# USDA-ARS-GBRU/itsxpress

Hardware: AMD Instinct MI355X
Metric: reads/sec trimmed (ITS2, stand-in taxon Tracheophyta for Fungi) (higher is better)
Workload: dtype u8+f32

## Files before the change

### include/itsx_hip.h

```cpp
#ifndef ITSX_HIP_H
#define ITSX_HIP_H
#include <stdint.h>

#ifdef __cplusplus
extern "C" {
#endif

#define ITSX_ABI_VERSION 6

enum {
  ITSX_OK            =  0,
  ITSX_E_ARG         = -1,
  ITSX_E_IO          = -2,
  ITSX_E_FORMAT      = -3,
  ITSX_E_DEVICE      = -4,
  ITSX_E_UNSUPPORTED = -5,
  ITSX_E_COLLISION   = -6,
  ITSX_E_NOMEM       = -7
};

typedef struct itsx_ctx itsx_ctx;
typedef struct itsx_stream itsx_stream;
typedef struct itsx_keyset itsx_keyset;
typedef struct itsx_twriter itsx_twriter;
// ... 213 lines not shown
int itsx_write_uc(const itsx_ctx *ctx, const char *path);
int itsx_write_rep_fasta(const itsx_ctx *ctx, const char *path);
int itsx_write_domtbl(const itsx_ctx *ctx, const char *path);
int itsx_write_derep_arrays(const char *uc_path, const char *rep_path, int64_t n, const int64_t *rep_of, const int8_t *strand,
                            const int32_t *len, const char *names, const int64_t *name_offsets, const char *seed_bases,
                            const int64_t *seed_offs, int64_t n_seeds);
int itsx_write_domtbl_arrays(const char *path, const itsx_domain *rows, int64_t n_rows, int64_t Z, const int64_t *domz, int32_t n_profiles,
                             const char *prof_names, const int64_t *prof_name_offsets, const int32_t *prof_M, const float *prof_tau,
                             const float *prof_lambda, const char *target_names, const int64_t *target_name_offsets);
const char *itsx_writers_last_error(void);
int itsx_profile_params(const itsx_ctx *ctx, int i, int32_t *M, float *evparam6);
int itsx_get_unique_seqs(itsx_ctx *ctx, char *bases, int64_t cap, int64_t *offsets);

int itsx_get_read_names(const itsx_ctx *ctx, char *names, int64_t cap, int64_t *offsets);

int itsx_get_stats(const itsx_ctx *ctx, itsx_stats *out, int64_t out_size);
int itsx_release_scratch(itsx_ctx *ctx);
int64_t itsx_switches(const itsx_ctx *ctx, char *buf, int64_t cap);
int64_t itsx_switch_registry(char *buf, int64_t cap);

int itsx_write_trimmed_fastq(const char *seq_path, const char *out_path, int compression, int trim_ccs,
                             const int32_t *start, const int32_t *stop, int64_t n_records,
                             int64_t *n_written, int64_t *total_len);
int itsx_twriter_open(const char *out_path, int compression, int trim_ccs, itsx_twriter **w);
int itsx_twriter_set_mode(itsx_twriter *w, int32_t mode);
int itsx_twriter_set_device(itsx_twriter *w, itsx_ctx *ctx);
int itsx_twriter_text(itsx_twriter *w, const char *text, int64_t avail, int32_t last);
int itsx_twriter_coords(itsx_twriter *w, int64_t first_record, int64_t n, const int32_t *start, const int32_t *stop, const uint8_t *decided);
int itsx_twriter_update(itsx_twriter *w, const int64_t *records, int64_t m, const int32_t *start, const int32_t *stop);
int itsx_twriter_close(itsx_twriter *w, int64_t *n_written, int64_t *total_len);

int itsx_write_trimmed_paired(const char *r1_path, const char *r2_path, const char *out1_path, const char *out2_path,
                              int compression, int trim_ccs, const char *names, const int64_t *name_offsets, int64_t n_names,
                              const int32_t *start, const int32_t *stop, const int32_t *tlen, int64_t *n_written);
const char *itsx_trim_last_error(void);
int  itsx_io_read(const char *path, char **text, int64_t *len);
int  itsx_fastq_ids(const char *path, char **names, int64_t **offsets, int64_t *n_records);
void itsx_io_free(char *text);
int  itsx_io_codecs(void);
int64_t itsx_io_parallel_inflates(void);
void itsx_io_cache_clear(void);

int itsx_debug_set_domains(itsx_ctx *ctx, const itsx_domain *rows, int64_t n_rows, const int64_t *seg_rows, int32_t n_segs, int mode);
int64_t itsx_debug_get_rows(itsx_ctx *ctx, itsx_domain *rows, int64_t cap);
int itsx_debug_read_hashes(itsx_ctx *ctx, uint64_t *fwd, uint64_t *rc);
int itsx_debug_read_samples(itsx_ctx *ctx, int32_t *device_ids, int32_t *host_ids);
int itsx_debug_packed_read(const itsx_ctx *ctx, int64_t i, uint32_t *words, int32_t *nwords,
                           uint32_t *exc, int32_t *nexc);
int itsx_debug_calibrate(itsx_ctx *ctx, int pattern, double gbytes, int iters, int64_t *bytes_per_launch, double *ms_per_launch);
int itsx_debug_issue(itsx_ctx *ctx, int op, int waves_per_simd, int iters, double *cycles_per_instr, double *ms);
int itsx_debug_detmath(itsx_ctx *ctx, const double *x, int64_t n, double *out_log, double *out_exp);
int itsx_debug_logf(itsx_ctx *ctx, const float *x, int64_t n, float *out);
int itsx_debug_dust(itsx_ctx *ctx, uint8_t *masked);

#ifdef __cplusplus
}
#endif
#endif
```

### itsxpress_amd/_lib.py

```python
import ctypes as C
import os
import subprocess

import numpy as np

_HERE = os.path.dirname(os.path.abspath(__file__))
LIB_PATH = os.path.join(_HERE, "libitsx_hip.so")
ABI_VERSION = 6
_LIB = None


class EngineError(subprocess.SubprocessError):

    def __init__(self, code, message):
        super().__init__("itsx_hip error %d: %s" % (code, message))
        self.code = code
        self.message = message


DOMAIN_DTYPE = np.dtype([("rep", "<i8"), ("prof", "<i4"), ("tlen", "<i4"), ("ienv", "<i4"), ("jenv", "<i4"),
                         ("dom_idx", "<i4"), ("ndom", "<i4"), ("flags", "<i4"), ("envsc", "<f4"),
                         ("domcorrection", "<f4"), ("dombias", "<f4"), ("bitscore", "<f4"), ("lnP", "<f8"),
                         ("seq_score", "<f4"), ("seq_bias", "<f4"), ("seq_reported", "<i4"),
                         ("dom_reported", "<i4")], align=True)
# ... 9 lines not shown
                ("msv_cells", "<i8"), ("msv_launches", "<i8"), ("ms_fwd_kernel", "<f4"), ("ms_bwd_kernel", "<f4"),
                ("fwd_rows", "<i8"), ("ms_env_kernel", "<f4"), ("ms_bias_kernel", "<f4"), ("env_rows", "<i8"),
                ("n_env_unique", "<i8"), ("ms_decode_kernel", "<f4"), ("n_batches", "<i4"), ("ms_cluster", "<f4"),
                ("n_tw_units_device", "<i4"), ("cl_windows", "<i8"), ("cl_cuts", "<i8"), ("cl_alignments", "<i8"), ("ms_merge", "<f4"),
                ("ms_trim_plan", "<f4"), ("cl_certified", "<i8"), ("ms_pack", "<f4"), ("ms_trim_copy", "<f4"),
                ("n_uniq_multi_winner", "<i8"), ("n_reads_multi_winner", "<i8"), ("n_uniq_region_cap", "<i8"),
                ("n_reads_region_cap", "<i8"), ("n_mr_clustered", "<i8"), ("n_mr_failed", "<i8"), ("n_mr_envelopes", "<i8"),
                ("ms_ensemble", "<f4"), ("ms_deflate", "<f4"), ("n_mr_distinct", "<i8"), ("n_slab_shrinks", "<i8"), ("ms_vit_kernel", "<f4"), ("n_tw_units_host", "<i4"),
                ("n_mr_fail_kind", "<i8", (8,)), ("n_rows_resident", "<i8"),
                ("lazy", "<i4"), ("n_bound_launches", "<i4"), ("n_lazy_pending_profiles", "<i8"), ("n_lazy_completed", "<i8"), ("n_lazy_completed_profiles", "<i8"), ("n_mr_overflow", "<i8"), ("ms_lazy_complete", "<f4"), ("lazy_bound_maxdiff", "<f4"), ("n_lazy_evaluated", "<i8"), ("n_lazy_round1", "<i8"),
                ("n_lazy_pending", "<i8"), ("n_lazy_reruns", "<i8"), ("bound_rows", "<i8"), ("ms_bound_kernel", "<f4"),
                ("ms_lazy_select", "<f4"),
                ("share_B", "<i4"), ("share_batches", "<i4"), ("share_nodes", "<i8"), ("share_chains", "<i8"), ("msv_rows", "<i8"), ("msv_rows_full", "<i8"),
                ("bound_rows_full", "<i8"), ("n_share_helpers", "<i8"), ("share_mismatch", "<i8"), ("ms_share_build", "<f4"), ("share_frac", "<f4"),
                ("two_sided", "<i4"), ("n_bwd_launches", "<i4"), ("n_joined", "<i8"), ("bwd_chains", "<i8"), ("gamma_nodes", "<i8"), ("bwd_rows", "<i8"),
                ("two_fwd_rows", "<i8"), ("two_bwd_rows", "<i8"), ("two_rows_full", "<i8"), ("join_maxdiff", "<f4"), ("ms_bwd_bound", "<f4"),
                ("n_lazy_topup", "<i8"), ("ms_lazy_topup", "<f4"), ("ms_lazy_topup_stages", "<f4"),
                ("ms_inflate", "<f4"), ("n_inflate_members", "<i4"), ("n_inflate_device", "<i8"), ("n_inflate_declined", "<i8")]
STATS_TAIL_FIELDS = [("ms_parse", "<f4"), ("parse_reserved", "<i4"), ("n_parse_device", "<i8"), ("n_parse_declined", "<i8")]
STATS_DTYPE_ALL = np.dtype(STATS_FIELDS + STATS_TAIL_FIELDS, align=True)
_head = np.dtype(STATS_FIELDS, align=True)
STATS_DTYPE = np.dtype({"names": list(_head.names), "formats": [_head.fields[k][0] for k in _head.names],
                        "offsets": [_head.fields[k][1] for k in _head.names], "itemsize": STATS_DTYPE_ALL.itemsize})

EXPORTS = ["itsx_abi_version", "itsx_last_error", "itsx_create", "itsx_destroy", "itsx_load_profiles_file",
           "itsx_load_profiles_mem", "itsx_profile_name", "itsx_profile_tables", "itsx_set_reads", "itsx_set_reads_view", "itsx_set_reads_device", "itsx_domz_device", "itsx_trim_coords_device",
           "itsx_rep_coords_device", "itsx_derep_device", "itsx_unique_keys128_device",
           "itsx_load_reads_file", "itsx_derep", "itsx_cluster", "itsx_cluster_multi", "itsx_cluster_samples", "itsx_get_cluster", "itsx_get_derep", "itsx_unique_keys", "itsx_set_active_uniques", "itsx_get_uniques",
           "itsx_search", "itsx_get_domz", "itsx_set_domz", "itsx_search_finalize", "itsx_num_domains",
           "itsx_get_domains", "itsx_num_pairtraces", "itsx_get_pairtraces", "itsx_trim_coords",
           "itsx_rep_coords", "itsx_write_uc", "itsx_write_rep_fasta", "itsx_write_domtbl", "itsx_get_stats", "itsx_switches", "itsx_switch_registry", "itsx_release_scratch",
           "itsx_debug_read_hashes", "itsx_debug_read_samples", "itsx_debug_packed_read", "itsx_debug_detmath", "itsx_debug_logf", "itsx_debug_dust", "itsx_debug_calibrate", "itsx_debug_issue", "itsx_shard_text", "itsx_shard_last_error", "itsx_owner_verdicts",
           "itsx_write_trimmed_fastq", "itsx_write_trimmed_paired", "itsx_trim_last_error",
           "itsx_merge_buffers", "itsx_merge_pairs_files", "itsx_merge_pairs_load", "itsx_merge_tables",
           "itsx_orient_load_db", "itsx_orient", "itsx_orient_apply", "itsx_write_oriented_fastq",
           "itsx_io_read", "itsx_io_free", "itsx_io_codecs", "itsx_fastq_ids",
           "itsx_load_reads_files", "itsx_set_samples", "itsx_num_samples", "itsx_select_sample",
           "itsx_io_parallel_inflates", "itsx_io_cache_clear", "itsx_get_read_names",
           "itsx_set_rows_mode", "itsx_lazy_pending", "itsx_domz_count", "itsx_lazy_pending_profiles", "itsx_lazy_complete",
           "itsx_load_reads_file_shard", "itsx_unique_keys128", "itsx_write_derep_arrays", "itsx_write_domtbl_arrays",
           "itsx_writers_last_error", "itsx_profile_params", "itsx_get_unique_seqs",
           "itsx_load_reads_text", "itsx_stream_open", "itsx_stream_next", "itsx_stream_close", "itsx_stream_last_error", "itsx_stream_records_bound",
           "itsx_stream_open_shared", "itsx_stream_open_threads", "itsx_stream_base", "itsx_stream_progress", "itsx_stream_next_records", "itsx_count_records",
           "itsx_merge_pairs_load_text", "itsx_merge_pair_index", "itsx_merge_pairs_load_files", "itsx_twriter_set_mode", "itsx_write_range",
           "itsx_keyset_create", "itsx_keyset_destroy", "itsx_keyset_size", "itsx_keyset_assign",
           "itsx_twriter_open", "itsx_twriter_text", "itsx_twriter_coords", "itsx_twriter_update", "itsx_twriter_close",
           "itsx_lazy_pending_uniques", "itsx_set_partial_coords", "itsx_set_kept_rows",
           "itsx_keep_records", "itsx_write_trimmed_samples",
           "itsx_keep_pair_records", "itsx_write_trimmed_paired_samples",
           "itsx_deflate_block_bytes", "itsx_deflate_bound", "itsx_deflate_device", "itsx_debug_huffman_lengths",
           "itsx_twriter_set_device",
           "itsx_inflate_device", "itsx_inflate_fetch", "itsx_debug_inflate_host", "itsx_debug_inflate_candidates", "itsx_debug_inflate_where", "itsx_set_device_inflate",
           "itsx_parse_device", "itsx_parse_fetch", "itsx_debug_parse_host", "itsx_set_device_parse",
           "itsx_debug_set_domains", "itsx_debug_get_rows"]


def lib():
    global _LIB
    if _LIB is not None:
        return _LIB
    if not os.path.exists(LIB_PATH):
        raise FileNotFoundError(
            "%s not found: build the HIP engine first (python -c 'import __graft_entry__ as g; g.build()' "
            "or make -C itsxpress_amd/csrc). There is no CPU fallback." % LIB_PATH)
    L = C.CDLL(LIB_PATH)
    vp, i32, i64, f64, cp = C.c_void_p, C.c_int, C.c_int64, C.c_double, C.c_char_p
    sig = {
        "itsx_abi_version": (i32, []),
        "itsx_last_error": (cp, [vp]),
        "itsx_create": (vp, [i32, i32]),
        "itsx_destroy": (None, [vp]),
        "itsx_load_profiles_file": (i32, [vp, cp, vp]),
        "itsx_load_profiles_mem": (i32, [vp, cp, i64, vp]),
        "itsx_profile_name": (i32, [vp, i32, vp, i32]),
        "itsx_profile_tables": (i32, [vp, i32, vp, vp, vp, vp]),
        "itsx_set_reads": (i32, [vp, vp, vp, i64, vp, vp]),
        "itsx_set_reads_view": (i32, [vp, vp, vp, i64, vp, vp]),
        "itsx_set_reads_device": (i32, [vp, vp, vp, i64, vp, vp]),
        "itsx_domz_device": (i32, [vp, vp, vp]),
        "itsx_trim_coords_device": (i32, [vp, cp, cp, vp, vp]),
        "itsx_rep_coords_device": (i32, [vp, cp, cp, vp, vp]),
        "itsx_derep_device": (i32, [vp, vp, vp, vp, vp]),
        "itsx_unique_keys128_device": (i32, [vp, C.c_uint64, C.c_uint64, i64, vp, vp]),
        "itsx_load_reads_file": (i32, [vp, cp, vp]),
        "itsx_load_reads_file_shard": (i32, [vp, cp, i32, i32, vp, vp, vp]),
        "itsx_load_reads_text": (i32, [vp, vp, i64, vp]),
        "itsx_stream_open": (i32, [cp, vp]),
        "itsx_stream_next": (i32, [vp, i64, vp, vp, vp]),
        "itsx_stream_close": (i32, [vp, i32]),
        "itsx_stream_records_bound": (i64, [vp]),
        "itsx_stream_open_shared": (i32, [cp, cp, vp, vp]),
        "itsx_stream_open_threads": (i32, [cp, i32, vp]),
        "itsx_stream_base": (vp, [vp]),
        "itsx_stream_progress": (i32, [vp, vp, vp, vp]),
        "itsx_stream_next_records": (i32, [vp, i64, vp, vp, vp, vp]),
        "itsx_count_records": (i64, [vp, i64]),
        "itsx_merge_pairs_load_text": (i32, [vp, vp, i64, vp, i64, i32, f64, i32, vp, vp]),
        "itsx_merge_pair_index": (i32, [vp, vp, i64]),
        "itsx_merge_pairs_load_files": (i32, [vp, vp, vp, vp, i32, i32, f64, i32, vp, vp]),
        "itsx_twriter_set_mode": (i32, [vp, i32]),
        "itsx_write_range": (i32, [cp, vp, i64]),
        "itsx_stream_last_error": (cp, []),
        "itsx_keyset_create": (vp, []),
        "itsx_keyset_destroy": (None, [vp]),
        "itsx_keyset_size": (i64, [vp]),
        "itsx_keyset_assign": (i32, [vp, vp, i64, i32, vp, vp]),
        "itsx_twriter_open": (i32, [cp, i32, i32, vp]),
# ... 26 lines not shown
        "itsx_debug_set_domains": (i32, [vp, vp, i64, vp, i32, i32]),
        "itsx_debug_get_rows": (i64, [vp, vp, i64]),
        "itsx_unique_keys128": (i32, [vp, C.c_uint64, C.c_uint64, i64, vp]),
        "itsx_write_derep_arrays": (i32, [cp, cp, i64, vp, vp, vp, vp, vp, vp, vp, i64]),
        "itsx_write_domtbl_arrays": (i32, [cp, vp, i64, i64, vp, i32, vp, vp, vp, vp, vp, vp, vp]),
        "itsx_writers_last_error": (cp, []),
        "itsx_profile_params": (i32, [vp, i32, vp, vp]),
        "itsx_get_unique_seqs": (i32, [vp, vp, i64, vp]),
        "itsx_derep": (i32, [vp, i32, i32, vp]),
        "itsx_cluster": (i32, [vp, f64, i32, vp]),
        "itsx_cluster_multi": (i32, [vp, vp, i32, f64, i32, vp]),
        "itsx_cluster_samples": (i32, [vp, f64, i32, vp]),
        "itsx_get_cluster": (i32, [vp, vp, vp, vp]),
        "itsx_merge_buffers": (i32, [vp, cp, cp, vp, cp, cp, vp, i64, i32, f64, i32, vp, vp, vp, vp, vp, vp]),
        "itsx_merge_pairs_files": (i32, [vp, cp, cp, cp, i32, f64, i32, vp, vp]),
        "itsx_merge_pairs_load": (i32, [vp, cp, cp, i32, f64, i32, vp, vp]),
        "itsx_merge_tables": (i32, [vp, vp, vp, vp, vp]),
        "itsx_orient_load_db": (i32, [vp, cp, vp]),
        "itsx_orient": (i32, [vp, vp, vp, vp]),
        "itsx_orient_apply": (i32, [vp, vp, vp, vp, vp]),
        "itsx_write_oriented_fastq": (i32, [cp, cp, vp, i64, vp]),
        "itsx_unique_keys": (i32, [vp, C.c_uint64, vp, vp]),
        "itsx_set_active_uniques": (i32, [vp, vp]),
        "itsx_get_derep": (i32, [vp, vp, vp, vp]),
        "itsx_get_uniques": (i32, [vp, vp, vp]),
        "itsx_search": (i32, [vp, f64, f64, f64, f64]),
        "itsx_set_rows_mode": (i32, [vp, i32]),
        "itsx_lazy_pending": (i64, [vp]),
        "itsx_lazy_pending_profiles": (i32, [vp, vp]),
        "itsx_lazy_complete": (i32, [vp, vp]),
        "itsx_domz_count": (i64, [vp]),
        "itsx_get_domz": (i32, [vp, vp]),
        "itsx_set_domz": (i32, [vp, vp]),
        "itsx_search_finalize": (i32, [vp, f64]),
        "itsx_num_domains": (i64, [vp]),
        "itsx_get_domains": (i32, [vp, vp]),
        "itsx_num_pairtraces": (i64, [vp]),
        "itsx_get_pairtraces": (i32, [vp, vp, i64]),
        "itsx_trim_coords": (i32, [vp, cp, cp, vp, vp, vp, vp]),
        "itsx_rep_coords": (i32, [vp, cp, cp, vp, vp, vp, vp]),
        "itsx_write_uc": (i32, [vp, cp]),
        "itsx_write_rep_fasta": (i32, [vp, cp]),
        "itsx_write_domtbl": (i32, [vp, cp]),
        "itsx_get_stats": (i32, [vp, vp, i64]),
        "itsx_switches": (i64, [vp, vp, i64]),
        "itsx_release_scratch": (i32, [vp]),
        "itsx_switch_registry": (i64, [vp, i64]),
        "itsx_debug_read_hashes": (i32, [vp, vp, vp]),
        "itsx_debug_read_samples": (i32, [vp, vp, vp]),
        "itsx_debug_packed_read": (i32, [vp, i64, vp, vp, vp, vp]),
        "itsx_debug_detmath": (i32, [vp, vp, i64, vp, vp]),
        "itsx_debug_logf": (i32, [vp, vp, i64, vp]),
        "itsx_debug_dust": (i32, [vp, vp]),
        "itsx_debug_calibrate": (i32, [vp, i32, f64, i32, vp, vp]),
        "itsx_debug_issue": (i32, [vp, i32, i32, i32, vp, vp]),
        "itsx_shard_text": (i32, [C.c_char_p, i32, vp, C.c_char_p, vp, vp]),
        "itsx_shard_last_error": (C.c_char_p, []),
        "itsx_owner_verdicts": (i32, [vp, vp, i64, vp]),
        "itsx_write_trimmed_fastq": (i32, [cp, cp, i32, i32, vp, vp, i64, vp, vp]),
        "itsx_write_trimmed_paired": (i32, [cp, cp, cp, cp, i32, i32, vp, vp, i64, vp, vp, vp, vp]),
        "itsx_trim_last_error": (cp, []),
        "itsx_io_read": (i32, [cp, vp, vp]),
        "itsx_fastq_ids": (i32, [cp, vp, vp, vp]),
        "itsx_io_free": (None, [vp]),
        "itsx_io_codecs": (i32, []),
        "itsx_io_parallel_inflates": (i64, []),
        "itsx_io_cache_clear": (None, []),
        "itsx_get_read_names": (i32, [vp, vp, i64, vp]),
        "itsx_load_reads_files": (i32, [vp, vp, i32, vp]),
        "itsx_set_samples": (i32, [vp, vp, i32]),
        "itsx_num_samples": (i32, [vp]),
        "itsx_select_sample": (i32, [vp, i32]),
    }
    for name, (res, args) in sig.items():
        fn = getattr(L, name)
        fn.restype = res
        fn.argtypes = args
    if L.itsx_abi_version() != ABI_VERSION:
        raise EngineError(-1, "ABI version mismatch: %s reports %d, this package binds version %d" % (LIB_PATH, L.itsx_abi_version(), ABI_VERSION))
    _LIB = L
    return L
```

### itsxpress_amd/csrc/engine.hip

```cpp
#include <algorithm>
#include <chrono>
#include <cmath>
#include <cstdio>
#include <cstring>
#include <functional>
#include <map>
#include <memory>
#include <numeric>
#include <atomic>
#include <condition_variable>
#include <mutex>
#include <string_view>
#include <thread>
#include <unordered_map>
#include "detmath.h"
#include "engine.h"
#include "k_api.h"
#include "deflate_codes.h"
#include "inflate_codes.h"
#include "fastq_rec.h"
#include "twriter_dev.h"
#include "cluster_multi.h"
#include "fastq_io.h"
#include "iupac.h"
// ... 24 lines not shown
}
__global__ void k_waves_build(int nw, int P, const int32_t *__restrict__ order, const int64_t *__restrict__ woff, const int64_t *__restrict__ seg_start,
                              const int32_t *__restrict__ total, const PairRec *__restrict__ pairs, WaveDesc *__restrict__ w, unsigned long long *__restrict__ lane_rows)
{
  const int i = blockIdx.x * blockDim.x + threadIdx.x;
  unsigned long long mine = 0;
  if (i < nw) {
    int lo = 0, hi = P;
    while (hi - lo > 1) { const int mid = (lo + hi) >> 1; if (woff[mid] <= (int64_t)i) lo = mid; else hi = mid; }
    const int p = order[lo];
    const int64_t k = ((int64_t)i - woff[lo]) * 64;
    WaveDesc d;
    d.prof = p; d.first = seg_start[p] + k; d.count = (int32_t)min((int64_t)64, (int64_t)total[p] - k); d.slab = 0;
    int mx = 0;
    for (int q = 0; q < d.count; q++) { const int L = pairs[d.first + q].L; mx = L > mx ? L : mx; mine += (unsigned long long)L; }
    d.rows = mx + 1;
    d.pad = 0;
    w[i] = d;
  }
  for (int o = 32; o >= 1; o >>= 1) mine += __shfl_xor(mine, o, 64);
  if ((threadIdx.x & 63) == 0 && mine) atomicAdd(lane_rows, mine);
}
__global__ void __launch_bounds__(256) k_gather_reads(const uint8_t *__restrict__ src, const int64_t *__restrict__ srcoff, const int64_t *__restrict__ dstoff, int64_t m,
                                                      uint8_t *__restrict__ dst)
{
  const int lane = threadIdx.x & 63;
  for (int64_t j = (int64_t)blockIdx.x * 4 + (threadIdx.x >> 6); j < m; j += (int64_t)gridDim.x * 4) {
    const int64_t so = srcoff[j], d0 = dstoff[j], len = dstoff[j + 1] - d0;
    for (int64_t k = lane; k < len; k += 64) dst[d0 + k] = src[so + k];
  }
}
__global__ void k_wave_rows_regions(const WaveDesc *w, int nw, const RegionRec *rg, int32_t *rows)
{
  const int i = blockIdx.x * blockDim.x + threadIdx.x;
  if (i >= nw) return;
  int mx = 0;
  for (int k = 0; k < w[i].count; k++) { const RegionRec r = rg[w[i].first + k]; mx = max(mx, r.jenv - r.ienv + 1); }
  rows[i] = mx + 1;
}
__global__ void k_pair_counters(const PairOut *po, int64_t n, unsigned long long *c)
{
  unsigned long long a0 = 0, a1 = 0, a2 = 0, a3 = 0, a4 = 0;
  for (int64_t i = (int64_t)blockIdx.x * blockDim.x + threadIdx.x; i < n; i += (int64_t)gridDim.x * blockDim.x) {
    const PairOut o = po[i];
    a0 += o.pass_bias; a1 += o.pass_fwd; a2 += o.pass_fwd ? o.nregions : 0; a3 += (o.flags & 2) ? 1 : 0; a4 += o.pass_fwd ? ((o.flags >> 8) & 0xff) : 0;
  }
  for (int d = 32; d >= 1; d >>= 1) { a0 += __shfl_down(a0, d, 64); a1 += __shfl_down(a1, d, 64); a2 += __shfl_down(a2, d, 64); a3 += __shfl_down(a3, d, 64); a4 += __shfl_down(a4, d, 64); }
  if ((threadIdx.x & 63) == 0) { atomicAdd(&c[0], a0); atomicAdd(&c[1], a1); atomicAdd(&c[2], a2); atomicAdd(&c[3], a3); atomicAdd(&c[4], a4); }
}
__global__ void k_gather_i32(const int32_t *src, const int64_t *idx, int n, int32_t *out)
{
  const int i = blockIdx.x * blockDim.x + threadIdx.x;
  if (i < n) out[i] = src[idx[i]];
}
__global__ void k_rep_coords(int32_t U, const unsigned long long *bl, const unsigned long long *br, const int32_t *cl, const int32_t *cr,
                             const int32_t *seed_read, const int32_t *len, int32_t *start, int32_t *stop, int32_t *tlen)
{
  const int u = blockIdx.x * blockDim.x + threadIdx.x;
  if (u >= U) return;
  const unsigned long long l = bl[u], r = br[u];
  start[u] = l ? cl[u] : -1;
  stop[u] = r ? cr[u] - 1 : -1;
  tlen[u] = (l || r) ? len[seed_read[u]] : -1;
}
__global__ void k_read_coords(int64_t n, const int32_t *uniq_of, const int32_t *us, const int32_t *ue, const int32_t *ut, const int32_t *uind,
                              int32_t *start, int32_t *stop, int32_t *tlen, int32_t *ind)
{
  const int64_t r = (int64_t)blockIdx.x * blockDim.x + threadIdx.x;
  if (r >= n) return;
  const int u = uniq_of[r];
  if (u < 0) { start[r] = stop[r] = tlen[r] = -1; ind[r] = 0; return; }
  start[r] = us[u]; stop[r] = ue[u]; tlen[r] = ut[u]; ind[r] = uind[u];
}
__global__ void k_pack_coords4(int64_t n, const int32_t *a, const int32_t *b, const int32_t *c, const int32_t *d, int32_t *out)
{
  const int64_t i = (int64_t)blockIdx.x * blockDim.x + threadIdx.x;
  if (i < n) { out[i * 4] = a[i]; out[i * 4 + 1] = b[i]; out[i * 4 + 2] = c[i]; out[i * 4 + 3] = d[i]; }
}
__global__ void k_unique_keys128(int32_t U, const int32_t *seed_read, const int32_t *len, const uint64_t *f0, const uint64_t *r0, const uint64_t *f1,
                                 const uint64_t *r1, int64_t base, int64_t *out)
{
  const int u = blockIdx.x * blockDim.x + threadIdx.x;
  if (u >= U) return;
  const int32_t r = seed_read[u];
  const uint64_t lm = (uint64_t)len[r] * 0x9E3779B97F4A7C15ULL;
  const uint64_t kf0 = f0[r] ^ lm, kr0 = r0[r] ^ lm, kf1 = f1[r] ^ lm, kr1 = r1[r] ^ lm;
  const bool fwd_le = (kf0 < kr0) || (kf0 == kr0 && kf1 <= kr1);
  out[(int64_t)u * 4 + 0] = (int64_t)(fwd_le ? kf0 : kr0);
  out[(int64_t)u * 4 + 1] = (int64_t)(fwd_le ? kf1 : kr1);
  out[(int64_t)u * 4 + 2] = base + r;
  out[(int64_t)u * 4 + 3] = fwd_le ? 1 : 0;
}
__global__ void k_widen_i32(int64_t n, const int32_t *in, int64_t *out)
{
  const int64_t i = (int64_t)blockIdx.x * blockDim.x + threadIdx.x;
  if (i < n) out[i] = in[i];
}
}

using namespace itsx;

static std::string g_create_error;

static std::mutex g_grave_mu;
static std::vector<void *> g_grave;
static size_t g_grave_bytes = 0;
// ... 152 lines not shown
  std::vector<int32_t> h_sample, h_usample;
  DBuf<int32_t> d_sample, d_usample;
  const int32_t *dev_sample() const { return S > 1 ? d_sample.p : nullptr; }
  const int32_t *dev_usample() const { return S > 1 ? d_usample.p : nullptr; }
  int32_t usample(int64_t u) const { return S > 1 ? h_usample[(size_t)u] : 0; }
  double slab_gb = 0.0;

  bool have_derep = false;
  std::vector<int32_t> order_cache; bool order_cache_ok = false;
  int derep_strand_both = 1;
  int32_t U = 0;
  int32_t U_active = 0;
  DBuf<int32_t> d_rep_of, d_uniq_of, d_seed_read, d_abund, d_sorted_uniq, d_ulen;
  DBuf<int8_t> d_strand;
  std::vector<int32_t> h_rep_of, h_uniq_of, h_seed_read, h_abund, h_sorted_uniq;
  std::vector<int8_t> h_strand;
  DBuf<uint32_t> d_orient_db; bool have_orient_db = false;
  DBuf<uint32_t> w_orient_tab; DBuf<int32_t> w_orient_list;
  std::vector<int32_t> h_orient_longs;
  bool clustered = false;
  std::vector<double> h_pct;
  std::vector<int32_t> h_order;

  bool have_search = false, have_final = false;
  bool injected = false;
  double T = 10.0;
  int64_t npairs_padded = 0;
  DBuf<PairRec> d_pairs;
  DBuf<PairOut> d_pout;
  DBuf<RegionRec> d_regions;
  DBuf<RegionOut> d_rout;
  DBuf<int64_t> d_pair_region0;
  DBuf<int32_t> d_upos;
  DBuf<RegionRec> d_ulist;
  std::vector<std::unique_ptr<DBuf<itsx_domain>>> dom_bufs;
  std::vector<int64_t> dom_n;
  int64_t pair_budget = 0; int32_t trace_u0 = 0; int n_chunks = 0; bool keep_trace = false, trace_sorted = false;
  DBuf<int16_t> d_vtab; DBuf<VitOut> d_vit; bool have_vit = false; double F2 = 1e-6;
  DBuf<int32_t> d_domz32;
  DBuf<int64_t> d_domz64; bool domz_on_device = false;
  bool compact_rows = false; double compact_zmax = 1e9, compact_dome_min = 1e-2, compact_lnp = 0; int compact_ncls = 0;
  DBuf<itsx_domain> w_domscratch; DBuf<int8_t> w_cls; DBuf<unsigned long long> w_bestc; DBuf<int32_t> w_keep, w_keeppos, w_keeptmp;
  int64_t rows_before_compaction = 0;
  int rows_mode = -1;
  bool lazy = false;
  bool domz_exchanged = false;
  int64_t lazy_pending = 0;
  double sF1 = 1e-6, sF3 = 1e-6;
  std::vector<int64_t> domz_ub;
  std::vector<int64_t> domz_loc, domz_ub_loc;
  bool completing = false;
  std::vector<int32_t> h_plist; DBuf<int32_t> d_plist;
  int64_t s_Uc = 0; int s_Lcap = 0;
  DBuf<float> l_fb; DBuf<uint32_t> l_b10; DBuf<uint8_t> l_done; DBuf<int32_t> l_flag, l_pos, l_scan, l_has; DBuf<unsigned long long> l_gtop, l_sure;
  DBuf<PairRec> l_pairs; DBuf<int64_t> l_seg, l_zub; DBuf<int32_t> l_pflag; DBuf<uint8_t> l_uflag; bool partial_coords = false; bool kept_rows = false; std::vector<int32_t> lazy_pending_prof;
  std::vector<uint16_t> thr_memo; std::vector<char> thr_memo_have; double thr_memo_F1 = -1.0; int thr_memo_Ppad = 0;
  DBuf<int32_t> w_coords4; DBuf<int64_t> w_keys128; DBuf<uint64_t> w_hf1, w_hr1;
  std::vector<int32_t> h_sorted_active;
  DBuf<LenTables> d_lt;
  std::vector<int64_t> domz;
  std::vector<itsx_domain> h_dom;
  std::vector<itsx_pairtrace> h_trace;

  DBuf<uint64_t> w_hf, w_hr; DBuf<unsigned long long> w_keys; DBuf<int32_t> w_vals, w_is_seed, w_seed_rank, w_scan_tmp, w_hist, w_cursor, w_tmp2;
  DBuf<uint32_t> w_slot_of; DBuf<unsigned int> w_ncoll;
  DBuf<uint16_t> w_thr, w_res; DBuf<int32_t> w_tjb, w_cnt, w_total, w_rows, w_rcnt, w_rpref, w_scan2, w_b, w_rrows;
  DBuf<int64_t> w_seg_start, w_idx, w_rseg, w_dz, w_counters, w_useg;
  DBuf<int32_t> w_rrep, w_ruq, w_rurank;
  DBuf<WaveDesc> w_waves, w_rw; DBuf<RegionRec> w_raw; DBuf<float> w_slab, w_eslab;
  DBuf<int32_t> w_mrcnt, w_mroff, w_mrlen, w_mrloff, w_mrrows, w_mrulist, w_mrulist2, w_mru; DBuf<int64_t> w_mrrowoff; DBuf<MrRec> w_mr; DBuf<MrOut> w_mrout; DBuf<int64_t> w_n2off; DBuf<float> w_n2sc, w_mrslab;
  DBuf<uint8_t> w_mrscratch; DBuf<WaveDesc> w_mrwaves;
  DBuf<RegionRec> w_pool, w_pool_sorted; DBuf<int32_t> w_pool_k; DBuf<unsigned long long> w_pool_n, w_pool_key; int64_t pool_cap = 0;
  DBuf<int32_t> w_mrsel; DBuf<int64_t> w_mrselrow; DBuf<MrBig> w_mrbig; DBuf<uint8_t> w_mrarena; DBuf<int32_t> w_mrenv; DBuf<WaveDesc> w_mrbigwaves;
  DBuf<int32_t> w_cl, w_cr;
  DBuf<int8_t> w_side; DBuf<unsigned long long> w_bl, w_br; DBuf<int32_t> w_uind, w_us, w_ue, w_ut, w_rs, w_re, w_rt, w_ri, w_uflag;

  struct ShareBatch { int32_t k0, k1; int64_t node0, nnodes; int32_t nsplit; int64_t gnode0, gnnodes; };
  bool share_on = false; int share_B = 32, share_logB = 5, share_maxd = 0;
  DBuf<unsigned long long> sh_tab, sh_mask_s, sh_mask, sh_counters; DBuf<uint8_t> sh_depth_s, sh_depth;
  DBuf<int32_t> sh_src, sh_parent_s, sh_parent, sh_nn_s, sh_nn, sh_node0_s, sh_node0, sh_order, sh_ulen, sh_uorder, sh_inv, sh_flag, sh_pos, sh_bstart, sh_cursor, sh_segk, sh_scan, sh_cuts;
  std::vector<ShareBatch> sh_batches; std::vector<int32_t> sh_segk_h;
  DBuf<uint4> sh_mgslots; size_t sh_mgslots_half = 0;
  DBuf<uint4> sh_mslots; size_t sh_mslots_half = 0, sh_fslots_half = 0; DBuf<uint32_t> sh_pass, sh_need; DBuf<int32_t> sh_real, sh_segflat, sh_segdepth, sh_wc, sh_woff; DBuf<int64_t> sh_bnd;
  DBuf<uint16_t> sh_res_chk; DBuf<float> sh_fb_chk;
  ShareDev sh_dev{};
  std::string switches_at_search;
  struct TopUp { bool valid = false; int64_t NP = 0; std::vector<int64_t> seg_start; std::vector<int32_t> total; int32_t u0 = 0, Uc = 0; } topup;
  DBuf<unsigned long long> l_zneed, l_zsplit, l_tcnt; DBuf<int32_t> l_slot, l_pslot; DBuf<uint32_t> l_cut;
  std::vector<unsigned long long> h_zneed;
  bool prev_lazy = false; int prev_P = 0; int64_t prev_U = 0, prev_Uc = 0;
  std::vector<int32_t> h_merge_index;
  bool keep_records = false;
  struct Records {
    bool have = false;
    DBuf<uint8_t> seq, qual, titles;
    const uint8_t *seq_p = nullptr;
    DBuf<int64_t> off, toff;
    NameList h_titles;
    void drop() { have = false; seq_p = nullptr; seq.release(); qual.release(); titles.release(); off.release(); toff.release(); h_titles.clear(); }
  } rec;
  bool keep_pair_records = false;
  struct PairRecords {
    bool have = false; int64_t n = 0;
    DBuf<uint8_t> s1, q1, t1, s2, q2, t2;
    DBuf<int64_t> o1, to1, o2, to2;
    DBuf<int32_t> pair_read;
    std::vector<int64_t> pstart;
// ... 1666 lines not shown
    {
      const double n = (double)L;
      const double c = 1.0 + (2.0 * log(2.0 * (n + 3.0) / (3.0 * (n + 2.0))) + n * log((n + 3.0) / (n + 2.0))) / 0.69314718055994529;
      const double margin = std::max(0.02, 6.0 * (n + (double)MMAX) * 5.9604644775390625e-8 / 0.69314718055994529);
      t.lazy_c = nextafterf((float)(c + margin), 1e30f);
    }
    { const float w = roundf((float)(500.0 / 0.69314718055994529) * logf((2.0f + 1.0f) / ((float)L + 2.0f + 1.0f)));
      t.vmove = (w >= 32767.0f) ? 32767 : (w <= -32768.0f) ? -32768 : (int)w; }
  }
  if (ctx->thr_memo_F1 != F1 || ctx->thr_memo_Ppad != Ppad) { ctx->thr_memo.clear(); ctx->thr_memo_have.clear(); ctx->thr_memo_F1 = F1; ctx->thr_memo_Ppad = Ppad; }
  if (ctx->thr_memo_have.size() < (size_t)Lcap) { ctx->thr_memo_have.resize((size_t)Lcap, 0); ctx->thr_memo.resize((size_t)Lcap * Ppad, 257); }
  std::vector<uint16_t> thr((size_t)Lcap * Ppad, 257);
  for (int L = 1; L < Lcap; L++) {
    if (!present[L]) continue;
    if (ctx->thr_memo_have[(size_t)L]) { memcpy(&thr[(size_t)L * Ppad], &ctx->thr_memo[(size_t)L * Ppad], (size_t)Ppad * sizeof(uint16_t)); continue; }
    ctx->thr_memo_have[(size_t)L] = 2;
    for (int p = 0; p < P; p++) {
      const HostProfile &h = ctx->profs[p];
      auto passes = [&](int xj) {
        const float usc = msv_score_from_byte(xj, lt[L].tjb);
        const double Pv = gumbel_surv((double)(usc - lt[L].nullsc) / 0.69314718055994529, (double)h.evparam[0], (double)h.evparam[1]);
        return !(Pv > F1);
      };
      int lo = 0, hi = 255;
      if (!passes(254)) { thr[(size_t)L * Ppad + p] = 256; continue; }
      while (lo < hi) { const int mid = (lo + hi) / 2; if (passes(mid)) hi = mid; else lo = mid + 1; }
      thr[(size_t)L * Ppad + p] = (uint16_t)lo;
    }
  }
  for (int L = 1; L < Lcap; L++)
    if (ctx->thr_memo_have[(size_t)L] == 2) { memcpy(&ctx->thr_memo[(size_t)L * Ppad], &thr[(size_t)L * Ppad], (size_t)Ppad * sizeof(uint16_t)); ctx->thr_memo_have[(size_t)L] = 1; }
  DBuf<uint16_t> &d_thr = ctx->w_thr; DBuf<int32_t> &d_tjb = ctx->w_tjb;
  HIPCHK(upload(ctx->d_lt, lt, st)); HIPCHK(upload(d_thr, thr, st)); HIPCHK(upload(d_tjb, tjb, st));

  HIPCHK(hipStreamSynchronize(st));
  HIPCHK(ctx->d_domz32.alloc((size_t)P * ctx->S));
  HIPCHK(hipMemsetAsync(ctx->d_domz32.p, 0, (size_t)P * ctx->S * 4, st));
  {
    const int64_t cells = cells_active;
    int64_t msum = 0; for (auto &h : ctx->profs) msum += h.M;
    S.msv_cells = cells * msum;
    S.msv_rows = S.msv_rows_full = cells * P; S.bound_rows_full = 0; S.n_share_helpers = 0; S.share_mismatch = 0;
  }
  if (ctx->pair_budget <= 0) {
    size_t fr = 0, tot = 0;
    double gb = 32.0;
    if (hipMemGetInfo(&fr, &tot) == hipSuccess) gb = std::max(1.0, (double)fr / (double)(1ull << 30) / 4.0);
    ctx->pair_budget = (int64_t)(gb * (double)(1ull << 30) / 400.0);
  }
  int64_t lazy_budget = ctx->pair_budget * 5;
  if (ctx->lazy) {
    size_t fr = 0, tot = 0;
    if (hipMemGetInfo(&fr, &tot) == hipSuccess) {
      const double held = (double)ctx->d_pairs.cap * sizeof(PairRec) + (double)ctx->l_fb.cap * 4 + (double)ctx->l_b10.cap * 4 + (double)ctx->l_flag.cap * 4 +
                          (double)ctx->l_pos.cap * 4 + (double)ctx->l_done.cap + (double)ctx->w_res.cap * 2;
      lazy_budget = std::min<int64_t>(lazy_budget, (int64_t)(((double)fr + held) / 3.0 / 64.0));
      lazy_budget = std::max<int64_t>(lazy_budget, (int64_t)1 << 20);
    }
  }
  int64_t Uc = std::max<int64_t>(1, (ctx->lazy ? lazy_budget : ctx->pair_budget) / std::max(P, 1));
  Uc = std::min<int64_t>(Uc, ((1ll << 31) - 4096) / std::max(Ppad, 1));
  if (ctx->lazy && ctx->prev_lazy && ctx->prev_P == P && (int64_t)U <= ctx->prev_U && ctx->prev_Uc > Uc) Uc = ctx->prev_Uc;
  if (const char *e = sw_get("ITSX_CHUNK_UNIQUES")) Uc = std::max<int64_t>(1, atoll(e));
  ctx->keep_trace = sw_get("ITSX_KEEP_TRACE") != nullptr;
  ctx->s_Uc = Uc; ctx->s_Lcap = Lcap;
  ctx->prev_lazy = ctx->lazy; ctx->prev_P = P; ctx->prev_U = U; ctx->prev_Uc = Uc;
  ctx->domz_ub_loc.assign((size_t)P * ctx->S, 0);
  { const int rc = build_share(ctx); if (rc != ITSX_OK) return rc; }
  { const int rc = run_chunks(ctx, T, F1, F3); if (rc != ITSX_OK) return rc; }
  std::vector<int32_t> dz32((size_t)P * ctx->S, 0);
  HIPCHK(hipMemcpyAsync(dz32.data(), ctx->d_domz32.p, dz32.size() * 4, hipMemcpyDeviceToHost, st));
  HIPCHK(hipStreamSynchronize(st));
  ctx->domz_loc.assign(dz32.begin(), dz32.end());
  ctx->domz = ctx->domz_loc; ctx->domz_ub = ctx->domz_ub_loc;
  S.n_rows_resident = 0;
  for (int64_t r : ctx->dom_n) S.n_rows_resident += r;
  if (S.n_mr_failed > 0) {
    ctx->have_search = false;
    SET_ERR(ctx, ITSX_E_UNSUPPORTED, std::to_string(S.n_mr_failed) + " multidomain region(s) with a Forward matrix that cannot be sampled (hmmsearch's stochastic traceback throws on them)");
  }
  return ITSX_OK;
}

struct PairList {
  PairRec *pairs = nullptr; PairOut *pout = nullptr;
  int64_t NP = 0;
  std::vector<int64_t> seg_start;
  std::vector<int32_t> total;
  const int64_t *d_seg_start = nullptr;
};

static int build_waves(itsx_ctx *ctx, const PairList &pl, std::vector<WaveDesc> &waves, std::vector<char> &wgeneric, std::vector<int32_t> &rows)
{
  hipStream_t st = ctx->st;
  const int P = ctx->P;
  waves.clear(); wgeneric.clear();
  for (int pass = 0; pass < 2; pass++)
    for (int p = 0; p < P; p++) {
      if ((int)ctx->generic_q[p] != pass) continue;
      for (int64_t k = 0; k < pl.total[(size_t)p]; k += 64) {
        WaveDesc w{}; w.prof = p; w.first = pl.seg_start[(size_t)p] + k; w.count = (int32_t)std::min<int64_t>(64, pl.total[(size_t)p] - k);
        waves.push_back(w); wgeneric.push_back((char)pass);
      }
    }
  const int NW = (int)waves.size();
  DBuf<WaveDesc> &d_waves = ctx->w_waves; DBuf<int32_t> &d_rows = ctx->w_rows;
  HIPCHK(upload(d_waves, waves, st)); HIPCHK(d_rows.alloc((size_t)std::max(NW, 1)));
  rows.assign((size_t)NW, 0);
// ... 132 lines not shown
      for (int w = w0; w < w1; w++) S.fwd_rows += (int64_t)(rows[w] - 1) * waves[w].count;
      S.n_batches++;
    }
    lazy2.collect();
    lazy.collect();
    S.ms_filters += tm.stop();
  }
  {
    unsigned long long pn = 0;
    HIPCHK(hipMemcpyAsync(&pn, ctx->w_pool_n.p, sizeof(pn), hipMemcpyDeviceToHost, st));
    HIPCHK(hipStreamSynchronize(st));
    if ((int64_t)pn > ctx->pool_cap) {
      while (ctx->pool_cap < (int64_t)pn) ctx->pool_cap *= 2;
      const float keep_ms = S.ms_filters;
      S = stats_before; S.ms_filters = keep_ms; S.n_slab_shrinks++;
      goto pool_retry;
    }
    if (pn > 0) {
      std::vector<RegionRec> hr((size_t)pn); std::vector<int32_t> hk((size_t)pn);
      HIPCHK(hipMemcpyAsync(hr.data(), ctx->w_pool.p, (size_t)pn * sizeof(RegionRec), hipMemcpyDeviceToHost, st));
      HIPCHK(hipMemcpyAsync(hk.data(), ctx->w_pool_k.p, (size_t)pn * 4, hipMemcpyDeviceToHost, st));
      HIPCHK(hipStreamSynchronize(st));
      std::vector<size_t> ord((size_t)pn);
      std::iota(ord.begin(), ord.end(), (size_t)0);
      auto key = [&](size_t i) { return ((unsigned long long)(uint32_t)hr[i].pair << 24) | (unsigned long long)(uint32_t)hk[i]; };
      std::sort(ord.begin(), ord.end(), [&](size_t x, size_t y) { return key(x) < key(y); });
      std::vector<RegionRec> sr((size_t)pn); std::vector<unsigned long long> sk((size_t)pn);
      for (size_t i = 0; i < (size_t)pn; i++) { sr[i] = hr[ord[i]]; sk[i] = key(ord[i]); }
      HIPCHK(upload(ctx->w_pool_sorted, sr, st)); HIPCHK(upload(ctx->w_pool_key, sk, st));
      HIPCHK(hipStreamSynchronize(st));
      pv.rec = ctx->w_pool_sorted.p; pv.key = ctx->w_pool_key.p; pv.n = (int64_t)pn;
    }
  }
  if (next_msv) { const int rc = (*next_msv)(); if (rc != ITSX_OK) return rc; }
  StageTimer tm_dom(st);
  int64_t NMR = 0;
  const bool ensemble = !(sw_get("ITSX_NO_ENSEMBLE") && atoi(sw_get("ITSX_NO_ENSEMBLE")) != 0);
  if (ensemble) {
    DBuf<int32_t> &mrcnt = ctx->w_mrcnt, &mroff = ctx->w_mroff, &stmp = ctx->w_scan2;
    HIPCHK(mrcnt.alloc((size_t)NP + 2)); HIPCHK(mroff.alloc((size_t)NP + 2)); HIPCHK(stmp.alloc((size_t)scan_tmp_elems(NP + 2)));
    launch_mr_count(pl.pout, d_raw.p, pv, NP, mrcnt.p, st);
    launch_exclusive_scan(mrcnt.p, mroff.p, NP + 1, stmp.p, st);
    int32_t tot = 0;
    HIPCHK(hipMemcpyAsync(&tot, mroff.p + NP, 4, hipMemcpyDeviceToHost, st));
    HIPCHK(hipStreamSynchronize(st));
    NMR = tot;
    if (NMR > 0) {
      StageTimer tm_e(st);
      static_assert(sizeof(MrRec) == sizeof(RegionRec), "MrRec is handed to the region memoisation kernels as a RegionRec");
      HIPCHK(ctx->w_mr.alloc((size_t)NMR));
      launch_mr_fill(pl.pout, d_raw.p, pv, NP, mroff.p, ctx->w_mr.p, st);
      DBuf<unsigned long long> &rkeys = ctx->w_keys; DBuf<int32_t> &rvals = ctx->w_vals; DBuf<uint32_t> &rslot = ctx->w_slot_of;
      DBuf<int32_t> &rrep = ctx->w_rrep, &ruq = ctx->w_ruq, &rurank = ctx->w_rurank, &rscan = ctx->w_scan_tmp;
      uint64_t tsize = 1024; while (tsize < (uint64_t)NMR * 2 + 16) tsize <<= 1;
      HIPCHK(rkeys.alloc(tsize)); HIPCHK(rvals.alloc(tsize)); HIPCHK(rslot.alloc((size_t)NMR + 1));
      HIPCHK(rrep.alloc((size_t)NMR + 1)); HIPCHK(ruq.alloc((size_t)NMR + 1)); HIPCHK(rurank.alloc((size_t)NMR + 1)); HIPCHK(rscan.alloc((size_t)scan_tmp_elems(NMR + 1)));
      HIPCHK(hipMemsetAsync(rkeys.p, 0, tsize * sizeof(unsigned long long), st));
      HIPCHK(hipMemsetAsync(rvals.p, 0x7f, tsize * sizeof(int32_t), st));
      HIPCHK(hipMemsetAsync(ruq.p, 0, ((size_t)NMR + 1) * sizeof(int32_t), st));
      const RegionRec *mr_as_regions = (const RegionRec *)ctx->w_mr.p;
      launch_region_keys(ctx->rd, mr_as_regions, NMR, pl.pairs, d_sorted, ctx->d_seed_read.p, rkeys.p, rvals.p, tsize - 1, rslot.p, st);
      launch_region_resolve(ctx->rd, mr_as_regions, NMR, pl.pairs, d_sorted, ctx->d_seed_read.p, rvals.p, rslot.p, rrep.p, ruq.p, st);
      launch_exclusive_scan(ruq.p, rurank.p, NMR + 1, rscan.p, st);
      int32_t NU = 0;
      HIPCHK(hipMemcpyAsync(&NU, rurank.p + NMR, 4, hipMemcpyDeviceToHost, st));
      HIPCHK(hipStreamSynchronize(st));
      DBuf<int32_t> &ulist0 = ctx->w_mrulist, &ulist = ctx->w_mrulist2, &ulen = ctx->w_mrlen, &newpos = ctx->w_mrloff, &mru = ctx->w_mru;
      HIPCHK(ulist0.alloc((size_t)NU + 1)); HIPCHK(ulist.alloc((size_t)NU + 1)); HIPCHK(ulen.alloc((size_t)NU + 2)); HIPCHK(newpos.alloc((size_t)NU + 2)); HIPCHK(mru.alloc((size_t)NMR + 1));
      launch_mr_ulist(NMR, ctx->w_mr.p, rrep.p, ruq.p, rurank.p, ulist0.p, ulen.p, mru.p, st);
      std::vector<int32_t> hlen((size_t)NU), ord((size_t)NU), hpos((size_t)NU);
      HIPCHK(hipMemcpyAsync(hlen.data(), ulen.p, (size_t)NU * 4, hipMemcpyDeviceToHost, st));
      HIPCHK(hipStreamSynchronize(st));
      std::iota(ord.begin(), ord.end(), 0);
      std::stable_sort(ord.begin(), ord.end(), [&](int32_t x, int32_t y) { return hlen[(size_t)x] < hlen[(size_t)y]; });
      std::vector<int64_t> hn2((size_t)NU + 1, 0), hrow((size_t)NU + 1, 0);
      for (int32_t x = 0; x < NU; x++) {
        const int32_t o = ord[(size_t)x];
        hpos[(size_t)o] = x;
        hn2[(size_t)x + 1] = hn2[(size_t)x] + hlen[(size_t)o];
        hrow[(size_t)x + 1] = hrow[(size_t)x] + hlen[(size_t)o] + 1;
      }
      HIPCHK(hipMemcpyAsync(newpos.p, hpos.data(), (size_t)NU * 4, hipMemcpyHostToDevice, st));
      launch_mr_reorder(NU, NMR, newpos.p, ulist0.p, ulist.p, mru.p, st);
      HIPCHK(upload(ctx->w_n2off, hn2, st)); HIPCHK(upload(ctx->w_mrrowoff, hrow, st));
      HIPCHK(ctx->w_mrout.alloc((size_t)NU)); HIPCHK(ctx->w_n2sc.alloc((size_t)hn2[(size_t)NU] + 1));
      static const int lanes_long = sw_get("ITSX_MR_LONG_LANES") ? std::max(1, std::min(MR_LANES, atoi(sw_get("ITSX_MR_LONG_LANES")))) : MR_LANES_LONG;
      static const double frac_long = sw_get("ITSX_MR_LONG_FRAC") ? atof(sw_get("ITSX_MR_LONG_FRAC")) : MR_LONG_FRAC;
      const int64_t n_long = std::min<int64_t>(NU, (int64_t)(frac_long * (double)NU));
      const int64_t waves_target = sw_get("ITSX_MR_WAVES") ? atoll(sw_get("ITSX_MR_WAVES")) : 4096;
      const int lanes_norm = waves_target <= 0 ? MR_LANES : (int)std::max<int64_t>(2, std::min<int64_t>(MR_LANES, (NU + waves_target - 1) / waves_target));
      std::vector<WaveDesc> mw;
      std::vector<int64_t> wfirst;
      for (int64_t x = 0; x < NU;) {
        const int lanes = x >= NU - n_long ? std::min(lanes_long, lanes_norm) : (int)std::min<int64_t>(lanes_norm, NU - n_long - x);
        WaveDesc d{};
        d.prof = -1; d.first = x; d.count = (int32_t)std::min<int64_t>(lanes, (int64_t)NU - x);
        d.rows = hlen[(size_t)ord[(size_t)(d.first + d.count - 1)]] + 1;
        wfirst.push_back(x);
        mw.push_back(d);
        x += d.count;
      }
      const int NMW = (int)mw.size();
      wfirst.push_back(NU);
      HIPCHK(upload(ctx->w_mrwaves, mw, st));
      const int64_t mrow_bytes = (int64_t)MRV * 16;
      const int64_t mbudget = std::max<int64_t>(1, (int64_t)(std::min(slab_gb, 16.0) * (1 << 30)) / mrow_bytes);
      const int64_t wave_cap = std::max<int64_t>(1, ((int64_t)6 << 30) / ((int64_t)MR_SCRATCH * MR_LANES));
// ... 87 lines not shown
            launch_mr_ensemble_big(mb, (int)bw.size(), st);
            x0 = x1;
          }
        }
      }
      S.ms_ensemble += tm_e.stop();
      HIPCHK(hipGetLastError());
      S.n_mr_clustered += NMR; S.n_mr_distinct += NU;
    }
  }
  DBuf<int32_t> &d_rcnt = ctx->w_rcnt, &d_rpref = ctx->w_rpref, &d_scan_tmp = ctx->w_scan2;
  HIPCHK(d_rcnt.alloc((size_t)NP + 1)); HIPCHK(d_rpref.alloc((size_t)NP + 1)); HIPCHK(d_scan_tmp.alloc((size_t)scan_tmp_elems(NP + 1)));
  HIPCHK(hipMemsetAsync(d_rcnt.p, 0, ((size_t)NP + 1) * 4, st));
  RegionListArgs rl{};
  rl.pout = pl.pout; rl.raw = d_raw.p; rl.pv = pv; rl.npairs = NP;
  if (NMR > 0) { rl.mr_off = ctx->w_mroff.p; rl.mr_u = ctx->w_mru.p; rl.mrout = ctx->w_mrout.p; rl.envpool = ctx->w_mrenv.p; }
  {
    DBuf<int64_t> &d_c = ctx->w_counters;
    HIPCHK(d_c.alloc(16));
    HIPCHK(hipMemsetAsync(d_c.p, 0, 16 * sizeof(int64_t), st));
    launch_region_list_count(rl, d_rcnt.p, (unsigned long long *)d_c.p, st);
    int64_t hc[10] = {0};
    HIPCHK(hipMemcpyAsync(hc, d_c.p, sizeof(hc), hipMemcpyDeviceToHost, st));
    HIPCHK(hipStreamSynchronize(st));
    S.n_mr_failed += hc[0]; S.n_mr_envelopes += hc[1];
    for (int k = 0; k < 8; k++) S.n_mr_fail_kind[k] += hc[2 + k];
  }
  launch_exclusive_scan(d_rcnt.p, d_rpref.p, NP + 1, d_scan_tmp.p, st);
  std::vector<int32_t> bound((size_t)P + 1);
  {
    DBuf<int64_t> &d_idx = ctx->w_idx; DBuf<int32_t> &d_b = ctx->w_b;
    HIPCHK(upload(d_idx, pl.seg_start, st)); HIPCHK(d_b.alloc((size_t)P + 1));
    hipLaunchKernelGGL(k_gather_i32, dim3((P + 1 + 255) / 256), dim3(256), 0, st, d_rpref.p, d_idx.p, P + 1, d_b.p);
    HIPCHK(hipMemcpyAsync(bound.data(), d_b.p, ((size_t)P + 1) * 4, hipMemcpyDeviceToHost, st));
    HIPCHK(hipStreamSynchronize(st));
  }
  std::vector<int64_t> rseg((size_t)P + 1, 0);
  std::vector<int32_t> rtotal((size_t)P);
  for (int p = 0; p < P; p++) { rtotal[p] = bound[p + 1] - bound[p]; rseg[p + 1] = rseg[p] + ((int64_t)rtotal[p] + 63) / 64 * 64; S.n_domains += rtotal[p]; }
  const int64_t NR = rseg[P];
  ctx->dom_n[di] = NR;
  HIPCHK(ctx->d_pair_region0.alloc((size_t)NP));
  HIPCHK(ctx->d_regions.alloc((size_t)std::max<int64_t>(NR, 1)));
  HIPCHK(d_dom.alloc((size_t)std::max<int64_t>(NR, 1)));
  HIPCHK(hipMemsetAsync(d_dom.p, 0xFF, (size_t)std::max<int64_t>(NR, 1) * sizeof(itsx_domain), st));
  if (NR > 0) {
    DBuf<int64_t> &d_rseg = ctx->w_rseg;
    HIPCHK(upload(d_rseg, rseg, st));
    launch_region_offsets(NP, pl.pairs, d_rpref.p, pl.d_seg_start, d_rseg.p, ctx->d_pair_region0.p, st);
    HIPCHK(hipMemsetAsync(ctx->d_regions.p, 0xFF, (size_t)NR * sizeof(RegionRec), st));
    launch_region_list_fill(rl, ctx->d_pair_region0.p, ctx->d_regions.p, st);
    DBuf<unsigned long long> &rkeys = ctx->w_keys; DBuf<int32_t> &rvals = ctx->w_vals; DBuf<uint32_t> &rslot = ctx->w_slot_of;
    DBuf<int32_t> &rrep = ctx->w_rrep, &ruq = ctx->w_ruq, &rurank = ctx->w_rurank, &rscan = ctx->w_scan_tmp;
    uint64_t tsize = 1024; while (tsize < (uint64_t)NR * 2 + 16) tsize <<= 1;
    HIPCHK(rkeys.alloc(tsize)); HIPCHK(rvals.alloc(tsize)); HIPCHK(rslot.alloc((size_t)NR + 1));
    HIPCHK(rrep.alloc((size_t)NR + 1)); HIPCHK(ruq.alloc((size_t)NR + 1)); HIPCHK(rurank.alloc((size_t)NR + 1));
    HIPCHK(rscan.alloc((size_t)scan_tmp_elems(NR + 1))); HIPCHK(ctx->d_upos.alloc((size_t)NR + 1));
    HIPCHK(hipMemsetAsync(rkeys.p, 0, tsize * sizeof(unsigned long long), st));
    HIPCHK(hipMemsetAsync(rvals.p, 0x7f, tsize * sizeof(int32_t), st));
    HIPCHK(hipMemsetAsync(ruq.p, 0, ((size_t)NR + 1) * sizeof(int32_t), st));
    launch_region_keys(ctx->rd, ctx->d_regions.p, NR, pl.pairs, d_sorted, ctx->d_seed_read.p, rkeys.p, rvals.p, tsize - 1, rslot.p, st);
    launch_region_resolve(ctx->rd, ctx->d_regions.p, NR, pl.pairs, d_sorted, ctx->d_seed_read.p, rvals.p, rslot.p, rrep.p, ruq.p, st);
    launch_exclusive_scan(ruq.p, rurank.p, NR + 1, rscan.p, st);
    std::vector<int32_t> ub((size_t)P + 1);
    {
      DBuf<int64_t> &d_idx = ctx->w_idx; DBuf<int32_t> &d_b = ctx->w_b;
      HIPCHK(upload(d_idx, rseg, st)); HIPCHK(d_b.alloc((size_t)P + 1));
      hipLaunchKernelGGL(k_gather_i32, dim3((P + 1 + 255) / 256), dim3(256), 0, st, rurank.p, d_idx.p, P + 1, d_b.p);
      HIPCHK(hipMemcpyAsync(ub.data(), d_b.p, ((size_t)P + 1) * 4, hipMemcpyDeviceToHost, st));
      HIPCHK(hipStreamSynchronize(st));
    }
    std::vector<int64_t> useg((size_t)P + 1, 0);
    std::vector<int32_t> utotal((size_t)P);
    for (int p = 0; p < P; p++) { utotal[p] = ub[p + 1] - ub[p]; useg[p + 1] = useg[p] + ((int64_t)utotal[p] + 63) / 64 * 64; S.n_env_unique += utotal[p]; }
    const int64_t NU = useg[P];
    DBuf<int64_t> &d_useg = ctx->w_useg;
    HIPCHK(upload(d_useg, useg, st));
    HIPCHK(ctx->d_ulist.alloc((size_t)std::max<int64_t>(NU, 1))); HIPCHK(ctx->d_rout.alloc((size_t)std::max<int64_t>(NU, 1)));
    HIPCHK(hipMemsetAsync(ctx->d_rout.p, 0, (size_t)std::max<int64_t>(NU, 1) * sizeof(RegionOut), st));
    launch_region_upos(NR, ctx->d_regions.p, pl.pairs, ruq.p, rurank.p, d_rseg.p, d_useg.p, ctx->d_upos.p, ctx->d_ulist.p, st);
    launch_region_upos_follow(NR, rrep.p, ruq.p, ctx->d_upos.p, st);
    std::vector<WaveDesc> rw; std::vector<char> rgen;
    for (int pass = 0; pass < 2; pass++)
      for (int p = 0; p < P; p++) {
        if ((int)ctx->generic_q[p] != pass) continue;
        for (int64_t k = 0; k < utotal[p]; k += 64) {
          WaveDesc w{}; w.prof = p; w.first = useg[p] + k; w.count = (int32_t)std::min<int64_t>(64, utotal[p] - k);
          rw.push_back(w); rgen.push_back((char)pass);
        }
      }
    const int NRW = (int)rw.size();
    DBuf<WaveDesc> &d_rw = ctx->w_rw; DBuf<int32_t> &d_rrows = ctx->w_rrows;
    HIPCHK(upload(d_rw, rw, st)); HIPCHK(d_rrows.alloc((size_t)NRW));
    hipLaunchKernelGGL(k_wave_rows_regions, dim3((NRW + 255) / 256), dim3(256), 0, st, d_rw.p, NRW, ctx->d_ulist.p, d_rrows.p);
    std::vector<int32_t> rrows((size_t)NRW);
    HIPCHK(hipMemcpyAsync(rrows.data(), d_rrows.p, (size_t)NRW * 4, hipMemcpyDeviceToHost, st));
    HIPCHK(hipStreamSynchronize(st));
    const int64_t erow_bytes = 104 * 64 * 4;
    int64_t ebudget = (int64_t)(slab_gb * (1 << 30)) / erow_bytes;
    LazyTimers elazy(st);
    DBuf<float> &d_eslab = ctx->w_eslab; int64_t ealloc = (int64_t)(d_eslab.cap / (104 * 64));
    if (adapt && !sw_get("ITSX_SLAB_GB")) {
      int64_t total_rows = 0;
      for (int w = 0; w < NRW; w++) total_rows += rrows[(size_t)w];
      ebudget = std::min(ebudget, std::max(std::max(total_rows / 4 + 1, ((int64_t)2 << 30) / erow_bytes), ealloc));
    }
    int w0 = 0;
    while (w0 < NRW) {
      int w1 = w0; int64_t r = 0;
      while (w1 < NRW && rgen[w1] == rgen[w0] && (w1 == w0 || r + rrows[w1] <= ebudget)) { rw[w1].slab = r; rw[w1].rows = rrows[w1]; r += rrows[w1]; w1++; }
      if (r > ealloc) {
        if (d_eslab.alloc((size_t)r * 104 * 64) != hipSuccess) {
          (void)hipGetLastError();
          ealloc = 0;
          if (w1 - w0 <= 1) SET_ERR(ctx, ITSX_E_NOMEM, "no device memory left for the envelope slab of a single wave");
          ebudget = std::max<int64_t>(r / 2, rrows[(size_t)w0]);
          S.n_slab_shrinks++;
          continue;
        }
        ealloc = r;
      }
      HIPCHK(hipMemcpyAsync(d_rw.p + w0, rw.data() + w0, (size_t)(w1 - w0) * sizeof(WaveDesc), hipMemcpyHostToDevice, st));
      EnvArgs a{};
      a.rd = ctx->rd; a.sorted_uniq = d_sorted; a.seed_read = ctx->d_seed_read.p; a.prof = ctx->d_prof.p; a.lt = ctx->d_lt.p;
      a.pairs = pl.pairs; a.regions = ctx->d_ulist.p; a.rout = ctx->d_rout.p; a.waves = d_rw.p; a.slab = d_eslab.p;
      { const size_t t = elazy.begin(&S.ms_env_kernel); launch_envelopes(a, w1 - w0, w0, rgen[w0], st); elazy.end(t); }
      for (int w = w0; w < w1; w++) S.env_rows += (int64_t)(rrows[w] - 1) * rw[w].count;
      w0 = w1;
    }
    ScoreArgs sa{};
    sa.rd = ctx->rd; sa.sorted_uniq = d_sorted; sa.seed_read = ctx->d_seed_read.p; sa.prof = ctx->d_prof.p; sa.lt = ctx->d_lt.p;
    sa.flogsum = ctx->d_flogsum.p; sa.pairs = pl.pairs; sa.pout = pl.pout; sa.regions = ctx->d_regions.p; sa.rout = ctx->d_rout.p;
    sa.pair_region0 = ctx->d_pair_region0.p; sa.upos = ctx->d_upos.p; sa.dom = d_dom.p; sa.npairs = NP; sa.T = T;
    if (NMR > 0) { sa.mr = ctx->w_mr.p; sa.mr_u = ctx->w_mru.p; sa.mrout = ctx->w_mrout.p; sa.n2off = ctx->w_n2off.p; sa.n2sc = ctx->w_n2sc.p; sa.mr_off = ctx->w_mroff.p; }
    sa.domz = ctx->d_domz32.p; sa.usample = ctx->dev_usample(); sa.P = ctx->P;
    launch_score(sa, st);
    if (ctx->compact_rows) {
      { const int rc = compact_segment(ctx, d_dom.p, NR, di); if (rc != ITSX_OK) return rc; }
    }
  }
  S.ms_domains += tm_dom.stop();
  {
    DBuf<int64_t> &d_c = ctx->w_counters;
    HIPCHK(d_c.alloc(8));
    HIPCHK(hipMemsetAsync(d_c.p, 0, 8 * sizeof(int64_t), st));
    hipLaunchKernelGGL(k_pair_counters, dim3((unsigned)std::min<int64_t>(4096, (NP + 255) / 256)), dim3(256), 0, st, pl.pout, NP, (unsigned long long *)d_c.p);
    int64_t hc[8];
    HIPCHK(hipMemcpyAsync(hc, d_c.p, sizeof(hc), hipMemcpyDeviceToHost, st));
    HIPCHK(hipStreamSynchronize(st));
    S.n_past_bias += hc[0]; S.n_past_fwd += hc[1]; S.n_regions += hc[2]; S.n_domain_overflow += hc[3]; S.n_multidomain += hc[4];
  }
  HIPCHK(hipGetLastError());
  return ITSX_OK;
}


namespace itsx {
__global__ void k_dbg_group_count(const PairRec *__restrict__ pairs, int64_t NP, const int32_t *__restrict__ flag, const int8_t *__restrict__ cls, int ncls, unsigned long long *__restrict__ cnt)
{
  const int64_t i = (int64_t)blockIdx.x * blockDim.x + threadIdx.x;
  if (i >= NP || !flag[i]) return;
  const PairRec pr = pairs[i];
  if (pr.prof < 0) return;
  atomicAdd(&cnt[(size_t)pr.useq * ncls + cls[pr.prof]], 1ull);
}
__global__ void k_dbg_group_hist(const unsigned long long *__restrict__ cnt, int64_t ng, unsigned long long *__restrict__ hist)
{
  const int64_t i = (int64_t)blockIdx.x * blockDim.x + threadIdx.x;
  if (i >= ng) return;
  const unsigned long long c = cnt[i];
  const int b = c <= 4 ? (int)c : c <= 8 ? 5 : c <= 16 ? 6 : 7;
  atomicAdd(&hist[b], 1ull);
  if (c > 1) atomicAdd(&hist[8], c - 1);
  if (c > 2) atomicAdd(&hist[9], c - 2);
}
}

static int lazy_rounds(itsx_ctx *ctx, const PairList &pl, const int32_t *d_sorted, int32_t u0, int32_t Uc, double T, double F1, double F3, const std::function<int()> *next_msv)
{
  hipStream_t st = ctx->st;
  const int P = ctx->P, ncls = ctx->compact_ncls;
  itsx_stats &S = ctx->stats;
  const int64_t NP = pl.NP;
  HIPCHK(ctx->l_fb.alloc((size_t)NP + 1)); HIPCHK(ctx->l_b10.alloc((size_t)NP + 1)); HIPCHK(ctx->l_done.alloc((size_t)NP + 1));
  HIPCHK(ctx->l_flag.alloc((size_t)NP + 2)); HIPCHK(ctx->l_pos.alloc((size_t)NP + 2)); HIPCHK(ctx->l_scan.alloc((size_t)scan_tmp_elems(NP + 2)));
  HIPCHK(ctx->l_gtop.alloc((size_t)Uc * ncls + 1));
  HIPCHK(hipMemsetAsync(ctx->l_done.p, 0, (size_t)NP + 1, st));
  HIPCHK(hipMemsetAsync(ctx->l_gtop.p, 0, ((size_t)Uc * ncls + 1) * sizeof(unsigned long long), st));
  if (ctx->share_on) {
    const int maxd = ctx->share_maxd, DS = maxd + 1;
    const bool two = ctx->two_on;
    std::vector<int32_t> segflat, segdepth, segbatch;
    for (size_t bi = 0; bi < ctx->sh_batches.size(); bi++) {
      const auto &b = ctx->sh_batches[bi];
      if (b.k0 < u0 || b.k0 >= u0 + Uc) continue;
      for (int d = 0; d < DS; d++) { segflat.push_back(ctx->sh_segk_h[bi * SHARE_SEGS + d] - u0); segdepth.push_back(d); segbatch.push_back((int32_t)bi); }
    }
    const int nseg = (int)segdepth.size();
    segflat.push_back(Uc);
    if ((int64_t)nseg * P + 1 >= (1ll << 31)) SET_ERR(ctx, ITSX_E_UNSUPPORTED, "prefix sharing: too many (batch, depth, profile) segments in one chunk");
    HIPCHK(upload(ctx->sh_segflat, segflat, st)); HIPCHK(upload(ctx->sh_segdepth, segdepth, st, 1)); HIPCHK(upload(ctx->w_rcnt, pl.total, st));
    HIPCHK(ctx->sh_bnd.alloc((size_t)(nseg + 1) * P)); HIPCHK(ctx->sh_wc.alloc((size_t)nseg * P + 2)); HIPCHK(ctx->sh_woff.alloc((size_t)nseg * P + 2));
    HIPCHK(ctx->sh_scan.alloc((size_t)scan_tmp_elems((int64_t)nseg * P + 2)));
    launch_share_bounds(pl.pairs, pl.d_seg_start, ctx->w_rcnt.p, ctx->sh_segflat.p, nseg, P, ctx->sh_bnd.p, st);
    launch_share_wcount(ctx->sh_bnd.p, nseg, P, ctx->sh_wc.p, st);
    launch_exclusive_scan(ctx->sh_wc.p, ctx->sh_woff.p, (int64_t)nseg * P + 1, ctx->sh_scan.p, st);
    std::vector<int32_t> woff((size_t)nseg * P + 1);
    HIPCHK(hipMemcpyAsync(woff.data(), ctx->sh_woff.p, woff.size() * 4, hipMemcpyDeviceToHost, st));
    HIPCHK(hipStreamSynchronize(st));
    const int NW = woff.back();
    HIPCHK(ctx->w_waves.alloc((size_t)std::max(NW, 1))); HIPCHK(ctx->w_counters.alloc(512));
    HIPCHK(hipMemsetAsync(ctx->w_counters.p, 0, 512 * sizeof(int64_t), st));
    launch_share_waves(NW, nseg, P, ctx->sh_woff.p, ctx->sh_bnd.p, ctx->sh_segdepth.p, ctx->share_B, pl.pairs, two ? ctx->sh_endrow.p + u0 : nullptr, 0, ctx->w_waves.p,
                       (unsigned long long *)ctx->w_counters.p, st);
    std::vector<int64_t> lr((size_t)384, 0);
    FloatArgs a{};
    a.rd = ctx->rd; a.sorted_uniq = d_sorted; a.seed_read = ctx->d_seed_read.p; a.prof = ctx->d_prof.p; a.lt = ctx->d_lt.p;
    a.pairs = pl.pairs; a.waves = ctx->w_waves.p; a.F1 = F1; a.F3 = F3;
    const int maxrd = ctx->share_maxrd, DSB = maxrd + 1;
    int32_t cb0 = 0, Ubc = 0; int NWB = 0;
    std::vector<int32_t> bwoff;
    FloatArgs ab = a;
    if (two) {
      int32_t cb1 = 0; bool any = false;
      std::vector<int32_t> bsegflat, bsegdepth;
      for (size_t bi = 0; bi < ctx->sh_batches.size(); bi++) {
        const auto &b = ctx->sh_batches[bi];
        if (b.k0 < u0 || b.k0 >= u0 + Uc) continue;
        const int32_t lo = ctx->sh_bsegk_h[bi * SHARE_SEGS], hi = ctx->sh_bsegk_h[bi * SHARE_SEGS + SHARE_SEGS - 1];
        if (!any) { cb0 = lo; any = true; }
        cb1 = hi;
      }
      Ubc = any ? cb1 - cb0 : 0;
      for (size_t bi = 0; bi < ctx->sh_batches.size(); bi++) {
        const auto &b = ctx->sh_batches[bi];
        if (b.k0 < u0 || b.k0 >= u0 + Uc) continue;
        for (int d = 0; d < DSB; d++) { bsegflat.push_back(ctx->sh_bsegk_h[bi * SHARE_SEGS + d] - cb0); bsegdepth.push_back(d); }
      }
// ... 155 lines not shown
      for (int p = 0; p < P; p++) {
        if ((int)ctx->generic_q[p] != pass) continue;
        order.push_back(p);
        woff.push_back(woff.back() + ((int64_t)pl.total[(size_t)p] + 63) / 64);
        if (pass == 0) nfast64 = woff.back();
      }
    if (woff.back() >= (1ll << 31)) SET_ERR(ctx, ITSX_E_UNSUPPORTED, "more than 2^31 waves of pairs in one chunk");
    const int NW = (int)woff.back(), nfast = (int)nfast64;
    DBuf<int32_t> &d_order = ctx->w_b; DBuf<int64_t> &d_woff = ctx->w_idx; DBuf<int32_t> &d_tot = ctx->w_rcnt;
    HIPCHK(upload(d_order, order, st)); HIPCHK(upload(d_woff, woff, st)); HIPCHK(upload(d_tot, pl.total, st));
    HIPCHK(ctx->w_waves.alloc((size_t)std::max(NW, 1))); HIPCHK(ctx->w_counters.alloc(16));
    HIPCHK(hipMemsetAsync(ctx->w_counters.p, 0, 16 * sizeof(int64_t), st));
    if (NW > 0) hipLaunchKernelGGL(k_waves_build, dim3((NW + 255) / 256), dim3(256), 0, st, NW, (int)order.size(), d_order.p, d_woff.p, pl.d_seg_start, d_tot.p,
                                   pl.pairs, ctx->w_waves.p, (unsigned long long *)ctx->w_counters.p);
    int64_t lane_rows = 0;
    HIPCHK(hipMemcpyAsync(&lane_rows, ctx->w_counters.p, sizeof(lane_rows), hipMemcpyDeviceToHost, st));
    FloatArgs a{};
    a.rd = ctx->rd; a.sorted_uniq = d_sorted; a.seed_read = ctx->d_seed_read.p; a.prof = ctx->d_prof.p; a.lt = ctx->d_lt.p;
    a.pairs = pl.pairs; a.waves = ctx->w_waves.p; a.F1 = F1; a.F3 = F3;
    StageTimer tm(st);
    static const bool exact_bound = sw_get("ITSX_LAZY_EXACT_BOUND") && atoi(sw_get("ITSX_LAZY_EXACT_BOUND")) != 0;
    if (!exact_bound) {
      for (int w0 = 0; w0 < NW; w0 += 1 << 20) { launch_fwd_bound_seq(a, ctx->d_btab.p, ctx->bound_fold, ctx->l_fb.p, std::min(1 << 20, NW - w0), w0, st); S.n_bound_launches++; }
    } else {
      for (int w0 = 0; w0 < nfast; w0 += 1 << 20) { launch_fwd_bound(a, ctx->l_fb.p, std::min(1 << 20, nfast - w0), w0, 0, st); S.n_bound_launches++; }
      if (NW > nfast) { launch_fwd_bound(a, ctx->l_fb.p, NW - nfast, nfast, 1, st); S.n_bound_launches++; }
    }
    const float ms = tm.stop();
    S.ms_bound_kernel += ms; S.ms_filters += ms;
    if (sw_get("ITSX_LAZY_CHECK_BOUND") && !exact_bound) {
      DBuf<float> ref;
      HIPCHK(ref.alloc((size_t)NP + 1));
      for (int w0 = 0; w0 < nfast; w0 += 1 << 20) launch_fwd_bound(a, ref.p, std::min(1 << 20, nfast - w0), w0, 0, st);
      if (NW > nfast) launch_fwd_bound(a, ref.p, NW - nfast, nfast, 1, st);
      std::vector<float> h0((size_t)NP), h1((size_t)NP); std::vector<PairRec> hp((size_t)NP);
      HIPCHK(hipMemcpyAsync(h0.data(), ref.p, (size_t)NP * 4, hipMemcpyDeviceToHost, st));
      HIPCHK(hipMemcpyAsync(h1.data(), ctx->l_fb.p, (size_t)NP * 4, hipMemcpyDeviceToHost, st));
      HIPCHK(hipMemcpyAsync(hp.data(), pl.pairs, (size_t)NP * sizeof(PairRec), hipMemcpyDeviceToHost, st));
      HIPCHK(hipStreamSynchronize(st));
      float mx = S.lazy_bound_maxdiff;
      for (int64_t i = 0; i < NP; i++) {
        if (hp[(size_t)i].prof < 0) continue;
        const float x = h0[(size_t)i], y = h1[(size_t)i];
        if (x != x || y != y) { if ((x != x) != (y != y)) mx = 1e30f; continue; }
        mx = std::max(mx, fabsf(x - y));
      }
      S.lazy_bound_maxdiff = mx;
    }
    S.bound_rows += lane_rows; S.bound_rows_full += lane_rows;
  }
  StageTimer tm_sel(st);
  LazyArgs la{};
  la.pairs = pl.pairs; la.NP = NP; la.fb = ctx->l_fb.p; la.lt = ctx->d_lt.p; la.cls = ctx->w_cls.p; la.ncls = ncls; la.sorted_uniq = d_sorted;
  la.b10 = ctx->l_b10.p; la.gtop = ctx->l_gtop.p; la.bestc = ctx->w_bestc.p; la.done = ctx->l_done.p; la.flag = ctx->l_flag.p;
  launch_lazy_bound(la, st);
  float ms_sel = tm_sel.stop();
  for (int round = 0; round < 2; round++) {
    StageTimer tm_r(st);
    launch_lazy_mark(la, round, st);
    if (round == 1 && sw_get("ITSX_LAZY_HIST")) {
      const int64_t ng = (int64_t)Uc * ncls;
      HIPCHK(hipMemsetAsync(ctx->l_gtop.p, 0, (size_t)ng * 8, st));
      hipLaunchKernelGGL(k_dbg_group_count, dim3((unsigned)((NP + 255) / 256)), dim3(256), 0, st, pl.pairs, NP, ctx->l_flag.p, ctx->w_cls.p, ncls, ctx->l_gtop.p);
      DBuf<unsigned long long> hist; HIPCHK(hist.alloc(16)); HIPCHK(hipMemsetAsync(hist.p, 0, 16 * 8, st));
      hipLaunchKernelGGL(k_dbg_group_hist, dim3((unsigned)((ng + 255) / 256)), dim3(256), 0, st, ctx->l_gtop.p, ng, hist.p);
      unsigned long long h[16];
      HIPCHK(hipMemcpyAsync(h, hist.p, sizeof(h), hipMemcpyDeviceToHost, st)); HIPCHK(hipStreamSynchronize(st));
      fprintf(stderr, "[itsx] round 2 candidates per group: 0:%llu 1:%llu 2:%llu 3:%llu 4:%llu 5-8:%llu 9-16:%llu 17+:%llu; pairs beyond a group's first %llu, beyond its second %llu\n",
              h[0], h[1], h[2], h[3], h[4], h[5], h[6], h[7], h[8], h[9]);
    }
    launch_exclusive_scan(ctx->l_flag.p, ctx->l_pos.p, NP + 1, ctx->l_scan.p, st);
    std::vector<int32_t> bound((size_t)P + 1);
    {
      DBuf<int64_t> &d_idx = ctx->w_idx; DBuf<int32_t> &d_b = ctx->w_b;
      HIPCHK(upload(d_idx, pl.seg_start, st)); HIPCHK(d_b.alloc((size_t)P + 1));
      hipLaunchKernelGGL(k_gather_i32, dim3((P + 1 + 255) / 256), dim3(256), 0, st, ctx->l_pos.p, d_idx.p, P + 1, d_b.p);
      HIPCHK(hipMemcpyAsync(bound.data(), d_b.p, ((size_t)P + 1) * 4, hipMemcpyDeviceToHost, st));
      HIPCHK(hipStreamSynchronize(st));
    }
    PairList sub;
    sub.seg_start.assign((size_t)P + 1, 0); sub.total.assign((size_t)P, 0);
    for (int p = 0; p < P; p++) { sub.total[(size_t)p] = bound[(size_t)p + 1] - bound[(size_t)p]; sub.seg_start[(size_t)p + 1] = sub.seg_start[(size_t)p] + ((int64_t)sub.total[(size_t)p] + 63) / 64 * 64; }
    sub.NP = sub.seg_start[(size_t)P];
    const int64_t nsel = (int64_t)bound[(size_t)P] - bound[0];
    const bool last = round == 1;
    if (sub.NP == 0) {
      ms_sel += tm_r.stop();
      if (last && next_msv) { const int rc = (*next_msv)(); if (rc != ITSX_OK) return rc; }
      continue;
    }
    HIPCHK(ctx->l_pairs.alloc((size_t)sub.NP)); HIPCHK(ctx->d_pout.alloc((size_t)sub.NP));
    HIPCHK(hipMemsetAsync(ctx->l_pairs.p, 0xFF, (size_t)sub.NP * sizeof(PairRec), st));
    HIPCHK(hipMemsetAsync(ctx->d_pout.p, 0, (size_t)sub.NP * sizeof(PairOut), st));
    HIPCHK(upload(ctx->l_seg, sub.seg_start, st));
    launch_lazy_scatter(pl.pairs, NP, ctx->l_flag.p, ctx->l_pos.p, pl.d_seg_start, ctx->l_seg.p, ctx->l_pairs.p, st);
    sub.pairs = ctx->l_pairs.p; sub.pout = ctx->d_pout.p; sub.d_seg_start = ctx->l_seg.p;
    ms_sel += tm_r.stop();
    S.n_lazy_evaluated += nsel;
    if (round == 0) S.n_lazy_round1 += nsel;
    { const int rc = domain_pipeline(ctx, sub, d_sorted, T, F1, F3, last ? next_msv : nullptr); if (rc != ITSX_OK) return rc; }
  }
  S.ms_lazy_select += ms_sel; S.ms_filters += ms_sel;
  ctx->topup.valid = !ctx->completing; ctx->topup.NP = NP; ctx->topup.seg_start = pl.seg_start; ctx->topup.total = pl.total; ctx->topup.u0 = u0; ctx->topup.Uc = Uc;
  return ITSX_OK;
}

static int search_chunk(itsx_ctx *ctx, int ci, int32_t u0, int32_t U, int Lcap, double T, double F1, double F3)
{
  (void)ci;
  hipStream_t st = ctx->st;
  const int P = ctx->P, G = ctx->G, Ppad = G * 64;
  itsx_stats &S = ctx->stats;
  const bool sh = ctx->share_on;
  const int32_t *d_sorted = (sh ? ctx->sh_order.p : ctx->d_sorted_uniq.p) + u0;
  const int32_t *d_ulen = (sh ? ctx->sh_ulen.p : ctx->d_ulen.p) + u0;
  DBuf<uint16_t> &d_thr = ctx->w_thr; DBuf<int32_t> &d_tjb = ctx->w_tjb;
  ctx->trace_u0 = u0;
  DBuf<uint16_t> &d_res = ctx->w_res;
  HIPCHK(d_res.alloc((size_t)Ppad * std::max<int64_t>(U, ctx->next_u0 >= 0 ? ctx->next_U : 0)));
  auto msv_for = [&](int64_t cu0, int32_t cU, hipStream_t s, int lds_pad = 0, uint16_t *res_out = nullptr, bool shared = true) {
    MsvArgs a{};
    a.rd = ctx->rd; a.sorted_uniq = (sh ? ctx->sh_order.p : ctx->d_sorted_uniq.p) + cu0; a.seed_read = ctx->d_seed_read.p; a.U = cU; a.G = G;
    a.etab = ctx->d_etab.p; a.pbias = ctx->d_pbias.p; a.ptec = ctx->d_ptec.p; a.ptbm = ctx->d_ptbm.p;
    a.thr = d_thr.p; a.tjb = d_tjb.p; a.Lcap = Lcap; a.res = res_out ? res_out : d_res.p;
    a.P = P;
    const int64_t tiles = ((int64_t)cU + 255) / 256;
    if (ctx->completing) {
      a.plist = ctx->d_plist.p; a.nlist = (int32_t)ctx->h_plist.size();
      (void)hipMemsetAsync(a.res, 0, (size_t)Ppad * (size_t)cU * sizeof(uint16_t), s);
    }
    const int np = a.plist ? a.nlist : P;
    a.PB = (int)std::max<int64_t>(1, std::min<int64_t>(32, tiles * np / 4096));
    if (!sh || !shared || ctx->completing) { launch_msv(a, s, lds_pad); return; }
    static const bool two = !(sw_get("ITSX_SHARE_MSV_STREAMS") && atoi(sw_get("ITSX_SHARE_MSV_STREAMS")) < 2);
    int nbatch_here = 0;
    for (const auto &b : ctx->sh_batches) nbatch_here += (b.k0 >= cu0 && b.k0 < cu0 + cU);
    hipStream_t alt = s;
    if (two && nbatch_here > 1) {
      if (!ctx->st3) {
        if (hipStreamCreateWithFlags(&ctx->st3, hipStreamNonBlocking) != hipSuccess) { (void)hipGetLastError(); ctx->st3 = nullptr; }
        else { (void)hipEventCreateWithFlags(&ctx->ev_s3a, hipEventDisableTiming); (void)hipEventCreateWithFlags(&ctx->ev_s3b, hipEventDisableTiming); }
      }
      if (ctx->st3) { alt = ctx->st3; (void)hipEventRecord(ctx->ev_s3a, s); (void)hipStreamWaitEvent(alt, ctx->ev_s3a, 0); }
    }
    static const bool msv_two = !(sw_get("ITSX_MSV_TWO") && atoi(sw_get("ITSX_MSV_TWO")) == 0);
    const bool bi2 = ctx->two_on && msv_two;
    int32_t cb0 = 0;
    if (bi2) { bool any = false; for (const auto &b : ctx->sh_batches) if (b.k0 >= cu0 && b.k0 < cu0 + cU && !any) { cb0 = ctx->sh_bsegk_h[(size_t)(&b - ctx->sh_batches.data()) * SHARE_SEGS]; any = true; } }
    int seen = 0;
// ... 333 lines not shown
  for (size_t c = 0; c < ctx->dom_n.size(); c++)
    if (ctx->dom_n[c] > 0) launch_finalize_lazy(ctx->dom_bufs[c]->p, ctx->dom_n[c], d_dz.p, d_dz.p + m, domE, ctx->dev_usample(), ctx->P, st);
  for (size_t c = 0; c < ctx->dom_n.size(); c++)
    if (ctx->dom_n[c] > 0) launch_lazy_sure(ctx->dom_bufs[c]->p, ctx->dom_n[c], ctx->w_cls.p, ncls, ctx->l_sure.p, ctx->l_has.p, st);
  for (size_t c = 0; c < ctx->dom_n.size(); c++)
    if (ctx->dom_n[c] > 0) launch_lazy_pending(ctx->dom_bufs[c]->p, ctx->dom_n[c], ctx->w_cls.p, ncls, ctx->l_sure.p, ctx->l_has.p, (unsigned long long *)ctx->w_counters.p, ctx->l_pflag.p, ctx->l_uflag.p, ctx->S == 1 ? ctx->l_zneed.p : nullptr, ctx->l_zsplit.p, domE, st);
  int64_t pend = 0;
  ctx->h_zneed.assign((size_t)std::max(ctx->P, 1) * 2, 0);
  HIPCHK(hipMemcpyAsync(ctx->h_zneed.data(), ctx->l_zneed.p, (size_t)std::max(ctx->P, 1) * 2 * sizeof(unsigned long long), hipMemcpyDeviceToHost, st));
  HIPCHK(hipMemcpyAsync(&pend, ctx->w_counters.p, sizeof(pend), hipMemcpyDeviceToHost, st));
  ctx->lazy_pending_prof.assign((size_t)std::max(ctx->P, 1), 0);
  HIPCHK(hipMemcpyAsync(ctx->lazy_pending_prof.data(), ctx->l_pflag.p, (size_t)std::max(ctx->P, 1) * 4, hipMemcpyDeviceToHost, st));
  HIPCHK(hipStreamSynchronize(st));
  { int np = 0; for (int32_t f : ctx->lazy_pending_prof) np += f != 0; ctx->stats.n_lazy_pending_profiles = np; }
  if (sw_get("ITSX_LAZY_FORCE_PENDING")) pend += atoll(sw_get("ITSX_LAZY_FORCE_PENDING"));
  ctx->lazy_pending = pend; ctx->stats.n_lazy_pending = pend;
  return ITSX_OK;
}

static int lazy_topup(itsx_ctx *ctx, double domE, bool *ran)
{
  (void)domE;
  *ran = false;
  const auto &tu = ctx->topup;
  if (sw_get("ITSX_LAZY_HIST")) fprintf(stderr, "[itsx] top-up: valid %d chunks %d samples %d pairs %lld\n", (int)tu.valid, ctx->n_chunks, ctx->S, (long long)tu.NP);
  if (!tu.valid || ctx->n_chunks != 1 || ctx->S != 1 || tu.NP <= 0) return ITSX_OK;
  if (sw_get("ITSX_LAZY_TOPUP") && atoi(sw_get("ITSX_LAZY_TOPUP")) == 0) return ITSX_OK;
  hipStream_t st = ctx->st;
  const int P = ctx->P;
  itsx_stats &S = ctx->stats;
  std::vector<int32_t> slot((size_t)P, -1), prof_of;
  for (int p = 0; p < P; p++) {
    if (!ctx->lazy_pending_prof[(size_t)p]) continue;
    if (ctx->h_zneed[(size_t)2 * p] == 0 && ctx->h_zneed[(size_t)2 * p + 1] == ~0ull) continue;
    slot[(size_t)p] = (int32_t)prof_of.size(); prof_of.push_back(p);
  }
  const int ns = (int)prof_of.size();
  if (ns == 0) return ITSX_OK;
  StageTimer tm(st);
  const int64_t NP = tu.NP;
  HIPCHK(upload(ctx->l_slot, slot, st)); HIPCHK(upload(ctx->l_pslot, prof_of, st));
  HIPCHK(upload(ctx->w_idx, tu.seg_start, st)); HIPCHK(upload(ctx->w_rcnt, tu.total, st));
  auto count_done = [&](std::vector<unsigned long long> &out) -> int {
    HIPCHK(ctx->l_tcnt.alloc((size_t)ns));
    HIPCHK(hipMemsetAsync(ctx->l_tcnt.p, 0, (size_t)ns * sizeof(unsigned long long), st));
    launch_topup_count(ctx->l_done.p, ctx->w_idx.p, ctx->w_rcnt.p, ctx->l_pslot.p, ns, ctx->l_tcnt.p, st);
    out.assign((size_t)ns, 0);
    HIPCHK(hipMemcpyAsync(out.data(), ctx->l_tcnt.p, (size_t)ns * sizeof(unsigned long long), hipMemcpyDeviceToHost, st));
    HIPCHK(hipStreamSynchronize(st));
    return ITSX_OK;
  };
  std::vector<unsigned long long> ndone;
  { const int rc = count_done(ndone); if (rc != ITSX_OK) return rc; }
  launch_topup_keys(ctx->d_pairs.p, NP, ctx->l_done.p, ctx->l_b10.p, ctx->l_slot.p, ctx->l_flag.p, nullptr, nullptr, nullptr, st);
  launch_exclusive_scan(ctx->l_flag.p, ctx->l_pos.p, NP + 1, ctx->l_scan.p, st);
  int32_t M32 = 0;
  HIPCHK(hipMemcpyAsync(&M32, ctx->l_pos.p + NP, 4, hipMemcpyDeviceToHost, st));
  HIPCHK(hipStreamSynchronize(st));
  const int64_t M = M32;
  if (M <= 0) return ITSX_OK;
  HIPCHK(ctx->sh_keys.alloc((size_t)M + 1)); HIPCHK(ctx->sh_keys2.alloc((size_t)M + 1)); HIPCHK(ctx->sh_vals.alloc((size_t)M + 1)); HIPCHK(ctx->sh_uorder.alloc((size_t)M + 1));
  const size_t sort_bytes = order_sort_bytes(M);
  HIPCHK(ctx->sh_sorttmp.alloc(sort_bytes));
  launch_topup_keys(ctx->d_pairs.p, NP, ctx->l_done.p, ctx->l_b10.p, ctx->l_slot.p, ctx->l_flag.p, ctx->l_pos.p, ctx->sh_keys.p, ctx->sh_vals.p, st);
  if (order_sort(ctx->sh_sorttmp.p, sort_bytes, ctx->sh_keys.p, ctx->sh_keys2.p, ctx->sh_vals.p, ctx->sh_uorder.p, M, st) != 0) SET_ERR(ctx, ITSX_E_DEVICE, "top-up round: the radix sort failed");
  HIPCHK(hipStreamSynchronize(st));
  auto lower = [&](unsigned long long key, int64_t &pos) -> int {
    int64_t lo = 0, hi = M;
    while (lo < hi) {
      const int64_t mid = (lo + hi) >> 1; unsigned long long v = 0;
      HIPCHK(hipMemcpy(&v, ctx->sh_keys2.p + mid, 8, hipMemcpyDeviceToHost));
      if (v < key) lo = mid + 1; else hi = mid;
    }
    pos = lo; return ITSX_OK;
  };
  std::vector<uint32_t> cut((size_t)2 * ns, 0);
  bool any = false;
  for (int k = 0; k < ns; k++) {
    const int p = prof_of[(size_t)k];
    int64_t a = 0, b = 0;
    { const int rc = lower((unsigned long long)k << 32, a); if (rc != ITSX_OK) return rc; }
    { const int rc = lower((unsigned long long)(k + 1) << 32, b); if (rc != ITSX_OK) return rc; }
    const int64_t have = b - a;
    if (have <= 0) continue;
    const int64_t lo = ctx->domz[(size_t)p], hi = lo + have;
    int64_t from_top = 0, from_bottom = 0;
    const unsigned long long zl = ctx->h_zneed[(size_t)2 * p], zh = ctx->h_zneed[(size_t)2 * p + 1];
    if (zl > 0 && (int64_t)zl > lo) { const int64_t need = (int64_t)zl - lo; from_top = need + need / 50 + 64; }
    const bool both = sw_get("ITSX_LAZY_TOPUP") && atoi(sw_get("ITSX_LAZY_TOPUP")) == 2;
    if (both && zh != ~0ull && hi > (int64_t)zh) { const int64_t need = hi - (int64_t)zh; from_bottom = need + need / 4 + 64; }
    if (sw_get("ITSX_LAZY_HIST")) fprintf(stderr, "[itsx] top-up: profile %d bounds %lld .. %lld (%lld unevaluated), rows need >= %llu / <= %llu: best %lld, weakest %lld\n", p, (long long)lo, (long long)hi,
                                          (long long)have, zl, zh == ~0ull ? 0ull : zh, (long long)from_top, (long long)from_bottom);
    static const bool topup_all = !(sw_get("ITSX_LAZY_TOPUP_ALL") && atoi(sw_get("ITSX_LAZY_TOPUP_ALL")) == 0);
    const bool above = zh != ~0ull && hi > (int64_t)zh;
    if ((above && !both) || from_top + from_bottom > have - have / 3) {
      if (!topup_all) continue;
      cut[(size_t)2 * k] = 1u; cut[(size_t)2 * k + 1] = 0u;
      any = true;
      continue;
    }
    unsigned long long v = 0;
    if (from_top > 0) {
      HIPCHK(hipMemcpy(&v, ctx->sh_keys2.p + a + from_top - 1, 8, hipMemcpyDeviceToHost));
      cut[(size_t)2 * k] = std::max<uint32_t>(1u, 0xFFFFFFFFu - (uint32_t)(v & 0xFFFFFFFFull));
    }
    if (from_bottom > 0) {
      HIPCHK(hipMemcpy(&v, ctx->sh_keys2.p + b - from_bottom, 8, hipMemcpyDeviceToHost));
      cut[(size_t)2 * k + 1] = std::max<uint32_t>(1u, 0xFFFFFFFFu - (uint32_t)(v & 0xFFFFFFFFull));
      if (cut[(size_t)2 * k] > 0 && cut[(size_t)2 * k + 1] >= cut[(size_t)2 * k]) { cut[(size_t)2 * k] = cut[(size_t)2 * k + 1] = 0; continue; }
    }
    any = any || from_top > 0 || from_bottom > 0;
  }
  if (!any) return ITSX_OK;
  HIPCHK(upload(ctx->l_cut, cut, st));
  launch_topup_mark(ctx->d_pairs.p, NP, ctx->l_done.p, ctx->l_b10.p, ctx->l_slot.p, ctx->l_cut.p, ctx->l_flag.p, st);
  launch_exclusive_scan(ctx->l_flag.p, ctx->l_pos.p, NP + 1, ctx->l_scan.p, st);
  std::vector<int32_t> bound((size_t)P + 1);
  {
    DBuf<int32_t> &d_b = ctx->w_b;
    HIPCHK(d_b.alloc((size_t)P + 1));
    hipLaunchKernelGGL(k_gather_i32, dim3((P + 1 + 255) / 256), dim3(256), 0, st, ctx->l_pos.p, ctx->w_idx.p, P + 1, d_b.p);
    HIPCHK(hipMemcpyAsync(bound.data(), d_b.p, ((size_t)P + 1) * 4, hipMemcpyDeviceToHost, st));
    HIPCHK(hipStreamSynchronize(st));
  }
  PairList sub;
  sub.seg_start.assign((size_t)P + 1, 0); sub.total.assign((size_t)P, 0);
  for (int p = 0; p < P; p++) { sub.total[(size_t)p] = bound[(size_t)p + 1] - bound[(size_t)p]; sub.seg_start[(size_t)p + 1] = sub.seg_start[(size_t)p] + ((int64_t)sub.total[(size_t)p] + 63) / 64 * 64; }
  sub.NP = sub.seg_start[(size_t)P];
  const int64_t nsel = (int64_t)bound[(size_t)P] - bound[0];
  if (sub.NP == 0) return ITSX_OK;
  HIPCHK(ctx->l_pairs.alloc((size_t)sub.NP)); HIPCHK(ctx->d_pout.alloc((size_t)sub.NP));
  HIPCHK(hipMemsetAsync(ctx->l_pairs.p, 0xFF, (size_t)sub.NP * sizeof(PairRec), st));
  HIPCHK(hipMemsetAsync(ctx->d_pout.p, 0, (size_t)sub.NP * sizeof(PairOut), st));
  HIPCHK(upload(ctx->l_seg, sub.seg_start, st));
  launch_lazy_scatter(ctx->d_pairs.p, NP, ctx->l_flag.p, ctx->l_pos.p, ctx->w_seg_start.p, ctx->l_seg.p, ctx->l_pairs.p, st);
  sub.pairs = ctx->l_pairs.p; sub.pout = ctx->d_pout.p; sub.d_seg_start = ctx->l_seg.p;
  const int32_t *d_sorted = (ctx->share_on ? ctx->sh_order.p : ctx->d_sorted_uniq.p) + tu.u0;
  ctx->trace_u0 = tu.u0;
  { StageTimer tp(st); const int rc = domain_pipeline(ctx, sub, d_sorted, ctx->T, ctx->sF1, ctx->sF3, nullptr); if (rc != ITSX_OK) return rc; S.ms_lazy_topup_stages += tp.stop(); }
  std::vector<int32_t> dz32((size_t)P * ctx->S, 0);
  HIPCHK(hipMemcpyAsync(dz32.data(), ctx->d_domz32.p, dz32.size() * 4, hipMemcpyDeviceToHost, st));
  HIPCHK(upload(ctx->w_idx, tu.seg_start, st)); HIPCHK(upload(ctx->w_rcnt, tu.total, st));
  { const int rc = count_done(ndone); if (rc != ITSX_OK) return rc; }
  for (size_t z = 0; z < dz32.size(); z++) { ctx->domz_loc[z] = dz32[z]; ctx->domz[z] = dz32[z]; }
  for (int k = 0; k < ns; k++) {
    const int p = prof_of[(size_t)k];
    const int64_t left = (int64_t)tu.total[(size_t)p] - (int64_t)ndone[(size_t)k];
    const int64_t hi = (int64_t)dz32[(size_t)p] + std::max<int64_t>(0, left);
    if (hi < ctx->domz_ub[(size_t)p]) { ctx->domz_ub[(size_t)p] = hi; ctx->domz_ub_loc[(size_t)p] = hi; }
    if (sw_get("ITSX_LAZY_HIST")) fprintf(stderr, "[itsx] top-up: profile %d now %d .. %lld\n", p, dz32[(size_t)p], (long long)ctx->domz_ub[(size_t)p]);
  }
  S.n_lazy_evaluated += nsel; S.n_lazy_topup += nsel;
  S.n_rows_resident = 0;
  for (int64_t r : ctx->dom_n) S.n_rows_resident += r;
  S.ms_lazy_topup += tm.stop();
  *ran = true;
  return ITSX_OK;
}

int itsx_search_finalize(itsx_ctx *ctx, double domE)
{
  CTXCHK(ctx && ctx->have_search);
  HIPCHK(hipSetDevice(ctx->device));
  if (ctx->injected && ctx->lazy && !ctx->domz_exchanged)
    SET_ERR(ctx, ITSX_E_ARG, "itsx_search_finalize: a lazy row table that was handed in (itsx_debug_set_domains) has no counters of its own: give both bounds with itsx_set_domz first");
  StageTimer tm(ctx->st);
  ctx->h_dom.clear();
  auto check_compaction = [&](const std::vector<int64_t> &z) -> int {
    int64_t zmax = 0;
    for (int64_t v : z) zmax = std::max(zmax, v);
    if ((double)zmax > ctx->compact_zmax || domE < ctx->compact_dome_min)
      SET_ERR(ctx, ITSX_E_UNSUPPORTED, "compacted domain rows: only the rows that are reported for every domZ <= " + std::to_string(ctx->compact_zmax) +
              " and every domE >= " + std::to_string(ctx->compact_dome_min) + " were kept, but finalize got domZ up to " + std::to_string(zmax) + " and domE " + std::to_string(domE) +
              " (raise ITSX_COMPACT_ZMAX / lower ITSX_COMPACT_DOME_MIN and search again)");
    return ITSX_OK;
  };
  if (ctx->lazy) {
    { const int rc = finalize_lazy(ctx, domE); if (rc != ITSX_OK) return rc; }
    { const int rc = check_compaction(ctx->domz_ub); if (rc != ITSX_OK) return rc; }
    if (ctx->lazy_pending > 0 && !ctx->domz_exchanged && !sw_get("ITSX_LAZY_NO_RERUN")) {
      const int64_t pend = ctx->lazy_pending;
      {
        bool ran = false;
        { const int rc = lazy_topup(ctx, domE, &ran); if (rc != ITSX_OK) return rc; }
        if (ran) {
          { const int rc = finalize_lazy(ctx, domE); if (rc != ITSX_OK) return rc; }
          ctx->stats.n_lazy_pending = pend;
          if (ctx->lazy_pending == 0) {
            ctx->stats.ms_finalize = tm.stop();
// ... 2025 lines not shown
  return ITSX_OK;
}

int itsx_debug_detmath(itsx_ctx *ctx, const double *x, int64_t n, double *out_log, double *out_exp)
{
  CTXCHK(ctx && x && out_log && out_exp && n >= 0);
  HIPCHK(hipSetDevice(ctx->device));
  DBuf<double> dx, dl, de;
  HIPCHK(dx.alloc((size_t)n + 1)); HIPCHK(dl.alloc((size_t)n + 1)); HIPCHK(de.alloc((size_t)n + 1));
  if (n > 0) {
    HIPCHK(hipMemcpyAsync(dx.p, x, (size_t)n * 8, hipMemcpyHostToDevice, ctx->st));
    launch_detmath(dx.p, n, dl.p, de.p, ctx->st);
    HIPCHK(hipMemcpyAsync(out_log, dl.p, (size_t)n * 8, hipMemcpyDeviceToHost, ctx->st));
    HIPCHK(hipMemcpyAsync(out_exp, de.p, (size_t)n * 8, hipMemcpyDeviceToHost, ctx->st));
  }
  HIPCHK(hipStreamSynchronize(ctx->st));
  return ITSX_OK;
}

int itsx_debug_dust(itsx_ctx *ctx, uint8_t *masked)
{
  CTXCHK(ctx && masked);
  HIPCHK(hipSetDevice(ctx->device));
  const int64_t n = ctx->N;
  if (n == 0) return ITSX_OK;
  DBuf<uint32_t> dm;
  HIPCHK(dm.alloc((size_t)ctx->h_woff[n] + 1));
  launch_dust(ctx->rd, dm.p, ctx->st);
  std::vector<uint32_t> h((size_t)ctx->h_woff[n] + 1);
  HIPCHK(hipMemcpyAsync(h.data(), dm.p, h.size() * 4, hipMemcpyDeviceToHost, ctx->st));
  HIPCHK(hipStreamSynchronize(ctx->st));
  HIPCHK(hipGetLastError());
  int64_t o = 0;
  for (int64_t r = 0; r < n; r++)
    for (int p = 0; p < ctx->h_len[r]; p++) masked[o++] = (uint8_t)((h[(size_t)ctx->h_woff[r] + (p >> 5)] >> (p & 31)) & 1u);
  return ITSX_OK;
}

int itsx_debug_logf(itsx_ctx *ctx, const float *x, int64_t n, float *out)
{
  CTXCHK(ctx && x && out && n >= 0);
  HIPCHK(hipSetDevice(ctx->device));
  DBuf<float> dx, dy;
  HIPCHK(dx.alloc((size_t)n + 1)); HIPCHK(dy.alloc((size_t)n + 1));
  if (n > 0) {
    HIPCHK(hipMemcpyAsync(dx.p, x, (size_t)n * 4, hipMemcpyHostToDevice, ctx->st));
    launch_logf_fast(dx.p, n, ctx->d_logtab.p, dy.p, ctx->st);
    HIPCHK(hipMemcpyAsync(out, dy.p, (size_t)n * 4, hipMemcpyDeviceToHost, ctx->st));
  }
  HIPCHK(hipStreamSynchronize(ctx->st));
  return ITSX_OK;
}

}
```

### itsxpress_amd/csrc/k_api.h

```cpp
#pragma once
#include "engine.h"

#include "detmath.h"
namespace itsx {

struct ReadsDev {
  const uint32_t *words;
  const int64_t  *woff;
  const int32_t  *len;
  const int64_t  *excoff;
  const uint32_t *exc;
  int64_t         n;
};

void launch_hash_reads(const ReadsDev &rd, uint64_t seed, int strand_both, uint64_t *hf, uint64_t *hr, hipStream_t st, const int32_t *sample = nullptr);
void launch_table_insert(int64_t n, const int32_t *len, int minlen, const uint64_t *hf, const uint64_t *hr,
                         unsigned long long *keys, int32_t *vals, uint64_t mask, uint32_t *slot_of, hipStream_t st);
void launch_table_resolve(const ReadsDev &rd, const uint64_t *hf, const int32_t *vals, const uint32_t *slot_of,
                          int32_t *rep_of, int8_t *strand, int32_t *is_seed, unsigned int *n_collisions, hipStream_t st,
                          const int32_t *sample = nullptr);
void launch_uniques(int64_t n, const int32_t *rep_of, const int32_t *seed_rank, int32_t *uniq_of, int32_t *seed_read,
                    int32_t *abundance, hipStream_t st);
void launch_len_hist(int32_t U, const int32_t *seed_read, const int32_t *len, int32_t *hist, int32_t lcap, hipStream_t st, int32_t nb = 0 );
void launch_len_scatter(int32_t U, const int32_t *seed_read, const int32_t *len, int32_t *cursor, int32_t lcap,
// ... 480 lines not shown
void launch_mr_ensemble(const MrArgs &a, int nwaves, int wave0, hipStream_t st, int64_t one_first = 0, int64_t one_count = 0);
void launch_mr_ensemble_big(const MrArgs &a, int nwaves, hipStream_t st);
void launch_mr_overflowed(const MrOut *out, int64_t nu, int32_t *list, unsigned long long *n, hipStream_t st);
struct RegionListArgs {
  PairOut *pout; const RegionRec *raw; RegionPoolView pv; int64_t npairs;
  const int32_t *mr_off; const int32_t *mr_u; const MrOut *mrout; const int32_t *envpool;
};
void launch_region_list_count(const RegionListArgs &a, int32_t *cnt, unsigned long long *counters, hipStream_t st);
void launch_region_list_fill(const RegionListArgs &a, const int64_t *pair_region0, RegionRec *out, hipStream_t st);

struct ScoreArgs {
  ReadsDev rd;
  const int32_t *sorted_uniq, *seed_read;
  const DevProfile *prof;
  const LenTables *lt;
  const float *flogsum;
  const PairRec *pairs;
  const PairOut *pout;
  const RegionRec *regions;
  const RegionOut *rout;
  const int64_t *pair_region0;
  const int32_t *upos;
  itsx_domain *dom;
  int64_t npairs;
  double T;
  const MrRec *mr; const int32_t *mr_u; const MrOut *mrout; const int64_t *n2off; const float *n2sc; const int32_t *mr_off;
  int32_t *domz;
  const int32_t *usample;
  int32_t P;
};
void launch_score(const ScoreArgs &a, hipStream_t st);
void launch_region_count_fill(const PairOut *pout, const RegionRec *raw, int64_t npairs, const int32_t *pref,
                              const int64_t *seg_pair_start, const int64_t *seg_region_start, const int32_t *seg_of_pair_base,
                              RegionRec *out, hipStream_t st);

__host__ __device__ __forceinline__ unsigned long long rank_key(const itsx_domain &d)
{
  long long tenths = (long long)__builtin_rint((double)d.bitscore * 10.0) + (1ll << 23);
  if (tenths < 0) tenths = 0;
  if (tenths > (1ll << 24) - 1) tenths = (1ll << 24) - 1;
  const unsigned long long di = (unsigned long long)(d.dom_idx < 0 ? 0 : (d.dom_idx > 0xFFFFF ? 0xFFFFF : d.dom_idx));
  return ((unsigned long long)tenths << 40) | ((unsigned long long)(0xFFFFF - (d.prof & 0xFFFFF)) << 20) | (0xFFFFFull - di);
}

constexpr int LAZY_TENTHS_BIAS = 1 << 23;
struct LazyArgs {
  const PairRec *pairs; int64_t NP;
  const float *fb;
  const LenTables *lt;
  const int8_t *cls; int32_t ncls;
  const int32_t *sorted_uniq;
  uint32_t *b10;
  unsigned long long *gtop;
  const unsigned long long *bestc;
  uint8_t *done;
  int32_t *flag;
};
void launch_lazy_bound(const LazyArgs &a, hipStream_t st);
void launch_lazy_mark(const LazyArgs &a, int round, hipStream_t st);
void launch_lazy_scatter(const PairRec *pairs, int64_t NP, const int32_t *flag, const int32_t *pos, const int64_t *seg_old, const int64_t *seg_new,
                         PairRec *out, hipStream_t st);
void launch_finalize_lazy(itsx_domain *dom, int64_t n, const int64_t *zlb, const int64_t *zub, double domE, const int32_t *usample, int P, hipStream_t st);
void launch_lazy_sure(const itsx_domain *dom, int64_t n, const int8_t *cls, int ncls, unsigned long long *sure, int32_t *has, hipStream_t st);
void launch_lazy_pending(const itsx_domain *dom, int64_t n, const int8_t *cls, int ncls, const unsigned long long *sure, const int32_t *has,
                         unsigned long long *count, int32_t *prof_flag, uint8_t *uniq_flag, unsigned long long *zneed , const unsigned long long *zsplit , double domE, hipStream_t st);
void launch_topup_count(const uint8_t *done, const int64_t *seg_start, const int32_t *total, const int32_t *prof_of_slot, int nslots, unsigned long long *cnt, hipStream_t st);
void launch_topup_keys(const PairRec *pairs, int64_t NP, const uint8_t *done, const uint32_t *b10, const int32_t *slot_of_prof, int32_t *flag, const int32_t *pos ,
                       unsigned long long *keys, int32_t *vals, hipStream_t st);
void launch_topup_mark(const PairRec *pairs, int64_t NP, uint8_t *done, const uint32_t *b10, const int32_t *slot_of_prof, const uint32_t *cutoff, int32_t *flag, hipStream_t st);

}
```

### itsxpress_amd/csrc/k_derep.hip

```cpp
#include "engine.h"
#include "k_api.h"

namespace itsx {

static constexpr uint64_t XP1 = 11400714785074694791ULL, XP2 = 14029467366897019727ULL,
                          XP3 = 1609587929392839161ULL, XP4 = 9650029242287828579ULL,
                          XP5 = 2870177450012600261ULL;
__device__ __forceinline__ uint64_t rotl64(uint64_t x, int r) { return (x << r) | (x >> (64 - r)); }
__device__ __forceinline__ uint64_t xround(uint64_t acc, uint64_t in) { acc += in * XP2; acc = rotl64(acc, 31); return acc * XP1; }
__device__ __forceinline__ uint64_t xmerge(uint64_t acc, uint64_t v) { acc ^= xround(0, v); return acc * XP1 + XP4; }

__device__ __forceinline__ uint32_t comp_code(uint32_t c)
{
  const uint64_t lut = 0xFBCDEA9785640123ULL;
  return (uint32_t)(lut >> (4 * c)) & 15u;
}

__device__ __forceinline__ uint32_t rev_fields(uint32_t w)
{
  w = __brev(w);
  return ((w >> 1) & 0x55555555u) | ((w & 0x55555555u) << 1);
}

__device__ __forceinline__ uint32_t rc_word(const uint32_t *__restrict__ w, int L, int nw, int j)
// ... 243 lines not shown
      todo &= ~same;
    }
  }
}

struct RegKey {
  const uint32_t *w; const uint32_t *exc; int nexc, nw_read, off, Ld, prof, L;
  int nwd, nex_in;
  __device__ __forceinline__ uint32_t word(int j) const
  {
    const int start = off + 16 * j;
    const int a = start >> 4, s = (start & 15) * 2;
    const uint32_t lo = w[a];
    const uint32_t up = (a + 1 < nw_read) ? w[a + 1] : 0u;
    uint32_t W = s ? ((lo >> s) | (up << (32 - s))) : lo;
    const int cnt = Ld - 16 * j;
    if (cnt < 16) W &= (1u << (2 * cnt)) - 1u;
    return W;
  }
  __device__ __forceinline__ uint32_t operator()(int j) const
  {
    if (j < nwd) return word(j);
    j -= nwd;
    if (j < nex_in) {
      int seen = 0;
      for (int e = 0; e < nexc; e++) {
        const int p = (int)(exc[e] >> 4);
        if (p >= off && p < off + Ld) { if (seen == j) return ((uint32_t)(p - off) << 4) | (exc[e] & 15u); seen++; }
      }
      return 0u;
    }
    j -= nex_in;
    return j == 0 ? (uint32_t)prof : j == 1 ? (uint32_t)L : (uint32_t)Ld;
  }
};
__device__ __forceinline__ RegKey make_regkey(const ReadsDev &rd, int read, int ienv, int jenv, int prof, int L)
{
  RegKey k;
  const int64_t wo = rd.woff[read], eo = rd.excoff[read];
  k.w = rd.words + wo; k.exc = rd.exc + eo; k.nexc = (int)(rd.excoff[read + 1] - eo); k.nw_read = (int)(rd.woff[read + 1] - wo);
  k.off = ienv - 1; k.Ld = jenv - ienv + 1; k.prof = prof; k.L = L;
  k.nwd = (k.Ld + 15) >> 4;
  int n = 0;
  for (int e = 0; e < k.nexc; e++) { const int p = (int)(k.exc[e] >> 4); n += (p >= k.off && p < k.off + k.Ld); }
  k.nex_in = n;
  return k;
}

__global__ void __launch_bounds__(256) k_region_keys(ReadsDev rd, const RegionRec *__restrict__ regions, int64_t nr, const PairRec *__restrict__ pairs,
                                                     const int32_t *__restrict__ sorted_uniq, const int32_t *__restrict__ seed_read,
                                                     unsigned long long *__restrict__ keys, int32_t *__restrict__ vals, uint64_t mask,
                                                     uint32_t *__restrict__ slot_of)
{
  for (int64_t g = (int64_t)blockIdx.x * blockDim.x + threadIdx.x; g < nr; g += (int64_t)gridDim.x * blockDim.x) {
    const RegionRec rg = regions[g];
    if (rg.pair < 0) { slot_of[g] = 0xFFFFFFFFu; continue; }
    const PairRec pr = pairs[rg.pair];
    const RegKey rk = make_regkey(rd, seed_read[sorted_uniq[pr.useq]], rg.ienv, rg.jenv, pr.prof, pr.L);
    uint64_t key = xxh64_words(rk, rk.nwd + rk.nex_in + 3, 0x9E3779B97F4A7C15ULL);
    if (key == 0) key = 1;
    uint64_t slot = (key * 0x9E3779B97F4A7C15ULL >> 20) & mask;
    for (;;) {
      const unsigned long long old = atomicCAS(&keys[slot], 0ull, (unsigned long long)key);
      if (old == 0ull || old == key) { atomicMin(&vals[slot], (int32_t)g); slot_of[g] = (uint32_t)slot; break; }
      slot = (slot + 1) & mask;
    }
  }
}
__global__ void __launch_bounds__(256) k_region_resolve(ReadsDev rd, const RegionRec *__restrict__ regions, int64_t nr, const PairRec *__restrict__ pairs,
                                                        const int32_t *__restrict__ sorted_uniq, const int32_t *__restrict__ seed_read,
                                                        const int32_t *__restrict__ vals, const uint32_t *__restrict__ slot_of,
                                                        int32_t *__restrict__ rep_region, int32_t *__restrict__ is_uniq)
{
  for (int64_t g = (int64_t)blockIdx.x * blockDim.x + threadIdx.x; g < nr; g += (int64_t)gridDim.x * blockDim.x) {
    const uint32_t slot = slot_of[g];
    if (slot == 0xFFFFFFFFu) { rep_region[g] = -1; is_uniq[g] = 0; continue; }
    int32_t s = vals[slot];
    if (s != (int32_t)g) {
      const RegionRec a = regions[g], b = regions[s];
      const PairRec pa = pairs[a.pair], pb = pairs[b.pair];
      bool same = pa.prof == pb.prof && pa.L == pb.L && (a.jenv - a.ienv) == (b.jenv - b.ienv);
      if (same) {
        const RegKey ka = make_regkey(rd, seed_read[sorted_uniq[pa.useq]], a.ienv, a.jenv, pa.prof, pa.L);
        const RegKey kb = make_regkey(rd, seed_read[sorted_uniq[pb.useq]], b.ienv, b.jenv, pb.prof, pb.L);
        same = ka.nex_in == kb.nex_in;
        for (int j = 0; same && j < ka.nwd + ka.nex_in; j++) same = ka(j) == kb(j);
      }
      if (!same) s = (int32_t)g;
    }
    rep_region[g] = s; is_uniq[g] = (s == (int32_t)g);
  }
}
__global__ void __launch_bounds__(256) k_region_upos(int64_t nr, const RegionRec *__restrict__ regions, const PairRec *__restrict__ pairs,
                                                     const int32_t *__restrict__ is_uniq, const int32_t *__restrict__ urank,
                                                     const int64_t *__restrict__ rseg, const int64_t *__restrict__ useg,
                                                     int32_t *__restrict__ upos, RegionRec *__restrict__ ulist)
{
  for (int64_t g = (int64_t)blockIdx.x * blockDim.x + threadIdx.x; g < nr; g += (int64_t)gridDim.x * blockDim.x) {
    if (!is_uniq[g]) continue;
    const RegionRec rg = regions[g];
    const int p = pairs[rg.pair].prof;
    const int64_t pos = useg[p] + (int64_t)(urank[g] - urank[rseg[p]]);
    upos[g] = (int32_t)pos;
    ulist[pos] = rg;
  }
}
__global__ void __launch_bounds__(256) k_region_upos_follow(int64_t nr, const int32_t *__restrict__ rep_region, const int32_t *__restrict__ is_uniq,
                                                            int32_t *__restrict__ upos)
{
  for (int64_t g = (int64_t)blockIdx.x * blockDim.x + threadIdx.x; g < nr; g += (int64_t)gridDim.x * blockDim.x) {
    const int32_t s = rep_region[g];
    if (s >= 0 && !is_uniq[g]) upos[g] = upos[s];
  }
}

static inline int grid_for(int64_t n, int block = 256, int cap = 8192)
{
  int64_t g = (n + block - 1) / block;
  if (g < 1) g = 1;
// ... 62 lines not shown
```

### itsxpress_amd/csrc/k_lazy.hip

```cpp
#include "engine.h"
#include "k_api.h"
#include "detmath.h"
#include "k_vec.h"

namespace itsx {

constexpr int BP = BOUND_PAIRS;
typedef const f4 __attribute__((address_space(4))) *cf4q;
struct BT { f2 mm, im, dm, mi, ii, bm, md; float dd1, dd2; };
DEV BT ldbt(const float *tab, int j)
{
  const f4 a = *(cf4q)(uintptr_t)(tab + j * 16), b = *(cf4q)(uintptr_t)(tab + j * 16 + 4), c = *(cf4q)(uintptr_t)(tab + j * 16 + 8),
           d = *(cf4q)(uintptr_t)(tab + j * 16 + 12);
  BT t;
  t.mm = (f2){a.x, a.y}; t.im = (f2){a.z, a.w}; t.dm = (f2){b.x, b.y}; t.ii = (f2){b.z, b.w};
  t.bm = (f2){c.x, c.y}; t.dd1 = c.z; t.dd2 = c.w; t.mi = (f2){d.x, d.y}; t.md = (f2){d.z, d.w};
  return t;
}
DEV f2 pfma(f2 a, f2 b, f2 c) { return __builtin_elementwise_fma(a, b, c); }

#ifndef ITSX_FWD_WPB
#define ITSX_FWD_WPB 1
#endif
constexpr int FWD_WPB = ITSX_FWD_WPB;
// ... 324 lines not shown
void launch_bwd_bound_share(const FloatArgs &a, const float *btab, const float *rtab, int nwaves, int wave0, const ShareLaunch &sl, hipStream_t st)
{
  if (nwaves <= 0) return;
  const dim3 g((nwaves + FWD_WPB - 1) / FWD_WPB), b(64 * FWD_WPB);
  hipLaunchKernelGGL(k_bwd_bound, g, b, 0, st, a, wave0, nwaves, btab, rtab, sl);
}

static float bound_rescale()
{
  static const float v = [] { const char *e = sw_get("ITSX_BOUND_RESCALE_EXP"); const double x = e ? atof(e) : 20.0; return (float)pow(10.0, x < 4.0 ? 4.0 : x > 28.0 ? 28.0 : x); }();
  return v;
}
void launch_fwd_bound_seq(const FloatArgs &a, const float *btab, bool fold, float *fb, int nwaves, int wave0, hipStream_t st)
{
  if (nwaves <= 0) return;
  ShareLaunch none{}; none.rescale = bound_rescale();
  const dim3 g((nwaves + FWD_WPB - 1) / FWD_WPB), b(64 * FWD_WPB);
  if (fold) hipLaunchKernelGGL((k_fwd_bound<false, true>), g, b, 0, st, a, wave0, nwaves, btab, fb, none);
  else hipLaunchKernelGGL((k_fwd_bound<false, false>), g, b, 0, st, a, wave0, nwaves, btab, fb, none);
}
void launch_fwd_bound_share(const FloatArgs &a, const float *btab, bool fold, float *fb, int nwaves, int wave0, const ShareLaunch &sl0, hipStream_t st)
{
  if (nwaves <= 0) return;
  ShareLaunch sl = sl0; sl.rescale = bound_rescale();
  const dim3 g((nwaves + FWD_WPB - 1) / FWD_WPB), b(64 * FWD_WPB);
  if (fold) hipLaunchKernelGGL((k_fwd_bound<true, true>), g, b, 0, st, a, wave0, nwaves, btab, fb, sl);
  else hipLaunchKernelGGL((k_fwd_bound<true, false>), g, b, 0, st, a, wave0, nwaves, btab, fb, sl);
}

__global__ void __launch_bounds__(256) k_lazy_bound(LazyArgs a)
{
  const int64_t i = (int64_t)blockIdx.x * blockDim.x + threadIdx.x;
  if (i >= a.NP) return;
  const PairRec pr = a.pairs[i];
  if (pr.prof < 0) { a.b10[i] = 0u; return; }
  if (pr.xj < 0) { a.b10[i] = 0u; a.done[i] = 1; return; }
  const float f = a.fb[i];
  const LenTables lt = a.lt[pr.L];
  uint32_t b;
  if (f != f || f == __builtin_inff()) b = (1u << 24) - 1;
  else if (f == -__builtin_inff()) b = 1u;
  else {
    const double bits = ((double)f - (double)lt.nullsc) / 0.69314718055994529 + (double)lt.lazy_c;
    double t = __builtin_floor(bits * 10.0 + 0.5) + (double)LAZY_TENTHS_BIAS;
    if (t < 1.0) t = 1.0;
    if (t > (double)((1 << 24) - 1)) t = (double)((1 << 24) - 1);
    b = (uint32_t)t;
  }
  a.b10[i] = b;
  const size_t g = (size_t)pr.useq * a.ncls + a.cls[pr.prof];
  atomicMax(&a.gtop[g], ((unsigned long long)b << 32) | (unsigned long long)(0xFFFFFFFFu - (uint32_t)i));
}

__global__ void __launch_bounds__(256) k_lazy_mark(LazyArgs a, int round)
{
  const int64_t i = (int64_t)blockIdx.x * blockDim.x + threadIdx.x;
  if (i > a.NP) return;
  int f = 0;
  if (i < a.NP) {
    const PairRec pr = a.pairs[i];
    if (pr.prof >= 0 && !a.done[i]) {
      const int c = a.cls[pr.prof];
      if (round == 0) f = (uint32_t)(a.gtop[(size_t)pr.useq * a.ncls + c] & 0xFFFFFFFFull) == 0xFFFFFFFFu - (uint32_t)i;
      else {
        const unsigned long long bc = a.bestc[(size_t)a.sorted_uniq[pr.useq] * a.ncls + c];
        f = bc == 0ull || a.b10[i] >= (uint32_t)(bc >> 40);
      }
      if (f) a.done[i] = 1;
    }
  }
  a.flag[i] = f;
}

__global__ void __launch_bounds__(256) k_lazy_scatter(const PairRec *__restrict__ pairs, int64_t NP, const int32_t *__restrict__ flag,
                                                      const int32_t *__restrict__ pos, const int64_t *__restrict__ seg_old,
                                                      const int64_t *__restrict__ seg_new, PairRec *__restrict__ out)
{
  const int64_t i = (int64_t)blockIdx.x * blockDim.x + threadIdx.x;
  if (i >= NP || !flag[i]) return;
  const PairRec pr = pairs[i];
  out[seg_new[pr.prof] + (int64_t)(pos[i] - pos[seg_old[pr.prof]])] = pr;
}

__global__ void __launch_bounds__(256) k_finalize_lazy(itsx_domain *__restrict__ dom, int64_t n, const int64_t *__restrict__ zlb,
                                                       const int64_t *__restrict__ zub, double domE, const int32_t *__restrict__ usample, int P)
{
  const int64_t i = (int64_t)blockIdx.x * blockDim.x + threadIdx.x;
  if (i >= n) return;
  const itsx_domain d = dom[i];
  if (d.dom_idx < 0) return;
  int rep = 0;
  if (d.seq_reported) {
    const size_t z = (size_t)(usample ? usample[d.rep] * P : 0) + d.prof;
    const double p = det_exp(d.lnP);
    const double lo = (double)(zlb[z] > 1 ? zlb[z] : 1), hi = (double)(zub[z] > 1 ? zub[z] : 1);
    rep = (p * hi <= domE) ? 1 : (p * lo <= domE) ? 2 : 0;
  }
  dom[i].dom_reported = rep;
}

__global__ void __launch_bounds__(256) k_lazy_sure(const itsx_domain *__restrict__ dom, int64_t n, const int8_t *__restrict__ cls, int ncls,
                                                   unsigned long long *__restrict__ sure, int32_t *__restrict__ has)
{
  const int64_t i = (int64_t)blockIdx.x * blockDim.x + threadIdx.x;
  if (i >= n) return;
  const itsx_domain d = dom[i];
  if (d.dom_idx < 0 || d.dom_reported != 1) return;
  has[d.rep] = 1;
  atomicMax(&sure[(size_t)d.rep * ncls + cls[d.prof]], rank_key(d));
}
__global__ void __launch_bounds__(256) k_lazy_pending(const itsx_domain *__restrict__ dom, int64_t n, const int8_t *__restrict__ cls, int ncls,
                                                      const unsigned long long *__restrict__ sure, const int32_t *__restrict__ has,
                                                      unsigned long long *__restrict__ count, int32_t *__restrict__ prof_flag,
                                                      uint8_t *__restrict__ uniq_flag, unsigned long long *__restrict__ zneed, const unsigned long long *__restrict__ zsplit,
                                                      double domE)
{
  const int64_t i = (int64_t)blockIdx.x * blockDim.x + threadIdx.x;
  int c = 0;
  if (i < n) {
    const itsx_domain d = dom[i];
    if (d.dom_idx >= 0 && d.dom_reported == 2) c = !has[d.rep] || rank_key(d) > sure[(size_t)d.rep * ncls + cls[d.prof]];
    if (c) {
      prof_flag[d.prof] = 1; uniq_flag[d.rep] = 1;
      if (zneed) {
        const double z = domE / det_exp(d.lnP);
        if (z < 9.0e18) {
          const unsigned long long zf = (unsigned long long)z;
          if (zf + 2ull <= zsplit[d.prof]) atomicMax(&zneed[2 * d.prof], zf + 2ull);
          else atomicMin(&zneed[2 * d.prof + 1], zf > 2ull ? zf - 2ull : 0ull);
        } else atomicMin(&zneed[2 * d.prof + 1], (unsigned long long)9.0e18);
      }
    }
  }
  const unsigned long long m = __ballot(c);
  if (m && (threadIdx.x & 63) == (unsigned)__builtin_ctzll(m)) atomicAdd(count, (unsigned long long)__builtin_popcountll(m));
}

void launch_lazy_bound(const LazyArgs &a, hipStream_t st)
{
  if (a.NP > 0) hipLaunchKernelGGL(k_lazy_bound, dim3((unsigned)((a.NP + 255) / 256)), dim3(256), 0, st, a);
}
void launch_lazy_mark(const LazyArgs &a, int round, hipStream_t st)
{
  hipLaunchKernelGGL(k_lazy_mark, dim3((unsigned)((a.NP + 1 + 255) / 256)), dim3(256), 0, st, a, round);
}
void launch_lazy_scatter(const PairRec *pairs, int64_t NP, const int32_t *flag, const int32_t *pos, const int64_t *seg_old, const int64_t *seg_new,
                         PairRec *out, hipStream_t st)
{
  if (NP > 0) hipLaunchKernelGGL(k_lazy_scatter, dim3((unsigned)((NP + 255) / 256)), dim3(256), 0, st, pairs, NP, flag, pos, seg_old, seg_new, out);
}
void launch_finalize_lazy(itsx_domain *dom, int64_t n, const int64_t *zlb, const int64_t *zub, double domE, const int32_t *usample, int P, hipStream_t st)
{
  if (n > 0) hipLaunchKernelGGL(k_finalize_lazy, dim3((unsigned)((n + 255) / 256)), dim3(256), 0, st, dom, n, zlb, zub, domE, usample, P);
}
void launch_lazy_sure(const itsx_domain *dom, int64_t n, const int8_t *cls, int ncls, unsigned long long *sure, int32_t *has, hipStream_t st)
{
  if (n > 0) hipLaunchKernelGGL(k_lazy_sure, dim3((unsigned)((n + 255) / 256)), dim3(256), 0, st, dom, n, cls, ncls, sure, has);
}
void launch_lazy_pending(const itsx_domain *dom, int64_t n, const int8_t *cls, int ncls, const unsigned long long *sure, const int32_t *has,
                         unsigned long long *count, int32_t *prof_flag, uint8_t *uniq_flag, unsigned long long *zneed, const unsigned long long *zsplit, double domE, hipStream_t st)
{
  if (n > 0) hipLaunchKernelGGL(k_lazy_pending, dim3((unsigned)((n + 255) / 256)), dim3(256), 0, st, dom, n, cls, ncls, sure, has, count, prof_flag, uniq_flag, zneed, zsplit, domE);
}
__global__ void __launch_bounds__(256) k_topup_count(const uint8_t *__restrict__ done, const int64_t *__restrict__ seg_start, const int32_t *__restrict__ total,
                                                     const int32_t *__restrict__ prof_of_slot, unsigned long long *__restrict__ cnt)
{
  const int sl = blockIdx.y, p = prof_of_slot[sl];
  const int64_t base = seg_start[p], n = total[p];
  unsigned long long c = 0;
  for (int64_t i = (int64_t)blockIdx.x * 256 + threadIdx.x; i < n; i += (int64_t)gridDim.x * 256) c += done[base + i] != 0;
  for (int o = 32; o >= 1; o >>= 1) c += __shfl_xor(c, o, 64);
  if ((threadIdx.x & 63) == 0 && c) atomicAdd(&cnt[sl], c);
}
void launch_topup_count(const uint8_t *done, const int64_t *seg_start, const int32_t *total, const int32_t *prof_of_slot, int nslots, unsigned long long *cnt, hipStream_t st)
{
  if (nslots > 0) hipLaunchKernelGGL(k_topup_count, dim3(512, (unsigned)nslots), dim3(256), 0, st, done, seg_start, total, prof_of_slot, cnt);
}

__global__ void __launch_bounds__(256) k_topup_keys(const PairRec *__restrict__ pairs, int64_t NP, const uint8_t *__restrict__ done, const uint32_t *__restrict__ b10,
                                                    const int32_t *__restrict__ slot_of_prof, int32_t *__restrict__ flag, const int32_t *__restrict__ pos,
                                                    unsigned long long *__restrict__ keys, int32_t *__restrict__ vals)
{
  const int64_t i = (int64_t)blockIdx.x * blockDim.x + threadIdx.x;
  if (i > NP) return;
  int f = 0, sl = -1;
  if (i < NP) {
    const PairRec pr = pairs[i];
    if (pr.prof >= 0 && pr.xj >= 0 && !done[i]) { sl = slot_of_prof[pr.prof]; f = sl >= 0; }
  }
  if (!pos) { flag[i] = f; return; }
  if (f) { keys[pos[i]] = ((unsigned long long)sl << 32) | (unsigned long long)(0xFFFFFFFFu - b10[i]); vals[pos[i]] = (int32_t)i; }
}
__global__ void __launch_bounds__(256) k_topup_mark(const PairRec *__restrict__ pairs, int64_t NP, uint8_t *__restrict__ done, const uint32_t *__restrict__ b10,
                                                    const int32_t *__restrict__ slot_of_prof, const uint32_t *__restrict__ cutoff, int32_t *__restrict__ flag)
{
  const int64_t i = (int64_t)blockIdx.x * blockDim.x + threadIdx.x;
  if (i > NP) return;
  int f = 0;
  if (i < NP) {
    const PairRec pr = pairs[i];
    if (pr.prof >= 0 && pr.xj >= 0 && !done[i]) {
      const int sl = slot_of_prof[pr.prof];
      if (sl >= 0) { const uint32_t hi = cutoff[2 * sl], lo = cutoff[2 * sl + 1], b = b10[i]; f = (hi > 0 && b >= hi) || (lo > 0 && b <= lo); }
    }
    if (f) done[i] = 1;
  }
  flag[i] = f;
}
void launch_topup_keys(const PairRec *pairs, int64_t NP, const uint8_t *done, const uint32_t *b10, const int32_t *slot_of_prof, int32_t *flag, const int32_t *pos,
                       unsigned long long *keys, int32_t *vals, hipStream_t st)
{
  hipLaunchKernelGGL(k_topup_keys, dim3((unsigned)((NP + 1 + 255) / 256)), dim3(256), 0, st, pairs, NP, done, b10, slot_of_prof, flag, pos, keys, vals);
}
void launch_topup_mark(const PairRec *pairs, int64_t NP, uint8_t *done, const uint32_t *b10, const int32_t *slot_of_prof, const uint32_t *cutoff, int32_t *flag, hipStream_t st)
{
  hipLaunchKernelGGL(k_topup_mark, dim3((unsigned)((NP + 1 + 255) / 256)), dim3(256), 0, st, pairs, NP, done, b10, slot_of_prof, cutoff, flag);
}

}
```

Baseline: 4.646 million.

## Replace per-pair flag arrays with 64-bit chunk bitmasks and chunk-level scans

The lazy-selection and top-up stages now record selected pairs as one 64-bit ballot mask per 64-pair chunk plus a per-chunk count, in place of a 32-bit flag per pair. The exclusive scan then runs over chunk counts instead of every pair, and the scatter and key-fill kernels recover each rank with a popcount. Round zero now seeds the mask from a per-group kernel (k_lazy_first) instead of testing every pair. The aim is to cut memory traffic and scan length in the selection passes. In exchange it requires the pair list to be padded to whole chunks of 64, and it adds debug entry points for the scan, select and region-key paths.

```diff
diff --git a/include/itsx_hip.h b/include/itsx_hip.h
--- a/include/itsx_hip.h
+++ b/include/itsx_hip.h
@@ -289,6 +289,12 @@
 int itsx_debug_detmath(itsx_ctx *ctx, const double *x, int64_t n, double *out_log, double *out_exp);
 int itsx_debug_logf(itsx_ctx *ctx, const float *x, int64_t n, float *out);
 int itsx_debug_dust(itsx_ctx *ctx, uint8_t *masked);
+int itsx_debug_scan(itsx_ctx *ctx, const int32_t *in, int64_t n, int32_t *out, int in_place);
+int itsx_debug_select(itsx_ctx *ctx, int mode, const int32_t *pairs, int64_t NP, const int64_t *seg_start, int32_t P, uint8_t *done, const uint32_t *b10,
+                      const int8_t *cls, int32_t ncls, const unsigned long long *group, int64_t n_group, const int32_t *sorted_uniq, int64_t n_sorted,
+                      const int32_t *slot_of_prof, const uint32_t *cutoff, int32_t n_slots, int64_t *out_seg, int32_t *out_pairs, int64_t out_cap,
+                      unsigned long long *out_keys, int32_t *out_vals, int64_t *out_n);
+int itsx_debug_region_keys(itsx_ctx *ctx, const int32_t *regions, int64_t n_regions, const int32_t *pairs, int64_t n_pairs, int32_t *rep_region, int32_t *is_uniq);
 
 #ifdef __cplusplus
 }
diff --git a/itsxpress_amd/_lib.py b/itsxpress_amd/_lib.py
--- a/itsxpress_amd/_lib.py
+++ b/itsxpress_amd/_lib.py
@@ -85,7 +85,8 @@
            "itsx_twriter_set_device",
            "itsx_inflate_device", "itsx_inflate_fetch", "itsx_debug_inflate_host", "itsx_debug_inflate_candidates", "itsx_debug_inflate_where", "itsx_set_device_inflate",
            "itsx_parse_device", "itsx_parse_fetch", "itsx_debug_parse_host", "itsx_set_device_parse",
-           "itsx_debug_set_domains", "itsx_debug_get_rows"]
+           "itsx_debug_set_domains", "itsx_debug_get_rows",
+           "itsx_debug_scan", "itsx_debug_select", "itsx_debug_region_keys"]
 
 
 def lib():
@@ -218,6 +219,9 @@
         "itsx_debug_detmath": (i32, [vp, vp, i64, vp, vp]),
         "itsx_debug_logf": (i32, [vp, vp, i64, vp]),
         "itsx_debug_dust": (i32, [vp, vp]),
+        "itsx_debug_scan": (i32, [vp, vp, i64, vp, i32]),
+        "itsx_debug_select": (i32, [vp, i32, vp, i64, vp, i32, vp, vp, vp, i32, vp, i64, vp, i64, vp, vp, i32, vp, vp, i64, vp, vp, vp]),
+        "itsx_debug_region_keys": (i32, [vp, vp, i64, vp, i64, vp, vp]),
         "itsx_debug_calibrate": (i32, [vp, i32, f64, i32, vp, vp]),
         "itsx_debug_issue": (i32, [vp, i32, i32, i32, vp, vp]),
         "itsx_shard_text": (i32, [C.c_char_p, i32, vp, C.c_char_p, vp, vp]),
diff --git a/itsxpress_amd/csrc/engine.hip b/itsxpress_amd/csrc/engine.hip
--- a/itsxpress_amd/csrc/engine.hip
+++ b/itsxpress_amd/csrc/engine.hip
@@ -100,6 +100,18 @@
 {
   const int i = blockIdx.x * blockDim.x + threadIdx.x;
   if (i < n) out[i] = src[idx[i]];
+}
+static uint64_t region_table_size(int64_t n)
+{
+  uint64_t tsize = 1024;
+  while (tsize < (uint64_t)n * 2 + 16) tsize <<= 1;
+  return tsize;
+}
+
+__global__ void k_gather_chunk_i32(const int32_t *src, const int64_t *idx, int n, int32_t *out)
+{
+  const int i = blockIdx.x * blockDim.x + threadIdx.x;
+  if (i < n) out[i] = src[idx[i] >> 6];
 }
 __global__ void k_rep_coords(int32_t U, const unsigned long long *bl, const unsigned long long *br, const int32_t *cl, const int32_t *cr,
                              const int32_t *seed_read, const int32_t *len, int32_t *start, int32_t *stop, int32_t *tlen)
@@ -358,7 +370,7 @@
   bool completing = false;
   std::vector<int32_t> h_plist; DBuf<int32_t> d_plist;
   int64_t s_Uc = 0; int s_Lcap = 0;
-  DBuf<float> l_fb; DBuf<uint32_t> l_b10; DBuf<uint8_t> l_done; DBuf<int32_t> l_flag, l_pos, l_scan, l_has; DBuf<unsigned long long> l_gtop, l_sure;
+  DBuf<float> l_fb; DBuf<uint32_t> l_b10; DBuf<uint8_t> l_done; DBuf<unsigned long long> l_smask; DBuf<int32_t> l_scnt, l_spos, l_scan, l_has; DBuf<unsigned long long> l_gtop, l_sure;
   DBuf<PairRec> l_pairs; DBuf<int64_t> l_seg, l_zub; DBuf<int32_t> l_pflag; DBuf<uint8_t> l_uflag; bool partial_coords = false; bool kept_rows = false; std::vector<int32_t> lazy_pending_prof;
   std::vector<uint16_t> thr_memo; std::vector<char> thr_memo_have; double thr_memo_F1 = -1.0; int thr_memo_Ppad = 0;
   DBuf<int32_t> w_coords4; DBuf<int64_t> w_keys128; DBuf<uint64_t> w_hf1, w_hr1;
@@ -2131,8 +2143,8 @@
   if (ctx->lazy) {
     size_t fr = 0, tot = 0;
     if (hipMemGetInfo(&fr, &tot) == hipSuccess) {
-      const double held = (double)ctx->d_pairs.cap * sizeof(PairRec) + (double)ctx->l_fb.cap * 4 + (double)ctx->l_b10.cap * 4 + (double)ctx->l_flag.cap * 4 +
-                          (double)ctx->l_pos.cap * 4 + (double)ctx->l_done.cap + (double)ctx->w_res.cap * 2;
+      const double held = (double)ctx->d_pairs.cap * sizeof(PairRec) + (double)ctx->l_fb.cap * 4 + (double)ctx->l_b10.cap * 4 + (double)ctx->l_smask.cap * 8 +
+                          (double)ctx->l_scnt.cap * 4 + (double)ctx->l_spos.cap * 4 + (double)ctx->l_done.cap + (double)ctx->w_res.cap * 2;
       lazy_budget = std::min<int64_t>(lazy_budget, (int64_t)(((double)fr + held) / 3.0 / 64.0));
       lazy_budget = std::max<int64_t>(lazy_budget, (int64_t)1 << 20);
     }
@@ -2371,7 +2383,7 @@
       launch_mr_fill(pl.pout, d_raw.p, pv, NP, mroff.p, ctx->w_mr.p, st);
       DBuf<unsigned long long> &rkeys = ctx->w_keys; DBuf<int32_t> &rvals = ctx->w_vals; DBuf<uint32_t> &rslot = ctx->w_slot_of;
       DBuf<int32_t> &rrep = ctx->w_rrep, &ruq = ctx->w_ruq, &rurank = ctx->w_rurank, &rscan = ctx->w_scan_tmp;
-      uint64_t tsize = 1024; while (tsize < (uint64_t)NMR * 2 + 16) tsize <<= 1;
+      const uint64_t tsize = region_table_size(NMR);
       HIPCHK(rkeys.alloc(tsize)); HIPCHK(rvals.alloc(tsize)); HIPCHK(rslot.alloc((size_t)NMR + 1));
       HIPCHK(rrep.alloc((size_t)NMR + 1)); HIPCHK(ruq.alloc((size_t)NMR + 1)); HIPCHK(rurank.alloc((size_t)NMR + 1)); HIPCHK(rscan.alloc((size_t)scan_tmp_elems(NMR + 1)));
       HIPCHK(hipMemsetAsync(rkeys.p, 0, tsize * sizeof(unsigned long long), st));
@@ -2565,7 +2577,7 @@
     launch_region_list_fill(rl, ctx->d_pair_region0.p, ctx->d_regions.p, st);
     DBuf<unsigned long long> &rkeys = ctx->w_keys; DBuf<int32_t> &rvals = ctx->w_vals; DBuf<uint32_t> &rslot = ctx->w_slot_of;
     DBuf<int32_t> &rrep = ctx->w_rrep, &ruq = ctx->w_ruq, &rurank = ctx->w_rurank, &rscan = ctx->w_scan_tmp;
-    uint64_t tsize = 1024; while (tsize < (uint64_t)NR * 2 + 16) tsize <<= 1;
+    const uint64_t tsize = region_table_size(NR);
     HIPCHK(rkeys.alloc(tsize)); HIPCHK(rvals.alloc(tsize)); HIPCHK(rslot.alloc((size_t)NR + 1));
     HIPCHK(rrep.alloc((size_t)NR + 1)); HIPCHK(ruq.alloc((size_t)NR + 1)); HIPCHK(rurank.alloc((size_t)NR + 1));
     HIPCHK(rscan.alloc((size_t)scan_tmp_elems(NR + 1))); HIPCHK(ctx->d_upos.alloc((size_t)NR + 1));
@@ -2669,10 +2681,10 @@
 
 
 namespace itsx {
-__global__ void k_dbg_group_count(const PairRec *__restrict__ pairs, int64_t NP, const int32_t *__restrict__ flag, const int8_t *__restrict__ cls, int ncls, unsigned long long *__restrict__ cnt)
+__global__ void k_dbg_group_count(const PairRec *__restrict__ pairs, int64_t NP, const unsigned long long *__restrict__ smask, const int8_t *__restrict__ cls, int ncls, unsigned long long *__restrict__ cnt)
 {
   const int64_t i = (int64_t)blockIdx.x * blockDim.x + threadIdx.x;
-  if (i >= NP || !flag[i]) return;
+  if (i >= NP || !((smask[i >> 6] >> (i & 63)) & 1ull)) return;
   const PairRec pr = pairs[i];
   if (pr.prof < 0) return;
   atomicAdd(&cnt[(size_t)pr.useq * ncls + cls[pr.prof]], 1ull);
@@ -2689,6 +2701,41 @@
 }
 }
 
+static int select_compact(itsx_ctx *ctx, const PairRec *pairs, int64_t NP, int P, const std::vector<int64_t> &seg_start, const int64_t *d_seg_start, PairList &sub, int64_t &nsel)
+{
+  hipStream_t st = ctx->st;
+  const int64_t nch = (NP + 63) >> 6;
+  launch_exclusive_scan(ctx->l_scnt.p, ctx->l_spos.p, nch + 1, ctx->l_scan.p, st);
+  std::vector<int32_t> bound((size_t)P + 1);
+  {
+    DBuf<int64_t> &d_idx = ctx->w_idx; DBuf<int32_t> &d_b = ctx->w_b;
+    HIPCHK(upload(d_idx, seg_start, st)); HIPCHK(d_b.alloc((size_t)P + 1));
+    hipLaunchKernelGGL(k_gather_chunk_i32, dim3((P + 1 + 255) / 256), dim3(256), 0, st, ctx->l_spos.p, d_idx.p, P + 1, d_b.p);
+    HIPCHK(hipMemcpyAsync(bound.data(), d_b.p, ((size_t)P + 1) * 4, hipMemcpyDeviceToHost, st));
+    HIPCHK(hipStreamSynchronize(st));
+  }
+  sub.seg_start.assign((size_t)P + 1, 0); sub.total.assign((size_t)P, 0);
+  for (int p = 0; p < P; p++) { sub.total[(size_t)p] = bound[(size_t)p + 1] - bound[(size_t)p]; sub.seg_start[(size_t)p + 1] = sub.seg_start[(size_t)p] + ((int64_t)sub.total[(size_t)p] + 63) / 64 * 64; }
+  sub.NP = sub.seg_start[(size_t)P];
+  nsel = (int64_t)bound[(size_t)P] - bound[0];
+  if (sub.NP == 0) return ITSX_OK;
+  HIPCHK(ctx->l_pairs.alloc((size_t)sub.NP)); HIPCHK(ctx->d_pout.alloc((size_t)sub.NP));
+  HIPCHK(hipMemsetAsync(ctx->l_pairs.p, 0xFF, (size_t)sub.NP * sizeof(PairRec), st));
+  HIPCHK(hipMemsetAsync(ctx->d_pout.p, 0, (size_t)sub.NP * sizeof(PairOut), st));
+  HIPCHK(upload(ctx->l_seg, sub.seg_start, st));
+  launch_lazy_scatter(pairs, NP, ctx->l_smask.p, ctx->l_spos.p, d_seg_start, ctx->l_seg.p, ctx->l_pairs.p, st);
+  sub.pairs = ctx->l_pairs.p; sub.pout = ctx->d_pout.p; sub.d_seg_start = ctx->l_seg.p;
+  return ITSX_OK;
+}
+static int select_alloc(itsx_ctx *ctx, int64_t NP)
+{
+  if (NP & 63) SET_ERR(ctx, ITSX_E_DEVICE, "lazy stage: the pair list is not padded to whole chunks of 64");
+  const int64_t nch = NP >> 6;
+  HIPCHK(ctx->l_smask.alloc((size_t)nch + 1)); HIPCHK(ctx->l_scnt.alloc((size_t)nch + 2)); HIPCHK(ctx->l_spos.alloc((size_t)nch + 2));
+  HIPCHK(ctx->l_scan.alloc((size_t)scan_tmp_elems(nch + 2)));
+  return ITSX_OK;
+}
+
 static int lazy_rounds(itsx_ctx *ctx, const PairList &pl, const int32_t *d_sorted, int32_t u0, int32_t Uc, double T, double F1, double F3, const std::function<int()> *next_msv)
 {
   hipStream_t st = ctx->st;
@@ -2696,7 +2743,7 @@
   itsx_stats &S = ctx->stats;
   const int64_t NP = pl.NP;
   HIPCHK(ctx->l_fb.alloc((size_t)NP + 1)); HIPCHK(ctx->l_b10.alloc((size_t)NP + 1)); HIPCHK(ctx->l_done.alloc((size_t)NP + 1));
-  HIPCHK(ctx->l_flag.alloc((size_t)NP + 2)); HIPCHK(ctx->l_pos.alloc((size_t)NP + 2)); HIPCHK(ctx->l_scan.alloc((size_t)scan_tmp_elems(NP + 2)));
+  { const int rc = select_alloc(ctx, NP); if (rc != ITSX_OK) return rc; }
   HIPCHK(ctx->l_gtop.alloc((size_t)Uc * ncls + 1));
   HIPCHK(hipMemsetAsync(ctx->l_done.p, 0, (size_t)NP + 1, st));
   HIPCHK(hipMemsetAsync(ctx->l_gtop.p, 0, ((size_t)Uc * ncls + 1) * sizeof(unsigned long long), st));
@@ -2958,7 +3005,7 @@
   StageTimer tm_sel(st);
   LazyArgs la{};
   la.pairs = pl.pairs; la.NP = NP; la.fb = ctx->l_fb.p; la.lt = ctx->d_lt.p; la.cls = ctx->w_cls.p; la.ncls = ncls; la.sorted_uniq = d_sorted;
-  la.b10 = ctx->l_b10.p; la.gtop = ctx->l_gtop.p; la.bestc = ctx->w_bestc.p; la.done = ctx->l_done.p; la.flag = ctx->l_flag.p;
+  la.b10 = ctx->l_b10.p; la.gtop = ctx->l_gtop.p; la.bestc = ctx->w_bestc.p; la.done = ctx->l_done.p; la.smask = ctx->l_smask.p; la.scnt = ctx->l_scnt.p; la.ngroups = (int64_t)Uc * ncls;
   launch_lazy_bound(la, st);
   float ms_sel = tm_sel.stop();
   for (int round = 0; round < 2; round++) {
@@ -2967,7 +3014,7 @@
     if (round == 1 && sw_get("ITSX_LAZY_HIST")) {
       const int64_t ng = (int64_t)Uc * ncls;
       HIPCHK(hipMemsetAsync(ctx->l_gtop.p, 0, (size_t)ng * 8, st));
-      hipLaunchKernelGGL(k_dbg_group_count, dim3((unsigned)((NP + 255) / 256)), dim3(256), 0, st, pl.pairs, NP, ctx->l_flag.p, ctx->w_cls.p, ncls, ctx->l_gtop.p);
+      hipLaunchKernelGGL(k_dbg_group_count, dim3((unsigned)((NP + 255) / 256)), dim3(256), 0, st, pl.pairs, NP, ctx->l_smask.p, ctx->w_cls.p, ncls, ctx->l_gtop.p);
       DBuf<unsigned long long> hist; HIPCHK(hist.alloc(16)); HIPCHK(hipMemsetAsync(hist.p, 0, 16 * 8, st));
       hipLaunchKernelGGL(k_dbg_group_hist, dim3((unsigned)((ng + 255) / 256)), dim3(256), 0, st, ctx->l_gtop.p, ng, hist.p);
       unsigned long long h[16];
@@ -2975,32 +3022,14 @@
       fprintf(stderr, "[itsx] round 2 candidates per group: 0:%llu 1:%llu 2:%llu 3:%llu 4:%llu 5-8:%llu 9-16:%llu 17+:%llu; pairs beyond a group's first %llu, beyond its second %llu\n",
               h[0], h[1], h[2], h[3], h[4], h[5], h[6], h[7], h[8], h[9]);
     }
-    launch_exclusive_scan(ctx->l_flag.p, ctx->l_pos.p, NP + 1, ctx->l_scan.p, st);
-    std::vector<int32_t> bound((size_t)P + 1);
-    {
-      DBuf<int64_t> &d_idx = ctx->w_idx; DBuf<int32_t> &d_b = ctx->w_b;
-      HIPCHK(upload(d_idx, pl.seg_start, st)); HIPCHK(d_b.alloc((size_t)P + 1));
-      hipLaunchKernelGGL(k_gather_i32, dim3((P + 1 + 255) / 256), dim3(256), 0, st, ctx->l_pos.p, d_idx.p, P + 1, d_b.p);
-      HIPCHK(hipMemcpyAsync(bound.data(), d_b.p, ((size_t)P + 1) * 4, hipMemcpyDeviceToHost, st));
-      HIPCHK(hipStreamSynchronize(st));
-    }
-    PairList sub;
-    sub.seg_start.assign((size_t)P + 1, 0); sub.total.assign((size_t)P, 0);
-    for (int p = 0; p < P; p++) { sub.total[(size_t)p] = bound[(size_t)p + 1] - bound[(size_t)p]; sub.seg_start[(size_t)p + 1] = sub.seg_start[(size_t)p] + ((int64_t)sub.total[(size_t)p] + 63) / 64 * 64; }
-    sub.NP = sub.seg_start[(size_t)P];
-    const int64_t nsel = (int64_t)bound[(size_t)P] - bound[0];
+    PairList sub; int64_t nsel = 0;
+    { const int rc = select_compact(ctx, pl.pairs, NP, P, pl.seg_start, pl.d_seg_start, sub, nsel); if (rc != ITSX_OK) return rc; }
     const bool last = round == 1;
     if (sub.NP == 0) {
       ms_sel += tm_r.stop();
       if (last && next_msv) { const int rc = (*next_msv)(); if (rc != ITSX_OK) return rc; }
       continue;
     }
-    HIPCHK(ctx->l_pairs.alloc((size_t)sub.NP)); HIPCHK(ctx->d_pout.alloc((size_t)sub.NP));
-    HIPCHK(hipMemsetAsync(ctx->l_pairs.p, 0xFF, (size_t)sub.NP * sizeof(PairRec), st));
-    HIPCHK(hipMemsetAsync(ctx->d_pout.p, 0, (size_t)sub.NP * sizeof(PairOut), st));
-    HIPCHK(upload(ctx->l_seg, sub.seg_start, st));
-    launch_lazy_scatter(pl.pairs, NP, ctx->l_flag.p, ctx->l_pos.p, pl.d_seg_start, ctx->l_seg.p, ctx->l_pairs.p, st);
-    sub.pairs = ctx->l_pairs.p; sub.pout = ctx->d_pout.p; sub.d_seg_start = ctx->l_seg.p;
     ms_sel += tm_r.stop();
     S.n_lazy_evaluated += nsel;
     if (round == 0) S.n_lazy_round1 += nsel;
@@ -3440,17 +3469,18 @@
   };
   std::vector<unsigned long long> ndone;
   { const int rc = count_done(ndone); if (rc != ITSX_OK) return rc; }
-  launch_topup_keys(ctx->d_pairs.p, NP, ctx->l_done.p, ctx->l_b10.p, ctx->l_slot.p, ctx->l_flag.p, nullptr, nullptr, nullptr, st);
-  launch_exclusive_scan(ctx->l_flag.p, ctx->l_pos.p, NP + 1, ctx->l_scan.p, st);
+  const int64_t nch = (NP + 63) >> 6;
+  launch_topup_keys(ctx->d_pairs.p, NP, ctx->l_done.p, ctx->l_b10.p, ctx->l_slot.p, ctx->l_smask.p, ctx->l_scnt.p, nullptr, nullptr, nullptr, st);
+  launch_exclusive_scan(ctx->l_scnt.p, ctx->l_spos.p, nch + 1, ctx->l_scan.p, st);
   int32_t M32 = 0;
-  HIPCHK(hipMemcpyAsync(&M32, ctx->l_pos.p + NP, 4, hipMemcpyDeviceToHost, st));
+  HIPCHK(hipMemcpyAsync(&M32, ctx->l_spos.p + nch, 4, hipMemcpyDeviceToHost, st));
   HIPCHK(hipStreamSynchronize(st));
   const int64_t M = M32;
   if (M <= 0) return ITSX_OK;
   HIPCHK(ctx->sh_keys.alloc((size_t)M + 1)); HIPCHK(ctx->sh_keys2.alloc((size_t)M + 1)); HIPCHK(ctx->sh_vals.alloc((size_t)M + 1)); HIPCHK(ctx->sh_uorder.alloc((size_t)M + 1));
   const size_t sort_bytes = order_sort_bytes(M);
   HIPCHK(ctx->sh_sorttmp.alloc(sort_bytes));
-  launch_topup_keys(ctx->d_pairs.p, NP, ctx->l_done.p, ctx->l_b10.p, ctx->l_slot.p, ctx->l_flag.p, ctx->l_pos.p, ctx->sh_keys.p, ctx->sh_vals.p, st);
+  launch_topup_keys(ctx->d_pairs.p, NP, ctx->l_done.p, ctx->l_b10.p, ctx->l_slot.p, ctx->l_smask.p, ctx->l_scnt.p, ctx->l_spos.p, ctx->sh_keys.p, ctx->sh_vals.p, st);
   if (order_sort(ctx->sh_sorttmp.p, sort_bytes, ctx->sh_keys.p, ctx->sh_keys2.p, ctx->sh_vals.p, ctx->sh_uorder.p, M, st) != 0) SET_ERR(ctx, ITSX_E_DEVICE, "top-up round: the radix sort failed");
   HIPCHK(hipStreamSynchronize(st));
   auto lower = [&](unsigned long long key, int64_t &pos) -> int {
@@ -3501,28 +3531,10 @@
   }
   if (!any) return ITSX_OK;
   HIPCHK(upload(ctx->l_cut, cut, st));
-  launch_topup_mark(ctx->d_pairs.p, NP, ctx->l_done.p, ctx->l_b10.p, ctx->l_slot.p, ctx->l_cut.p, ctx->l_flag.p, st);
-  launch_exclusive_scan(ctx->l_flag.p, ctx->l_pos.p, NP + 1, ctx->l_scan.p, st);
-  std::vector<int32_t> bound((size_t)P + 1);
-  {
-    DBuf<int32_t> &d_b = ctx->w_b;
-    HIPCHK(d_b.alloc((size_t)P + 1));
-    hipLaunchKernelGGL(k_gather_i32, dim3((P + 1 + 255) / 256), dim3(256), 0, st, ctx->l_pos.p, ctx->w_idx.p, P + 1, d_b.p);
-    HIPCHK(hipMemcpyAsync(bound.data(), d_b.p, ((size_t)P + 1) * 4, hipMemcpyDeviceToHost, st));
-    HIPCHK(hipStreamSynchronize(st));
-  }
-  PairList sub;
-  sub.seg_start.assign((size_t)P + 1, 0); sub.total.assign((size_t)P, 0);
-  for (int p = 0; p < P; p++) { sub.total[(size_t)p] = bound[(size_t)p + 1] - bound[(size_t)p]; sub.seg_start[(size_t)p + 1] = sub.seg_start[(size_t)p] + ((int64_t)sub.total[(size_t)p] + 63) / 64 * 64; }
-  sub.NP = sub.seg_start[(size_t)P];
-  const int64_t nsel = (int64_t)bound[(size_t)P] - bound[0];
+  launch_topup_mark(ctx->d_pairs.p, NP, ctx->l_done.p, ctx->l_b10.p, ctx->l_slot.p, ctx->l_cut.p, ctx->l_smask.p, ctx->l_scnt.p, st);
+  PairList sub; int64_t nsel = 0;
+  { const int rc = select_compact(ctx, ctx->d_pairs.p, NP, P, tu.seg_start, ctx->w_seg_start.p, sub, nsel); if (rc != ITSX_OK) return rc; }
   if (sub.NP == 0) return ITSX_OK;
-  HIPCHK(ctx->l_pairs.alloc((size_t)sub.NP)); HIPCHK(ctx->d_pout.alloc((size_t)sub.NP));
-  HIPCHK(hipMemsetAsync(ctx->l_pairs.p, 0xFF, (size_t)sub.NP * sizeof(PairRec), st));
-  HIPCHK(hipMemsetAsync(ctx->d_pout.p, 0, (size_t)sub.NP * sizeof(PairOut), st));
-  HIPCHK(upload(ctx->l_seg, sub.seg_start, st));
-  launch_lazy_scatter(ctx->d_pairs.p, NP, ctx->l_flag.p, ctx->l_pos.p, ctx->w_seg_start.p, ctx->l_seg.p, ctx->l_pairs.p, st);
-  sub.pairs = ctx->l_pairs.p; sub.pout = ctx->d_pout.p; sub.d_seg_start = ctx->l_seg.p;
   const int32_t *d_sorted = (ctx->share_on ? ctx->sh_order.p : ctx->d_sorted_uniq.p) + tu.u0;
   ctx->trace_u0 = tu.u0;
   { StageTimer tp(st); const int rc = domain_pipeline(ctx, sub, d_sorted, ctx->T, ctx->sF1, ctx->sF3, nullptr); if (rc != ITSX_OK) return rc; S.ms_lazy_topup_stages += tp.stop(); }
@@ -5654,4 +5666,132 @@
   return ITSX_OK;
 }
 
-}
+int itsx_debug_scan(itsx_ctx *ctx, const int32_t *in, int64_t n, int32_t *out, int in_place)
+{
+  CTXCHK(ctx && n >= 0 && n < ((int64_t)1 << 31) && (n == 0 || (in && out)));
+  HIPCHK(hipSetDevice(ctx->device));
+  if (n == 0) return ITSX_OK;
+  DBuf<int32_t> din, dout, tmp;
+  HIPCHK(din.alloc((size_t)n)); HIPCHK(dout.alloc((size_t)n)); HIPCHK(tmp.alloc((size_t)scan_tmp_elems(n)));
+  HIPCHK(hipMemcpyAsync(din.p, in, (size_t)n * 4, hipMemcpyHostToDevice, ctx->st));
+  int32_t *res = in_place ? din.p : dout.p;
+  launch_exclusive_scan(din.p, res, n, tmp.p, ctx->st);
+  HIPCHK(hipMemcpyAsync(out, res, (size_t)n * 4, hipMemcpyDeviceToHost, ctx->st));
+  HIPCHK(hipStreamSynchronize(ctx->st));
+  HIPCHK(hipGetLastError());
+  return ITSX_OK;
+}
+
+int itsx_debug_select(itsx_ctx *ctx, int mode, const int32_t *pairs, int64_t NP, const int64_t *seg_start, int32_t P, uint8_t *done, const uint32_t *b10,
+                      const int8_t *cls, int32_t ncls, const unsigned long long *group, int64_t n_group, const int32_t *sorted_uniq, int64_t n_sorted,
+                      const int32_t *slot_of_prof, const uint32_t *cutoff, int32_t n_slots, int64_t *out_seg, int32_t *out_pairs, int64_t out_cap,
+                      unsigned long long *out_keys, int32_t *out_vals, int64_t *out_n)
+{
+  CTXCHK(ctx && mode >= 0 && mode <= 3 && pairs && NP > 0 && NP < ((int64_t)1 << 31) && seg_start && P > 0 && done && b10 && out_n && out_cap >= 0);
+  CTXCHK(mode > 1 || (cls && ncls > 0 && group && n_group > 0 && (mode == 0 || (sorted_uniq && n_sorted > 0))));
+  CTXCHK(mode <= 1 || (slot_of_prof && n_slots > 0 && (mode == 3 || cutoff)));
+  CTXCHK(mode <= 2 ? (out_seg && out_pairs) : (out_keys && out_vals));
+  const PairRec *hp = (const PairRec *)pairs;
+  if (seg_start[0] != 0 || seg_start[P] != NP) SET_ERR(ctx, ITSX_E_ARG, "itsx_debug_select: the segments do not cover the list");
+  for (int p = 0; p < P; p++) {
+    if (seg_start[p + 1] < seg_start[p] || (seg_start[p + 1] & 63)) SET_ERR(ctx, ITSX_E_ARG, "itsx_debug_select: segment " + std::to_string(p) + " is not a whole number of chunks of 64");
+    if (mode >= 2 && (slot_of_prof[p] < -1 || slot_of_prof[p] >= n_slots)) SET_ERR(ctx, ITSX_E_ARG, "itsx_debug_select: slot of profile " + std::to_string(p));
+    if (mode <= 1 && (cls[p] < 0 || cls[p] >= ncls)) SET_ERR(ctx, ITSX_E_ARG, "itsx_debug_select: class of profile " + std::to_string(p));
+    for (int64_t i = seg_start[p]; i < seg_start[p + 1]; i++) {
+      const PairRec &r = hp[i];
+      if (r.prof < 0) continue;
+      bool ok = r.prof == p && r.useq >= 0;
+      if (ok && mode == 0) ok = (int64_t)r.useq * ncls + cls[p] < n_group;
+      if (ok && mode == 1) ok = r.useq < n_sorted && sorted_uniq[r.useq] >= 0 && (int64_t)sorted_uniq[r.useq] * ncls + cls[p] < n_group;
+      if (!ok) SET_ERR(ctx, ITSX_E_ARG, "itsx_debug_select: pair " + std::to_string(i) + " points outside the tables");
+    }
+  }
+  HIPCHK(hipSetDevice(ctx->device));
+  hipStream_t st = ctx->st;
+  DBuf<PairRec> dp; DBuf<uint8_t> dd; DBuf<uint32_t> db, dcut; DBuf<int8_t> dcls; DBuf<unsigned long long> dg; DBuf<int32_t> dsu, dslot; DBuf<int64_t> dseg;
+  HIPCHK(dp.alloc((size_t)NP)); HIPCHK(dd.alloc((size_t)NP)); HIPCHK(db.alloc((size_t)NP)); HIPCHK(dseg.alloc((size_t)P + 1));
+  HIPCHK(hipMemcpyAsync(dp.p, pairs, (size_t)NP * sizeof(PairRec), hipMemcpyHostToDevice, st));
+  HIPCHK(hipMemcpyAsync(dd.p, done, (size_t)NP, hipMemcpyHostToDevice, st));
+  HIPCHK(hipMemcpyAsync(db.p, b10, (size_t)NP * 4, hipMemcpyHostToDevice, st));
+  HIPCHK(hipMemcpyAsync(dseg.p, seg_start, ((size_t)P + 1) * 8, hipMemcpyHostToDevice, st));
+  if (mode <= 1) {
+    HIPCHK(dcls.alloc((size_t)P)); HIPCHK(dg.alloc((size_t)n_group));
+    HIPCHK(hipMemcpyAsync(dcls.p, cls, (size_t)P, hipMemcpyHostToDevice, st));
+    HIPCHK(hipMemcpyAsync(dg.p, group, (size_t)n_group * 8, hipMemcpyHostToDevice, st));
+    if (mode == 1) { HIPCHK(dsu.alloc((size_t)n_sorted)); HIPCHK(hipMemcpyAsync(dsu.p, sorted_uniq, (size_t)n_sorted * 4, hipMemcpyHostToDevice, st)); }
+  } else {
+    HIPCHK(dslot.alloc((size_t)P)); HIPCHK(dcut.alloc((size_t)2 * n_slots));
+    HIPCHK(hipMemcpyAsync(dslot.p, slot_of_prof, (size_t)P * 4, hipMemcpyHostToDevice, st));
+    if (cutoff) HIPCHK(hipMemcpyAsync(dcut.p, cutoff, (size_t)2 * n_slots * 4, hipMemcpyHostToDevice, st));
+  }
+  { const int rc = select_alloc(ctx, NP); if (rc != ITSX_OK) return rc; }
+  if (mode == 3) {
+    const int64_t nch = NP >> 6;
+    launch_topup_keys(dp.p, NP, dd.p, db.p, dslot.p, ctx->l_smask.p, ctx->l_scnt.p, nullptr, nullptr, nullptr, st);
+    launch_exclusive_scan(ctx->l_scnt.p, ctx->l_spos.p, nch + 1, ctx->l_scan.p, st);
+    int32_t M = 0;
+    HIPCHK(hipMemcpyAsync(&M, ctx->l_spos.p + nch, 4, hipMemcpyDeviceToHost, st));
+    HIPCHK(hipStreamSynchronize(st));
+    *out_n = M;
+    if (M > 0 && M <= out_cap) {
+      DBuf<unsigned long long> dk; DBuf<int32_t> dv;
+      HIPCHK(dk.alloc((size_t)M)); HIPCHK(dv.alloc((size_t)M));
+      launch_topup_keys(dp.p, NP, dd.p, db.p, dslot.p, ctx->l_smask.p, ctx->l_scnt.p, ctx->l_spos.p, dk.p, dv.p, st);
+      HIPCHK(hipMemcpyAsync(out_keys, dk.p, (size_t)M * 8, hipMemcpyDeviceToHost, st));
+      HIPCHK(hipMemcpyAsync(out_vals, dv.p, (size_t)M * 4, hipMemcpyDeviceToHost, st));
+      HIPCHK(hipStreamSynchronize(st));
+    }
+    HIPCHK(hipGetLastError());
+    return ITSX_OK;
+  }
+  if (mode <= 1) {
+    LazyArgs la{};
+    la.pairs = dp.p; la.NP = NP; la.cls = dcls.p; la.ncls = ncls; la.sorted_uniq = dsu.p; la.b10 = db.p;
+    la.gtop = mode == 0 ? dg.p : nullptr; la.ngroups = mode == 0 ? n_group : 0; la.bestc = mode == 1 ? dg.p : nullptr; la.done = dd.p; la.smask = ctx->l_smask.p; la.scnt = ctx->l_scnt.p;
+    launch_lazy_mark(la, mode, st);
+  } else launch_topup_mark(dp.p, NP, dd.p, db.p, dslot.p, dcut.p, ctx->l_smask.p, ctx->l_scnt.p, st);
+  PairList sub; int64_t nsel = 0;
+  const std::vector<int64_t> hseg(seg_start, seg_start + P + 1);
+  { const int rc = select_compact(ctx, dp.p, NP, P, hseg, dseg.p, sub, nsel); if (rc != ITSX_OK) return rc; }
+  for (int p = 0; p <= P; p++) out_seg[p] = sub.seg_start[(size_t)p];
+  *out_n = sub.NP;
+  HIPCHK(hipMemcpyAsync(done, dd.p, (size_t)NP, hipMemcpyDeviceToHost, st));
+  if (sub.NP > 0 && sub.NP <= out_cap) HIPCHK(hipMemcpyAsync(out_pairs, sub.pairs, (size_t)sub.NP * sizeof(PairRec), hipMemcpyDeviceToHost, st));
+  HIPCHK(hipStreamSynchronize(st));
+  HIPCHK(hipGetLastError());
+  return ITSX_OK;
+}
+
+int itsx_debug_region_keys(itsx_ctx *ctx, const int32_t *regions, int64_t n_regions, const int32_t *pairs, int64_t n_pairs, int32_t *rep_region, int32_t *is_uniq)
+{
+  CTXCHK(ctx && regions && n_regions > 0 && n_regions < ((int64_t)1 << 30) && pairs && n_pairs > 0 && rep_region && is_uniq);
+  if (ctx->N <= 0) SET_ERR(ctx, ITSX_E_ARG, "itsx_debug_region_keys: no reads are loaded");
+  const RegionRec *hr = (const RegionRec *)regions; const PairRec *hp = (const PairRec *)pairs;
+  for (int64_t g = 0; g < n_regions; g++) {
+    if (hr[g].pair < 0) continue;
+    bool ok = hr[g].pair < n_pairs;
+    if (ok) { const PairRec &r = hp[hr[g].pair]; ok = r.useq >= 0 && r.useq < ctx->N && hr[g].ienv >= 1 && hr[g].jenv >= hr[g].ienv && hr[g].jenv <= ctx->h_len[(size_t)r.useq]; }
+    if (!ok) SET_ERR(ctx, ITSX_E_ARG, "itsx_debug_region_keys: region " + std::to_string(g) + " points outside its read");
+  }
+  HIPCHK(hipSetDevice(ctx->device));
+  hipStream_t st = ctx->st;
+  std::vector<int32_t> ident((size_t)ctx->N);
+  std::iota(ident.begin(), ident.end(), 0);
+  DBuf<RegionRec> dr; DBuf<PairRec> dp; DBuf<int32_t> did, dvals, drep, duq; DBuf<unsigned long long> dkeys; DBuf<uint32_t> dslot;
+  const uint64_t tsize = region_table_size(n_regions);
+  HIPCHK(dr.alloc((size_t)n_regions)); HIPCHK(dp.alloc((size_t)n_pairs)); HIPCHK(upload(did, ident, st));
+  HIPCHK(dkeys.alloc(tsize)); HIPCHK(dvals.alloc(tsize)); HIPCHK(dslot.alloc((size_t)n_regions)); HIPCHK(drep.alloc((size_t)n_regions)); HIPCHK(duq.alloc((size_t)n_regions));
+  HIPCHK(hipMemcpyAsync(dr.p, regions, (size_t)n_regions * sizeof(RegionRec), hipMemcpyHostToDevice, st));
+  HIPCHK(hipMemcpyAsync(dp.p, pairs, (size_t)n_pairs * sizeof(PairRec), hipMemcpyHostToDevice, st));
+  HIPCHK(hipMemsetAsync(dkeys.p, 0, tsize * sizeof(unsigned long long), st));
+  HIPCHK(hipMemsetAsync(dvals.p, 0x7f, tsize * sizeof(int32_t), st));
+  launch_region_keys(ctx->rd, dr.p, n_regions, dp.p, did.p, did.p, dkeys.p, dvals.p, tsize - 1, dslot.p, st);
+  launch_region_resolve(ctx->rd, dr.p, n_regions, dp.p, did.p, did.p, dvals.p, dslot.p, drep.p, duq.p, st);
+  HIPCHK(hipMemcpyAsync(rep_region, drep.p, (size_t)n_regions * 4, hipMemcpyDeviceToHost, st));
+  HIPCHK(hipMemcpyAsync(is_uniq, duq.p, (size_t)n_regions * 4, hipMemcpyDeviceToHost, st));
+  HIPCHK(hipStreamSynchronize(st));
+  HIPCHK(hipGetLastError());
+  return ITSX_OK;
+}
+
+}
diff --git a/itsxpress_amd/csrc/k_api.h b/itsxpress_amd/csrc/k_api.h
--- a/itsxpress_amd/csrc/k_api.h
+++ b/itsxpress_amd/csrc/k_api.h
@@ -556,21 +556,23 @@
   const int32_t *sorted_uniq;
   uint32_t *b10;
   unsigned long long *gtop;
+  int64_t ngroups;
   const unsigned long long *bestc;
   uint8_t *done;
-  int32_t *flag;
+  unsigned long long *smask;
+  int32_t *scnt;
 };
 void launch_lazy_bound(const LazyArgs &a, hipStream_t st);
 void launch_lazy_mark(const LazyArgs &a, int round, hipStream_t st);
-void launch_lazy_scatter(const PairRec *pairs, int64_t NP, const int32_t *flag, const int32_t *pos, const int64_t *seg_old, const int64_t *seg_new,
+void launch_lazy_scatter(const PairRec *pairs, int64_t NP, const unsigned long long *smask, const int32_t *spos, const int64_t *seg_old, const int64_t *seg_new,
                          PairRec *out, hipStream_t st);
 void launch_finalize_lazy(itsx_domain *dom, int64_t n, const int64_t *zlb, const int64_t *zub, double domE, const int32_t *usample, int P, hipStream_t st);
 void launch_lazy_sure(const itsx_domain *dom, int64_t n, const int8_t *cls, int ncls, unsigned long long *sure, int32_t *has, hipStream_t st);
 void launch_lazy_pending(const itsx_domain *dom, int64_t n, const int8_t *cls, int ncls, const unsigned long long *sure, const int32_t *has,
                          unsigned long long *count, int32_t *prof_flag, uint8_t *uniq_flag, unsigned long long *zneed , const unsigned long long *zsplit , double domE, hipStream_t st);
 void launch_topup_count(const uint8_t *done, const int64_t *seg_start, const int32_t *total, const int32_t *prof_of_slot, int nslots, unsigned long long *cnt, hipStream_t st);
-void launch_topup_keys(const PairRec *pairs, int64_t NP, const uint8_t *done, const uint32_t *b10, const int32_t *slot_of_prof, int32_t *flag, const int32_t *pos ,
+void launch_topup_keys(const PairRec *pairs, int64_t NP, const uint8_t *done, const uint32_t *b10, const int32_t *slot_of_prof, unsigned long long *smask, int32_t *scnt, const int32_t *spos ,
                        unsigned long long *keys, int32_t *vals, hipStream_t st);
-void launch_topup_mark(const PairRec *pairs, int64_t NP, uint8_t *done, const uint32_t *b10, const int32_t *slot_of_prof, const uint32_t *cutoff, int32_t *flag, hipStream_t st);
+void launch_topup_mark(const PairRec *pairs, int64_t NP, uint8_t *done, const uint32_t *b10, const int32_t *slot_of_prof, const uint32_t *cutoff, unsigned long long *smask, int32_t *scnt, hipStream_t st);
 
 }
diff --git a/itsxpress_amd/csrc/k_derep.hip b/itsxpress_amd/csrc/k_derep.hip
--- a/itsxpress_amd/csrc/k_derep.hip
+++ b/itsxpress_amd/csrc/k_derep.hip
@@ -319,19 +319,42 @@
                                                      unsigned long long *__restrict__ keys, int32_t *__restrict__ vals, uint64_t mask,
                                                      uint32_t *__restrict__ slot_of)
 {
-  for (int64_t g = (int64_t)blockIdx.x * blockDim.x + threadIdx.x; g < nr; g += (int64_t)gridDim.x * blockDim.x) {
-    const RegionRec rg = regions[g];
-    if (rg.pair < 0) { slot_of[g] = 0xFFFFFFFFu; continue; }
-    const PairRec pr = pairs[rg.pair];
-    const RegKey rk = make_regkey(rd, seed_read[sorted_uniq[pr.useq]], rg.ienv, rg.jenv, pr.prof, pr.L);
-    uint64_t key = xxh64_words(rk, rk.nwd + rk.nex_in + 3, 0x9E3779B97F4A7C15ULL);
-    if (key == 0) key = 1;
-    uint64_t slot = (key * 0x9E3779B97F4A7C15ULL >> 20) & mask;
-    for (;;) {
-      const unsigned long long old = atomicCAS(&keys[slot], 0ull, (unsigned long long)key);
-      if (old == 0ull || old == key) { atomicMin(&vals[slot], (int32_t)g); slot_of[g] = (uint32_t)slot; break; }
-      slot = (slot + 1) & mask;
-    }
+  const int lane = threadIdx.x & 63;
+  for (int64_t g = (int64_t)blockIdx.x * blockDim.x + threadIdx.x; g - lane < nr; g += (int64_t)gridDim.x * blockDim.x) {
+    uint64_t key = 0;
+    if (g < nr) {
+      const RegionRec rg = regions[g];
+      if (rg.pair < 0) slot_of[g] = 0xFFFFFFFFu;
+      else {
+        const PairRec pr = pairs[rg.pair];
+        const RegKey rk = make_regkey(rd, seed_read[sorted_uniq[pr.useq]], rg.ienv, rg.jenv, pr.prof, pr.L);
+        key = xxh64_words(rk, rk.nwd + rk.nex_in + 3, 0x9E3779B97F4A7C15ULL);
+        if (key == 0) key = 1;
+      }
+    }
+    unsigned long long todo = __ballot(key != 0);
+    int leader = lane;
+    while (todo) {
+      const int l0 = __builtin_ctzll(todo);
+      const uint64_t k0 = ((uint64_t)(uint32_t)__shfl((int)(key >> 32), l0, 64) << 32) | (uint64_t)(uint32_t)__shfl((int)key, l0, 64);
+      const unsigned long long same = __ballot(key == k0) & todo;
+      if (key == k0) leader = l0;
+      todo &= ~same;
+    }
+    uint32_t myslot = 0;
+    if (key != 0 && leader == lane) {
+      uint64_t slot = (key * 0x9E3779B97F4A7C15ULL >> 20) & mask;
+      for (;;) {
+        unsigned long long cur = __hip_atomic_load(&keys[slot], __ATOMIC_RELAXED, __HIP_MEMORY_SCOPE_AGENT);
+        if (cur == 0ull) { cur = atomicCAS(&keys[slot], 0ull, (unsigned long long)key); if (cur == 0ull) cur = key; }
+        if (cur == key) break;
+        slot = (slot + 1) & mask;
+      }
+      if (__hip_atomic_load(&vals[slot], __ATOMIC_RELAXED, __HIP_MEMORY_SCOPE_AGENT) > (int32_t)g) atomicMin(&vals[slot], (int32_t)g);
+      myslot = (uint32_t)slot;
+    }
+    myslot = (uint32_t)__shfl((int)myslot, leader, 64);
+    if (key != 0) slot_of[g] = myslot;
   }
 }
 __global__ void __launch_bounds__(256) k_region_resolve(ReadsDev rd, const RegionRec *__restrict__ regions, int64_t nr, const PairRec *__restrict__ pairs,
diff --git a/itsxpress_amd/csrc/k_lazy.hip b/itsxpress_amd/csrc/k_lazy.hip
--- a/itsxpress_amd/csrc/k_lazy.hip
+++ b/itsxpress_amd/csrc/k_lazy.hip
@@ -400,34 +400,68 @@
   atomicMax(&a.gtop[g], ((unsigned long long)b << 32) | (unsigned long long)(0xFFFFFFFFu - (uint32_t)i));
 }
 
-__global__ void __launch_bounds__(256) k_lazy_mark(LazyArgs a, int round)
+__device__ __forceinline__ void select_store(int64_t i, int64_t nch, int f, unsigned long long *__restrict__ smask, int32_t *__restrict__ scnt)
+{
+  const unsigned long long m = __ballot(f);
+  if ((threadIdx.x & 63) == 0) {
+    const int64_t c = i >> 6;
+    if (c < nch) smask[c] = m;
+    scnt[c] = (int32_t)__popcll(m);
+  }
+}
+
+__global__ void __launch_bounds__(256) k_lazy_first(LazyArgs a)
+{
+  const int64_t g = (int64_t)blockIdx.x * blockDim.x + threadIdx.x;
+  if (g >= a.ngroups) return;
+  const unsigned long long top = a.gtop[g];
+  const int64_t i = (int64_t)(0xFFFFFFFFu - (uint32_t)(top & 0xFFFFFFFFull));
+  if (i >= a.NP) return;
+  const PairRec pr = a.pairs[i];
+  if (pr.prof < 0 || a.done[i] || (int64_t)pr.useq * a.ncls + a.cls[pr.prof] != g) return;
+  a.done[i] = 1;
+  atomicOr(&a.smask[i >> 6], 1ull << (i & 63));
+}
+__global__ void __launch_bounds__(256) k_select_count(const unsigned long long *__restrict__ smask, int64_t nch, int32_t *__restrict__ scnt)
+{
+  const int64_t c = (int64_t)blockIdx.x * blockDim.x + threadIdx.x;
+  if (c <= nch) scnt[c] = c < nch ? (int32_t)__popcll(smask[c]) : 0;
+}
+__global__ void __launch_bounds__(256) k_lazy_mark(LazyArgs a)
 {
   const int64_t i = (int64_t)blockIdx.x * blockDim.x + threadIdx.x;
-  if (i > a.NP) return;
+  const int64_t nch = (a.NP + 63) >> 6;
+  if ((i >> 6) > nch) return;
   int f = 0;
   if (i < a.NP) {
     const PairRec pr = a.pairs[i];
     if (pr.prof >= 0 && !a.done[i]) {
-      const int c = a.cls[pr.prof];
-      if (round == 0) f = (uint32_t)(a.gtop[(size_t)pr.useq * a.ncls + c] & 0xFFFFFFFFull) == 0xFFFFFFFFu - (uint32_t)i;
-      else {
-        const unsigned long long bc = a.bestc[(size_t)a.sorted_uniq[pr.useq] * a.ncls + c];
-        f = bc == 0ull || a.b10[i] >= (uint32_t)(bc >> 40);
-      }
+      const unsigned long long bc = a.bestc[(size_t)a.sorted_uniq[pr.useq] * a.ncls + a.cls[pr.prof]];
+      f = bc == 0ull || a.b10[i] >= (uint32_t)(bc >> 40);
       if (f) a.done[i] = 1;
     }
   }
-  a.flag[i] = f;
-}
-
-__global__ void __launch_bounds__(256) k_lazy_scatter(const PairRec *__restrict__ pairs, int64_t NP, const int32_t *__restrict__ flag,
-                                                      const int32_t *__restrict__ pos, const int64_t *__restrict__ seg_old,
+  select_store(i, nch, f, a.smask, a.scnt);
+}
+
+constexpr int SCATTER_CHUNKS = 16;
+__global__ void __launch_bounds__(256) k_lazy_scatter(const PairRec *__restrict__ pairs, int64_t NP, const unsigned long long *__restrict__ smask,
+                                                      const int32_t *__restrict__ spos, const int64_t *__restrict__ seg_old,
                                                       const int64_t *__restrict__ seg_new, PairRec *__restrict__ out)
 {
-  const int64_t i = (int64_t)blockIdx.x * blockDim.x + threadIdx.x;
-  if (i >= NP || !flag[i]) return;
-  const PairRec pr = pairs[i];
-  out[seg_new[pr.prof] + (int64_t)(pos[i] - pos[seg_old[pr.prof]])] = pr;
+  const int lane = threadIdx.x & 63;
+  const int64_t nch = (NP + 63) >> 6;
+  const int64_t c0 = ((int64_t)blockIdx.x * 4 + (threadIdx.x >> 6)) * SCATTER_CHUNKS;
+  for (int k = 0; k < SCATTER_CHUNKS; k++) {
+    const int64_t c = c0 + k;
+    if (c >= nch) return;
+    const unsigned long long m = smask[c];
+    if (!((m >> lane) & 1ull)) continue;
+    const int64_t i = c * 64 + lane;
+    const PairRec pr = pairs[i];
+    const int32_t rank = spos[c] + (int32_t)__popcll(m & ((1ull << lane) - 1ull)) - spos[seg_old[pr.prof] >> 6];
+    out[seg_new[pr.prof] + (int64_t)rank] = pr;
+  }
 }
 
 __global__ void __launch_bounds__(256) k_finalize_lazy(itsx_domain *__restrict__ dom, int64_t n, const int64_t *__restrict__ zlb,
@@ -490,12 +524,18 @@
 }
 void launch_lazy_mark(const LazyArgs &a, int round, hipStream_t st)
 {
-  hipLaunchKernelGGL(k_lazy_mark, dim3((unsigned)((a.NP + 1 + 255) / 256)), dim3(256), 0, st, a, round);
-}
-void launch_lazy_scatter(const PairRec *pairs, int64_t NP, const int32_t *flag, const int32_t *pos, const int64_t *seg_old, const int64_t *seg_new,
+  const int64_t nch = (a.NP + 63) >> 6;
+  if (round == 0) {
+    (void)hipMemsetAsync(a.smask, 0, (size_t)nch * sizeof(unsigned long long), st);
+    if (a.ngroups > 0) hipLaunchKernelGGL(k_lazy_first, dim3((unsigned)((a.ngroups + 255) / 256)), dim3(256), 0, st, a);
+    hipLaunchKernelGGL(k_select_count, dim3((unsigned)((nch + 1 + 255) / 256)), dim3(256), 0, st, a.smask, nch, a.scnt);
+  } else hipLaunchKernelGGL(k_lazy_mark, dim3((unsigned)((nch * 64 + 64 + 255) / 256)), dim3(256), 0, st, a);
+}
+void launch_lazy_scatter(const PairRec *pairs, int64_t NP, const unsigned long long *smask, const int32_t *spos, const int64_t *seg_old, const int64_t *seg_new,
                          PairRec *out, hipStream_t st)
 {
-  if (NP > 0) hipLaunchKernelGGL(k_lazy_scatter, dim3((unsigned)((NP + 255) / 256)), dim3(256), 0, st, pairs, NP, flag, pos, seg_old, seg_new, out);
+  const int64_t nch = (NP + 63) >> 6, per_block = 4 * SCATTER_CHUNKS;
+  if (NP > 0) hipLaunchKernelGGL(k_lazy_scatter, dim3((unsigned)((nch + per_block - 1) / per_block)), dim3(256), 0, st, pairs, NP, smask, spos, seg_old, seg_new, out);
 }
 void launch_finalize_lazy(itsx_domain *dom, int64_t n, const int64_t *zlb, const int64_t *zub, double domE, const int32_t *usample, int P, hipStream_t st)
 {
@@ -526,24 +566,36 @@
 }
 
 __global__ void __launch_bounds__(256) k_topup_keys(const PairRec *__restrict__ pairs, int64_t NP, const uint8_t *__restrict__ done, const uint32_t *__restrict__ b10,
-                                                    const int32_t *__restrict__ slot_of_prof, int32_t *__restrict__ flag, const int32_t *__restrict__ pos,
-                                                    unsigned long long *__restrict__ keys, int32_t *__restrict__ vals)
+                                                    const int32_t *__restrict__ slot_of_prof, unsigned long long *__restrict__ smask, int32_t *__restrict__ scnt,
+                                                    const int32_t *__restrict__ spos, unsigned long long *__restrict__ keys, int32_t *__restrict__ vals)
 {
   const int64_t i = (int64_t)blockIdx.x * blockDim.x + threadIdx.x;
-  if (i > NP) return;
-  int f = 0, sl = -1;
-  if (i < NP) {
-    const PairRec pr = pairs[i];
-    if (pr.prof >= 0 && pr.xj >= 0 && !done[i]) { sl = slot_of_prof[pr.prof]; f = sl >= 0; }
-  }
-  if (!pos) { flag[i] = f; return; }
-  if (f) { keys[pos[i]] = ((unsigned long long)sl << 32) | (unsigned long long)(0xFFFFFFFFu - b10[i]); vals[pos[i]] = (int32_t)i; }
+  const int64_t nch = (NP + 63) >> 6;
+  if ((i >> 6) > nch) return;
+  if (!spos) {
+    int f = 0;
+    if (i < NP) {
+      const PairRec pr = pairs[i];
+      if (pr.prof >= 0 && pr.xj >= 0 && !done[i]) f = slot_of_prof[pr.prof] >= 0;
+    }
+    select_store(i, nch, f, smask, scnt);
+    return;
+  }
+  if ((i >> 6) >= nch) return;
+  const int lane = threadIdx.x & 63;
+  const unsigned long long m = smask[i >> 6];
+  if (!((m >> lane) & 1ull)) return;
+  const int32_t at = spos[i >> 6] + (int32_t)__popcll(m & ((1ull << lane) - 1ull));
+  const int sl = slot_of_prof[pairs[i].prof];
+  keys[at] = ((unsigned long long)sl << 32) | (unsigned long long)(0xFFFFFFFFu - b10[i]); vals[at] = (int32_t)i;
 }
 __global__ void __launch_bounds__(256) k_topup_mark(const PairRec *__restrict__ pairs, int64_t NP, uint8_t *__restrict__ done, const uint32_t *__restrict__ b10,
-                                                    const int32_t *__restrict__ slot_of_prof, const uint32_t *__restrict__ cutoff, int32_t *__restrict__ flag)
+                                                    const int32_t *__restrict__ slot_of_prof, const uint32_t *__restrict__ cutoff,
+                                                    unsigned long long *__restrict__ smask, int32_t *__restrict__ scnt)
 {
   const int64_t i = (int64_t)blockIdx.x * blockDim.x + threadIdx.x;
-  if (i > NP) return;
+  const int64_t nch = (NP + 63) >> 6;
+  if ((i >> 6) > nch) return;
   int f = 0;
   if (i < NP) {
     const PairRec pr = pairs[i];
@@ -553,16 +605,18 @@
     }
     if (f) done[i] = 1;
   }
-  flag[i] = f;
-}
-void launch_topup_keys(const PairRec *pairs, int64_t NP, const uint8_t *done, const uint32_t *b10, const int32_t *slot_of_prof, int32_t *flag, const int32_t *pos,
-                       unsigned long long *keys, int32_t *vals, hipStream_t st)
-{
-  hipLaunchKernelGGL(k_topup_keys, dim3((unsigned)((NP + 1 + 255) / 256)), dim3(256), 0, st, pairs, NP, done, b10, slot_of_prof, flag, pos, keys, vals);
-}
-void launch_topup_mark(const PairRec *pairs, int64_t NP, uint8_t *done, const uint32_t *b10, const int32_t *slot_of_prof, const uint32_t *cutoff, int32_t *flag, hipStream_t st)
-{
-  hipLaunchKernelGGL(k_topup_mark, dim3((unsigned)((NP + 1 + 255) / 256)), dim3(256), 0, st, pairs, NP, done, b10, slot_of_prof, cutoff, flag);
-}
-
-}
+  select_store(i, nch, f, smask, scnt);
+}
+static inline unsigned select_grid(int64_t NP) { return (unsigned)((((NP + 63) >> 6) * 64 + 64 + 255) / 256); }
+void launch_topup_keys(const PairRec *pairs, int64_t NP, const uint8_t *done, const uint32_t *b10, const int32_t *slot_of_prof, unsigned long long *smask, int32_t *scnt,
+                       const int32_t *spos, unsigned long long *keys, int32_t *vals, hipStream_t st)
+{
+  hipLaunchKernelGGL(k_topup_keys, dim3(select_grid(NP)), dim3(256), 0, st, pairs, NP, done, b10, slot_of_prof, smask, scnt, spos, keys, vals);
+}
+void launch_topup_mark(const PairRec *pairs, int64_t NP, uint8_t *done, const uint32_t *b10, const int32_t *slot_of_prof, const uint32_t *cutoff,
+                       unsigned long long *smask, int32_t *scnt, hipStream_t st)
+{
+  hipLaunchKernelGGL(k_topup_mark, dim3(select_grid(NP)), dim3(256), 0, st, pairs, NP, done, b10, slot_of_prof, cutoff, smask, scnt);
+}
+
+}
```

Result: faster. 4.753 million, median of 6 (+2.3%).
